# maxgillett/tinysplat

Measured on AMD Instinct MI355X. Metric: Gaussians*pixels/s fwd+bwd, higher is better.
Workload: dtype f32; 1 GPU; 1000000 random Gaussians, SH degree 3, 1920x1080, fwd+bwd (RGB), BASELINE configs[2]; max_per_tile=614, parallelism=single GPU, tile_lists=16x16 (gsplat's) (auto), gaussian_order=as generated (i.i.d.)

## Files before the change

include/tinysplat_hip.h:

```cpp
#ifndef TINYSPLAT_HIP_H
#define TINYSPLAT_HIP_H

#include <stdint.h>

#ifdef __cplusplus
extern "C" {
#endif

#define TS_ABI_VERSION 8

#define TS_E_BADARG (-1)
#define TS_E_DEGREE (-2)

#define TS_TILE 16
#define TS_SPLAT_RECORD_FLOATS 12
#define TS_PARTIAL_ROW_FLOATS 12

int ts_abi_version(void);

typedef struct ts_camera {
    float fx, fy, cx, cy;
    int32_t img_width, img_height;
    int32_t tile_bounds_x, tile_bounds_y;
    int32_t tile_row0, tile_rows;
    float glob_scale;
    float clip_thresh;
    int32_t wide_tiles;
    int32_t hints;
} ts_camera;
#define TS_HINT_BALANCED_WALK 1
#define TS_HINT_COOP_SPLIT (1 << 20)
#define TS_CAM_LIST_SEGMENTS(s) (((s) & 15) << 8)
#define TS_CAM_WHOLE_TILES(w16) (((w16) & 15) << 12)
#define TS_CAM_COOP_TILES(c16) (((c16) & 15) << 16)
int64_t ts_final_floats(const ts_camera* cam_host, int32_t channels);
int32_t ts_cut_tiles(const ts_camera* cam_host, int32_t* band, int32_t* whole);
int32_t ts_num_tiles(const ts_camera* cam_host);


#define TS_PROJECT_LOG_SCALES 1
#define TS_PROJECT_RAW_QUATS 2

int ts_project_fwd(int32_t n, const float* means3d, const float* scales, const float* quats,
                   const float* viewmat, const float* projmat, const ts_camera* cam_host,
                   int32_t flags, float* xys, float* depths, int32_t* radii, float* conics,
                   int32_t* num_tiles_hit, float* cov3d, void* stream);

int ts_project_bwd(int32_t n, const float* means3d, const float* scales, const float* quats,
                   const float* viewmat, const float* projmat, const ts_camera* cam_host,
                   int32_t flags, const int32_t* radii, const float* v_xy, const float* v_depth,
                   const float* v_conic, const float* v_cov3d,
                   float* v_means3d, float* v_scales, float* v_quats, void* stream);


int ts_sh_fwd(int32_t n, int32_t degrees_to_use, int32_t num_bases, const float* viewdirs,
              const float* coeffs, float* colors, void* stream);

int ts_sh_bwd(int32_t n, int32_t degrees_to_use, int32_t num_bases, const float* viewdirs,
              const float* v_colors, float* v_coeffs, void* stream);

int ts_sh_colors_fwd(int32_t n, int32_t degrees_to_use, int32_t num_bases, const float* means3d,
                     const float* origin, const float* colors_dc, const float* colors_rest,
                     float* colors, uint8_t* clamp_mask, const int32_t* live, void* stream);
int ts_sh_colors_bwd(int32_t n, int32_t degrees_to_use, int32_t num_bases, const float* means3d,
                     const float* origin, const uint8_t* clamp_mask, const float* v_colors,
                     float* v_colors_dc, float* v_colors_rest, void* stream);
int ts_colors_pack_fwd(int32_t n, int32_t degrees_to_use, int32_t num_bases, const float* means3d,
                       const float* origin, const float* colors_dc, const float* colors_rest,
                       uint8_t* clamp_mask, const int32_t* live, int32_t channels, int32_t flags,
                       const float* xys, const int32_t* radii, const float* conics, const float* opacity,
                       const int32_t* cum_tiles_hit, const ts_camera* cam_host, const float* depths,
                       float* splats, void* stream);


int64_t ts_scan_ws_ints(int32_t n);
int ts_scan_tiles(int32_t n, const int32_t* num_tiles_hit, int32_t* cum_tiles_hit,
                  int32_t* scan_ws, int32_t* total_out, void* stream);

int64_t ts_bin_ws_ints(int32_t n, int32_t num_tiles);

int ts_bin_count(int32_t n, const float* xys, const int32_t* radii, const float* splats,
                 const ts_camera* cam_host, int32_t* bin_ws, void* stream);

int ts_tile_offsets(int32_t n, int32_t num_tiles, int32_t* bin_ws, int32_t* tile_bins,
                    const int32_t* cum_tiles_hit, int64_t capacity, void* stream);
int ts_tile_offsets_stats(int32_t n, int32_t num_tiles, int32_t* bin_ws, int32_t* tile_bins,
                          const int32_t* cum_tiles_hit, int64_t capacity, int32_t* longest_list, void* stream);

int ts_bin_scatter(int32_t n, const float* xys, const int32_t* radii, const float* splats,
                   const ts_camera* cam_host, const int32_t* bin_ws, int32_t* bucket_ids, int32_t* scratch,
                   void* stream);

int ts_sort_tiles(int32_t num_tiles, const int32_t* tile_bins, const float* depths,
                  const int32_t* bucket_ids, int32_t* gaussian_ids_sorted, int32_t* sort_ws,
                  int32_t* zeroed_counter, void* stream);
int ts_sort_tiles_above(int32_t num_tiles, const int32_t* tile_bins, const float* depths,
                        const int32_t* bucket_ids, int32_t* gaussian_ids_sorted, int32_t* sort_ws,
                        int32_t* zeroed_counter, void* stream);

#define TS_RASTER_LOGIT_OPACITY 1

int ts_pack_splats(int32_t n, int32_t channels, int32_t flags, const float* xys, const int32_t* radii,
                   const float* conics, const float* colors, const float* opacity,
                   const int32_t* cum_tiles_hit, const ts_camera* cam_host, const float* depths,
                   float* splats, void* stream);

#define TS_RASTER_CLAMP_RGB 2
#define TS_RASTER_SPLIT_BLOCKS 4
#define TS_RASTER_NARROW_WAVES 8
#define TS_RASTER_FLAG_GEN(g) (((g) & 0xff) << 8)
int ts_raster_fwd(int32_t channels, int32_t flags, const ts_camera* cam_host, const int32_t* tile_bins,
                  const int32_t* gaussian_ids_sorted, const float* splats, const float* background,
                  float* out_img, float* final_Ts, int32_t* final_index, uint8_t* clamp_mask,
                  void* stream);
int ts_raster_fwd_planes(int32_t channels, int32_t flags, const ts_camera* cam_host, const int32_t* tile_bins,
                         const int32_t* gaussian_ids_sorted, const float* splats, const float* background,
                         float* out_img, float* out_depth, float* final_Ts, int32_t* final_index,
                         uint8_t* clamp_mask, void* stream);

int ts_raster_fwd_sort(int32_t channels, int32_t flags, const ts_camera* cam_host, const int32_t* tile_bins,
                       const int32_t* bucket_ids, const float* depths, int32_t* gaussian_ids_sorted,
                       const float* splats, const float* background, float* out_img, float* out_depth,
                       float* final_Ts, int32_t* final_index, uint8_t* clamp_mask, void* stream);

int ts_raster_bwd(int32_t channels, int32_t flags, int64_t num_intersects, const ts_camera* cam_host,
                  const int32_t* tile_bins, const int32_t* gaussian_ids_sorted, const float* splats,
                  const float* background, const float* final_Ts, const int32_t* final_index,
                  const float* v_out_img, const float* v_out_alpha, const uint8_t* clamp_mask,
                  float* partials, uint8_t* row_flags, void* stream);
int ts_raster_bwd_planes(int32_t channels, int32_t flags, int64_t num_intersects, const ts_camera* cam_host,
                         const int32_t* tile_bins, const int32_t* gaussian_ids_sorted, const float* splats,
                         const float* background, const float* final_Ts, const int32_t* final_index,
                         const float* v_out_img, const float* v_out_depth, int32_t planes,
                         const float* v_out_alpha, const uint8_t* clamp_mask,
                         float* partials, uint8_t* row_flags, void* stream);

int ts_reduce_partials(int32_t n, int32_t channels, int32_t flags, const int32_t* num_tiles_hit,
                       const int32_t* cum_tiles_hit, const float* partials,
                       const uint8_t* row_flags, const float* splats, float* v_xy, float* v_conic,
                       float* v_colors, float* v_opacity, float* v_depth, const uint8_t* color_mask,
                       void* stream);

#define TS_FRAME_TIGHT 1
#define TS_FRAME_SPLIT 2
#define TS_FRAME_NARROW_WAVES 8
#define TS_FRAME_DIRECT_SCATTER 32
#define TS_FRAME_PLANES 64
#define TS_FRAME_LIST_STATS 256
#define TS_FRAME_SEPARATE_SORT 128
#define TS_FRAME_STRIPE 16
#define TS_FRAME_SURVIVORS 512
typedef struct ts_frame {
    int32_t n, num_bases, sh_degree, channels, flags;
    int32_t flag_gen;
    ts_camera cam;
    const float *means, *scales, *quats, *opacities, *colors_dc, *colors_rest;
    const float *view34, *projview, *origin, *background;
    float *xys, *depths, *conics, *colors, *splats;
    int32_t *radii, *num_tiles_hit, *cum_tiles_hit;
    uint8_t* sh_mask;
    int32_t *scan_ws, *bin_ws, *tile_bins;
    int32_t* total_host;
    int64_t num_intersects;
    int64_t capacity;
    int32_t *bucket_ids, *gaussian_ids_sorted;
    float *out_img, *final_Ts;
    int32_t* final_index;
    uint8_t* clamp_mask;
    const float* v_out_img;
    float* partials;
    uint8_t* row_flags;
    float *v_xy, *v_conic, *v_colors, *v_depth, *v_opacity;
    float *v_means, *v_scales, *v_quats, *v_colors_dc, *v_colors_rest;
    float* out_depth;
    const float* v_out_depth;
    int32_t* survivors;
} ts_frame;
int32_t ts_frame_struct_bytes(void);
int ts_frame_fwd_project(const ts_frame* f, void* stream);
int ts_frame_fwd_prepare(const ts_frame* f, void* stream);
int ts_frame_fwd_composite(const ts_frame* f, void* stream);
int ts_frame_bwd_composite(const ts_frame* f, void* stream);
int ts_frame_bwd_params(const ts_frame* f, void* stream);

typedef void (*ts_entry_probe)(const char* entry, int32_t end, void* user);
int ts_set_entry_probe(ts_entry_probe fn, void* user);

#define TS_MAX_RANKS 16
#define TS_EXPORT_RECORD_FLOATS 16
typedef struct ts_stripes {
    int32_t num;
    int32_t row[TS_MAX_RANKS + 1];
} ts_stripes;
int64_t ts_route_ws_ints(int32_t n, int32_t num_ranks);
int ts_route_count(int32_t n, const float* xys, const int32_t* radii, const ts_camera* cam_host,
                   const ts_stripes* stripes_host, int32_t* route_ws, int32_t* counts, void* stream);
int ts_route_count_padded(int32_t n, const float* xys, const int32_t* radii, const ts_camera* cam_host,
                          const ts_stripes* stripes_host, const int32_t* group_base_host, int32_t* route_ws,
                          int32_t* counts, void* stream);
int ts_route_pack(int32_t n, int32_t gid_base, const float* xys, const int32_t* radii, const float* depths,
                  const float* splats, const ts_camera* cam_host, const ts_stripes* stripes_host,
                  const int32_t* route_ws, float* records, void* stream);
int ts_import_records(int32_t m, const float* records, const ts_camera* cam_host, float* xys, float* depths,
                      int32_t* radii, int32_t* num_tiles_hit, void* stream);
int ts_import_pack(int32_t m, const float* records, const int32_t* cum_tiles_hit, const ts_camera* cam_host,
                   float* splats, void* stream);
int ts_reduce_partials_rows(int32_t n, int32_t channels, int32_t flags, const int32_t* num_tiles_hit,
                            const int32_t* cum_tiles_hit, const float* partials, const uint8_t* row_flags,
                            const float* splats, float* grad_rows, void* stream);
int ts_route_accumulate(int32_t n, int32_t channels, const float* xys, const int32_t* radii, const float* splats,
                        const uint8_t* color_mask, const ts_camera* cam_host, const ts_stripes* stripes_host,
                        const int32_t* route_ws, const float* grad_rows, float* v_xy, float* v_conic,
                        float* v_colors, float* v_depth, float* v_opacity, void* stream);

int ts_shard_owner_fwd(const ts_frame* fo, const ts_stripes* stripes_host, int32_t* route_ws, int32_t* counts,
                       void* stream);
int ts_shard_owner_fwd_padded(const ts_frame* fo, const ts_stripes* stripes_host, const int32_t* group_base_host,
                              int32_t* route_ws, int32_t* counts, void* stream);
int ts_shard_owner_fwd_fused(int32_t n, int32_t degrees_to_use, int32_t num_bases, const float* means3d,
                             const float* scales, const float* quats, const float* view34, const float* projview,
                             const ts_camera* cam_host, int32_t project_flags, const float* origin,
                             const float* colors_dc, const float* colors_rest, const float* opacity, int32_t channels,
                             int32_t raster_flags, float* xys, float* depths, int32_t* radii, float* conics,
                             int32_t* num_tiles_hit, uint8_t* clamp_mask, float* splats, const ts_stripes* stripes_host,
                             const int32_t* group_base_host, int32_t* route_ws, int32_t* counts, void* stream);
int ts_shard_owner_bwd_fused(int32_t n, int32_t channels, int32_t degrees_to_use, int32_t num_bases, const float* means3d,
                             const float* scales, const float* quats, const float* view34, const float* projview,
                             const float* origin, const float* xys, const int32_t* radii, const float* splats,
                             const uint8_t* color_mask, const ts_camera* cam_host, const ts_stripes* stripes_host,
                             const int32_t* route_ws, const float* grad_rows, float* v_xy, float* v_conic,
                             float* v_colors, float* v_depth, float* v_opacity, float* v_colors_dc, float* v_colors_rest,
                             float* v_means3d, float* v_scales, float* v_quats, void* stream);
int ts_shard_stripe_fwd_import(const ts_frame* fs, const float* records, void* stream);
int ts_shard_stripe_bwd(const ts_frame* fs, float* grad_rows, void* stream);
int ts_shard_owner_bwd(const ts_frame* fo, const ts_stripes* stripes_host, const int32_t* route_ws,
                       const float* grad_rows, void* stream);

typedef struct ts_rank_step {
    ts_stripes stripes;
    int32_t group_base[TS_MAX_RANKS + 1];
    int32_t gid_base;
    int32_t send_rows, recv_rows;
    int32_t* route_ws;
    int32_t* counts;
    float *send, *recv;
    float *grad_rows, *back;
} ts_rank_step;
int32_t ts_rank_step_struct_bytes(void);
int ts_shard_rank_fwd_a(const ts_frame* fo, const ts_rank_step* r, void* stream);
int ts_shard_rank_fwd_b(const ts_frame* fs, const ts_rank_step* r, void* stream);
int ts_shard_rank_bwd_a(const ts_frame* fs, const ts_rank_step* r, void* stream);
int ts_shard_rank_bwd_b(const ts_frame* fo, const ts_rank_step* r, void* stream);


int64_t ts_photometric_ws_floats(int32_t height, int32_t width);
int ts_photometric_loss_rgbd(int32_t height, int32_t width, int32_t pixel_floats, const float* image,
                             const float* target, const float* depth_target, float w_l1,
                             float w_ssim, float w_depth, float* ws, float* v_image, void* stream);
int ts_photometric_loss(int32_t height, int32_t width, const float* image, const float* target,
                        float w_l1, float w_ssim, float* ws, float* v_image, void* stream);
int ts_photometric_loss_planes(int32_t height, int32_t width, const float* image, const float* depth,
                               const float* target, const float* depth_target, float w_l1, float w_ssim,
                               float w_depth, float* ws, float* v_image, float* v_depth, void* stream);
int ts_photometric_loss_reduce(int32_t height, int32_t width, float w_l1, float w_ssim, float w_depth,
                               const float* ws, float* out4, void* stream);

#define TS_ADAM_MAX_TENSORS 8
int ts_adam_step(int32_t num_tensors, float* const* params_host, const float* const* grads_host,
                 float* const* exp_avg_host, float* const* exp_avg_sq_host, const int64_t* numel_host,
                 const float* lr_host, const int32_t* steps_host, float beta1, float beta2, float eps,
                 void* stream);

#define TS_ADAM_MEANS 0
#define TS_ADAM_COLORS_DC 1
#define TS_ADAM_COLORS_REST 2
#define TS_ADAM_SCALES 3
#define TS_ADAM_QUATS 4
#define TS_ADAM_OPACITIES 5
typedef struct ts_adam {
    float* exp_avg[6];
    float* exp_avg_sq[6];
    float lr[6];
    int32_t step[6];
    float beta1, beta2, eps;
} ts_adam;
int ts_sh_colors_bwd_adam(int32_t n, int32_t degrees_to_use, int32_t num_bases, const float* means3d,
                          const float* origin, const uint8_t* clamp_mask, const float* v_colors,
                          float* colors_dc, float* colors_rest, const ts_adam* adam_host, void* stream);
int ts_project_bwd_adam(int32_t n, float* means3d, float* scales, float* quats, const float* viewmat,
                        const float* projmat, const ts_camera* cam_host, int32_t flags, const int32_t* radii,
                        const float* v_xy, const float* v_depth, const float* v_conic, float* opacities,
                        const float* v_opacity, const ts_adam* adam_host, void* stream);
int ts_frame_bwd_params_adam(const ts_frame* f, const ts_adam* adam_host, void* stream);

#define TS_DENSIFY_CLONE 1
#define TS_DENSIFY_SPLIT 2
#define TS_DENSIFY_PRUNE 4

typedef struct ts_densify_policy {
    float interval_densify;
    float max_dim;
    float tau_means;
    float scale_thresh;
} ts_densify_policy;

int ts_grad_accum(int32_t n, const float* v_xy, float* accum, void* stream);

int ts_densify_classify(int32_t n, const float* accum, const float* scales, const float* opacities,
                        const ts_densify_policy* policy, uint8_t* flags, void* stream);

int64_t ts_densify_ws_ints(int32_t n);
int ts_densify_plan(int32_t n, const uint8_t* flags, int32_t* ws, int32_t* counts, int32_t* src_of,
                    void* stream);

#define TS_GATHER_MAX_TENSORS 8
int ts_gather_rows(int32_t num_tensors, const float* const* src_host, float* const* dst_host,
                   const int32_t* row_floats_host, int32_t dst_rows, int32_t copy_rows,
                   const int32_t* src_of, void* stream);

int ts_split_fixup(int32_t rows, const int32_t* src_of_split, const float* means, const float* scales,
                   const float* quats, const float* z, float* means_out, float* scales_out,
                   void* stream);

int32_t ts_ply_row_floats(int32_t k_rest);
int ts_ply_pack_rows(int32_t n, int32_t k_rest, const float* means, const float* colors_dc,
                     const float* colors_rest, const float* opacities, const float* scales,
                     const float* quats, float* rows, void* stream);
int ts_ply_unpack_rows(int32_t n, int32_t k_rest, const float* rows, float* means, float* colors_dc,
                       float* colors_rest, float* opacities, float* scales, float* quats,
                       void* stream);

#define TS_KNN_MAX_K 16
int64_t ts_knn_ws_bytes(int32_t n, int32_t m, int32_t k);
int ts_knn(int32_t n, const float* points, int32_t m, const float* queries, int32_t k, float* dist,
           int32_t* idx, void* ws, int32_t* stats, void* stream);

// ... 76 lines not shown
```

tinysplat_amd/_lib.py:

```python
from __future__ import annotations

import ctypes
import os
from ctypes import POINTER, c_float, c_int32, c_int64, c_void_p
from pathlib import Path

LIB_PATH = Path(os.environ["TS_LIB_PATH"]) if os.environ.get("TS_LIB_PATH") else \
    Path(__file__).resolve().parent / "csrc" / "libtinysplat_hip.so"
ABI_VERSION = 8
HINT_BALANCED_WALK = 1
HINT_COOP_SPLIT = 1 << 20
PARTIAL_ROW_FLOATS = 12


class TsCamera(ctypes.Structure):
    _fields_ = [
        ("fx", c_float), ("fy", c_float), ("cx", c_float), ("cy", c_float),
        ("img_width", c_int32), ("img_height", c_int32),
        ("tile_bounds_x", c_int32), ("tile_bounds_y", c_int32),
        ("tile_row0", c_int32), ("tile_rows", c_int32),
        ("glob_scale", c_float), ("clip_thresh", c_float),
        ("wide_tiles", c_int32), ("hints", c_int32),
    ]


_P = c_void_p
_CAM = POINTER(TsCamera)


class TsDensifyPolicy(ctypes.Structure):
    _fields_ = [("interval_densify", c_float), ("max_dim", c_float), ("tau_means", c_float),
                ("scale_thresh", c_float)]


class TsFrame(ctypes.Structure):
    _fields_ = ([("n", c_int32), ("num_bases", c_int32), ("sh_degree", c_int32), ("channels", c_int32),
                 ("flags", c_int32), ("flag_gen", c_int32), ("cam", TsCamera)]
                + [(name, c_void_p) for name in (
                    "means", "scales", "quats", "opacities", "colors_dc", "colors_rest",
                    "view34", "projview", "origin", "background",
                    "xys", "depths", "conics", "colors", "splats",
                    "radii", "num_tiles_hit", "cum_tiles_hit", "sh_mask",
                    "scan_ws", "bin_ws", "tile_bins", "total_host")]
                + [("num_intersects", c_int64), ("capacity", c_int64)]
                + [(name, c_void_p) for name in (
                    "bucket_ids", "gaussian_ids_sorted", "out_img", "final_Ts", "final_index", "clamp_mask",
                    "v_out_img", "partials", "row_flags",
                    "v_xy", "v_conic", "v_colors", "v_depth", "v_opacity",
                    "v_means", "v_scales", "v_quats", "v_colors_dc", "v_colors_rest",
                    "out_depth", "v_out_depth", "survivors")])


_FRAME = POINTER(TsFrame)


class TsAdam(ctypes.Structure):
    _fields_ = [("exp_avg", c_void_p * 6), ("exp_avg_sq", c_void_p * 6), ("lr", c_float * 6), ("step", c_int32 * 6),
                ("beta1", c_float), ("beta2", c_float), ("eps", c_float)]


_ADAM = POINTER(TsAdam)

MAX_RANKS = 16


class TsStripes(ctypes.Structure):
    _fields_ = [("num", c_int32), ("row", c_int32 * (MAX_RANKS + 1))]


_STRIPES = POINTER(TsStripes)


class TsRankStep(ctypes.Structure):
    _fields_ = [("stripes", TsStripes), ("group_base", c_int32 * (MAX_RANKS + 1)), ("gid_base", c_int32),
                ("send_rows", c_int32), ("recv_rows", c_int32), ("route_ws", c_void_p), ("counts", c_void_p),
                ("send", c_void_p), ("recv", c_void_p), ("grad_rows", c_void_p), ("back", c_void_p)]


_RANK = POINTER(TsRankStep)

ENTRY_PROBE = ctypes.CFUNCTYPE(None, ctypes.c_char_p, c_int32, c_void_p)

SIGNATURES = {
    "ts_abi_version": (c_int32, []),
    "ts_project_fwd": (c_int32, [c_int32, _P, _P, _P, _P, _P, _CAM, c_int32, _P, _P, _P, _P, _P, _P, _P]),
    "ts_project_bwd": (c_int32, [c_int32, _P, _P, _P, _P, _P, _CAM, c_int32, _P, _P, _P, _P, _P, _P, _P, _P, _P]),
    "ts_sh_fwd": (c_int32, [c_int32, c_int32, c_int32, _P, _P, _P, _P]),
    "ts_sh_bwd": (c_int32, [c_int32, c_int32, c_int32, _P, _P, _P, _P]),
    "ts_sh_colors_fwd": (c_int32, [c_int32, c_int32, c_int32, _P, _P, _P, _P, _P, _P, _P, _P]),
    "ts_sh_colors_bwd": (c_int32, [c_int32, c_int32, c_int32, _P, _P, _P, _P, _P, _P, _P]),
    "ts_scan_ws_ints": (c_int64, [c_int32]),
    "ts_scan_tiles": (c_int32, [c_int32, _P, _P, _P, _P, _P]),
    "ts_bin_ws_ints": (c_int64, [c_int32, c_int32]),
    "ts_bin_count": (c_int32, [c_int32, _P, _P, _P, _CAM, _P, _P]),
    "ts_tile_offsets": (c_int32, [c_int32, c_int32, _P, _P, _P, c_int64, _P]),
    "ts_tile_offsets_stats": (c_int32, [c_int32, c_int32, _P, _P, _P, c_int64, _P, _P]),
    "ts_bin_scatter": (c_int32, [c_int32, _P, _P, _P, _CAM, _P, _P, _P, _P]),
    "ts_sort_tiles": (c_int32, [c_int32, _P, _P, _P, _P, _P, _P, _P]),
    "ts_sort_tiles_above": (c_int32, [c_int32, _P, _P, _P, _P, _P, _P, _P]),
    "ts_num_tiles": (c_int32, [_CAM]),
    "ts_final_floats": (c_int64, [_CAM, c_int32]),
    "ts_cut_tiles": (c_int32, [_CAM, _P, _P]),
    "ts_colors_pack_fwd": (c_int32, [c_int32, c_int32, c_int32, _P, _P, _P, _P, _P, _P, c_int32, c_int32,
                                     _P, _P, _P, _P, _P, _CAM, _P, _P, _P]),
    "ts_pack_splats": (c_int32, [c_int32, c_int32, c_int32, _P, _P, _P, _P, _P, _P, _CAM, _P, _P, _P]),
    "ts_raster_fwd": (c_int32, [c_int32, c_int32, _CAM, _P, _P, _P, _P, _P, _P, _P, _P, _P]),
    "ts_raster_bwd": (c_int32, [c_int32, c_int32, c_int64, _CAM, _P, _P, _P, _P, _P, _P, _P, _P, _P, _P, _P, _P]),
    "ts_raster_fwd_planes": (c_int32, [c_int32, c_int32, _CAM, _P, _P, _P, _P, _P, _P, _P, _P, _P, _P]),
    "ts_raster_fwd_sort": (c_int32, [c_int32, c_int32, _CAM, _P, _P, _P, _P, _P, _P, _P, _P, _P, _P, _P, _P]),
    "ts_raster_bwd_planes": (c_int32, [c_int32, c_int32, c_int64, _CAM, _P, _P, _P, _P, _P, _P, _P, _P, c_int32,
                                       _P, _P, _P, _P, _P]),
    "ts_bench_stream_read": (c_int32, [_P, c_int64, _P, _P]),
    "ts_bench_gather48": (c_int32, [_P, _P, c_int64, _P, _P]),
    "ts_photometric_ws_floats": (c_int64, [c_int32, c_int32]),
    "ts_photometric_loss": (c_int32, [c_int32, c_int32, _P, _P, c_float, c_float, _P, _P, _P]),
    "ts_photometric_loss_rgbd": (c_int32, [c_int32, c_int32, c_int32, _P, _P, _P, c_float, c_float, c_float, _P, _P, _P]),
    "ts_photometric_loss_planes": (c_int32, [c_int32, c_int32, _P, _P, _P, _P, c_float, c_float, c_float, _P, _P, _P,
                                             _P]),
    "ts_photometric_loss_reduce": (c_int32, [c_int32, c_int32, c_float, c_float, c_float, _P, _P, _P]),
    "ts_adam_step": (c_int32, [c_int32, _P, _P, _P, _P, _P, _P, _P, c_float, c_float, c_float, _P]),
    "ts_sh_colors_bwd_adam": (c_int32, [c_int32, c_int32, c_int32, _P, _P, _P, _P, _P, _P, _ADAM, _P]),
    "ts_project_bwd_adam": (c_int32, [c_int32, _P, _P, _P, _P, _P, _CAM, c_int32, _P, _P, _P, _P, _P, _P, _ADAM, _P]),
    "ts_frame_bwd_params_adam": (c_int32, [_FRAME, _ADAM, _P]),
    "ts_grad_accum": (c_int32, [c_int32, _P, _P, _P]),
    "ts_densify_classify": (c_int32, [c_int32, _P, _P, _P, POINTER(TsDensifyPolicy), _P, _P]),
    "ts_densify_ws_ints": (c_int64, [c_int32]),
    "ts_densify_plan": (c_int32, [c_int32, _P, _P, _P, _P, _P]),
    "ts_gather_rows": (c_int32, [c_int32, _P, _P, _P, c_int32, c_int32, _P, _P]),
    "ts_split_fixup": (c_int32, [c_int32, _P, _P, _P, _P, _P, _P, _P, _P]),
    "ts_ply_row_floats": (c_int32, [c_int32]),
    "ts_ply_pack_rows": (c_int32, [c_int32, c_int32, _P, _P, _P, _P, _P, _P, _P, _P]),
    "ts_ply_unpack_rows": (c_int32, [c_int32, c_int32, _P, _P, _P, _P, _P, _P, _P, _P]),
    "ts_reduce_partials": (c_int32, [c_int32, c_int32, c_int32, _P, _P, _P, _P, _P, _P, _P, _P, _P, _P, _P, _P]),
    "ts_route_ws_ints": (c_int64, [c_int32, c_int32]),
    "ts_route_count": (c_int32, [c_int32, _P, _P, _CAM, _STRIPES, _P, _P, _P]),
    "ts_route_count_padded": (c_int32, [c_int32, _P, _P, _CAM, _STRIPES, _P, _P, _P, _P]),
    "ts_route_pack": (c_int32, [c_int32, c_int32, _P, _P, _P, _P, _CAM, _STRIPES, _P, _P, _P]),
    "ts_import_records": (c_int32, [c_int32, _P, _CAM, _P, _P, _P, _P, _P]),
    "ts_import_pack": (c_int32, [c_int32, _P, _P, _CAM, _P, _P]),
    "ts_reduce_partials_rows": (c_int32, [c_int32, c_int32, c_int32, _P, _P, _P, _P, _P, _P, _P]),
    "ts_route_accumulate": (c_int32, [c_int32, c_int32, _P, _P, _P, _P, _CAM, _STRIPES, _P, _P, _P, _P, _P, _P, _P, _P]),
    "ts_shard_owner_fwd": (c_int32, [_FRAME, _STRIPES, _P, _P, _P]),
    "ts_shard_owner_fwd_padded": (c_int32, [_FRAME, _STRIPES, _P, _P, _P, _P]),
    "ts_shard_owner_fwd_fused": (c_int32, [c_int32, c_int32, c_int32, _P, _P, _P, _P, _P, _CAM, c_int32, _P, _P, _P, _P,
                                           c_int32, c_int32, _P, _P, _P, _P, _P, _P, _P, _STRIPES, _P, _P, _P, _P]),
    "ts_shard_owner_bwd_fused": (c_int32, [c_int32, c_int32, c_int32, c_int32, _P, _P, _P, _P, _P, _P, _P, _P, _P, _P,
                                           _CAM, _STRIPES, _P, _P, _P, _P, _P, _P, _P, _P, _P, _P, _P, _P, _P]),
    "ts_shard_stripe_fwd_import": (c_int32, [_FRAME, _P, _P]),
    "ts_shard_stripe_bwd": (c_int32, [_FRAME, _P, _P]),
    "ts_shard_owner_bwd": (c_int32, [_FRAME, _STRIPES, _P, _P, _P]),
    "ts_rank_step_struct_bytes": (c_int32, []),
    "ts_shard_rank_fwd_a": (c_int32, [_FRAME, _RANK, _P]),
    "ts_shard_rank_fwd_b": (c_int32, [_FRAME, _RANK, _P]),
    "ts_shard_rank_bwd_a": (c_int32, [_FRAME, _RANK, _P]),
    "ts_shard_rank_bwd_b": (c_int32, [_FRAME, _RANK, _P]),
    "ts_frame_struct_bytes": (c_int32, []),
    "ts_frame_fwd_project": (c_int32, [_FRAME, _P]),
    "ts_frame_fwd_prepare": (c_int32, [_FRAME, _P]),
    "ts_frame_fwd_composite": (c_int32, [_FRAME, _P]),
    "ts_frame_bwd_composite": (c_int32, [_FRAME, _P]),
    "ts_frame_bwd_params": (c_int32, [_FRAME, _P]),
    "ts_set_entry_probe": (c_int32, [_P, _P]),
    "ts_knn_ws_bytes": (c_int64, [c_int32, c_int32, c_int32]),
    "ts_knn": (c_int32, [c_int32, _P, c_int32, _P, c_int32, _P, _P, _P, _P, _P]),
    "ts_init_from_points": (c_int32, [c_int32, c_int32, _P, _P, _P, _P, _P, _P, _P, _P, _P, _P, _P, _P, _P, _P]),
    "ts_opacity_entropy_ws_bytes": (c_int64, [c_int32]),
    "ts_opacity_entropy": (c_int32, [c_int32, _P, _P, _P, _P, _P]),
    "ts_density_sample_ws_bytes": (c_int64, [c_int32]),
    "ts_density_sample": (c_int32, [c_int32, c_int32, c_int32, _P, _P, _P, _P, _P, _P, _P, _P, _P, _P, _P]),
    "ts_density_loss_ws_bytes": (c_int64, [c_int32]),
    "ts_density_loss": (c_int32, [c_int32, c_int32, _P, _P, _P, _P, _P, _P, _P, _P, c_int32, c_int32, _P, _P, c_int32,
                                  c_float, _P, _P, _P, _P, _P, _P, _P, _P, _P, _P]),
    "ts_segment_sum_ws_bytes": (c_int64, [c_int64, c_int32]),
    "ts_segment_sum": (c_int32, [c_int64, c_int32, c_int32, _P, _P, _P, _P, _P, _P, _P]),
    "ts_extract_pack": (c_int32, [c_int32, _P, _P, _P, _P, _P, _P, _P]),
    "ts_extract_rays": (c_int32, [c_int32, _P, c_int32, c_int32, _P, c_int32, _P, _P, _P, _P, _P, _P]),
    "ts_extract_samples": (c_int32, [c_int32, c_int32, c_int32, c_float, _P, _P, _P, _P, _P, _P, _P]),
    "ts_extract_march": (c_int32, [c_int32, c_int32, c_int32, c_float, c_float, _P, _P, _P, _P, _P, _P, _P, _P, _P, _P,
                                   _P, _P, _P]),
    "ts_extract_normals": (c_int32, [c_int32, c_int32, _P, _P, _P, _P, _P]),
    "ts_extract_chunk_bytes": (c_int64, [c_int32, c_int32, c_int32]),
    "ts_mesh_boxes": (c_int32, [c_int32, _P, _P, _P, c_float, _P, _P]),
    "ts_mesh_mark": (c_int32, [c_int32, _P, _P, _P, _P, _P]),
    "ts_mesh_chunk_bytes": (c_int64, [c_int32, c_int32]),
    "ts_mesh_corners": (c_int32, [c_int32, _P, _P, _P, _P, _P]),
    "ts_mesh_density": (c_int32, [c_int32, c_int32, _P, _P, _P, _P, _P, _P, _P, _P]),
    "ts_mesh_count": (c_int32, [c_int32, _P, _P, _P, c_float, _P, _P, _P]),
    "ts_mesh_emit": (c_int32, [c_int32, _P, _P, _P, c_float, _P, _P, _P, _P, _P, _P]),
}

_lib = None


class HipLibraryError(RuntimeError):
    pass


def load() -> ctypes.CDLL:
    global _lib
    if _lib is not None:
        return _lib
    if not LIB_PATH.exists():
        raise HipLibraryError(
            f"{LIB_PATH} is missing: tinysplat_amd has no CPU or PyTorch fallback. "
            "Build it with `python -m tinysplat_amd._build` (needs hipcc, targets gfx950).")
    stamp = LIB_PATH.with_suffix(LIB_PATH.suffix + ".flags")
    if stamp.exists() and "-DTS_" in stamp.read_text() and os.environ.get("TS_ALLOW_VARIANT_LIB") != "1":
        raise HipLibraryError(
            f"{LIB_PATH} was built with developer -DTS_* overrides (ablation variant; its results may be "
            "wrong). Rebuild with `python -m tinysplat_amd._build`, or set TS_ALLOW_VARIANT_LIB=1.")
    lib = ctypes.CDLL(str(LIB_PATH))
    for name, (res, args) in SIGNATURES.items():
        try:
            fn = getattr(lib, name)
        except AttributeError as e:
            raise HipLibraryError(f"{LIB_PATH} does not export {name}") from e
        fn.restype = res
        fn.argtypes = args
    v = lib.ts_abi_version()
    if v != ABI_VERSION:
        raise HipLibraryError(f"ABI version mismatch: library {v}, binding {ABI_VERSION}")
    if lib.ts_frame_struct_bytes() != ctypes.sizeof(TsFrame):
        raise HipLibraryError("struct ts_frame: the ctypes mirror does not match the library's layout")
    if lib.ts_rank_step_struct_bytes() != ctypes.sizeof(TsRankStep):
        raise HipLibraryError("struct ts_rank_step: the ctypes mirror does not match the library's layout")
    _lib = lib
    return lib


def check(code: int, what: str) -> None:
    if code == 0:
        return
    if code == -1:
        raise ValueError(f"{what}: bad argument (TS_E_BADARG)")
    if code == -2:
        raise ValueError(f"{what}: SH degree / number of bases not supported (TS_E_DEGREE)")
    raise RuntimeError(f"{what}: HIP error {code}")
```

tinysplat_amd/csrc/binning.hip:

```cpp
#include <hip/hip_runtime.h>

#include "../../include/tinysplat_hip.h"
#include "pack.h"
#include "splat_math.h"

namespace {

constexpr int kThreads = 256;
constexpr int kScanItems = 4;
constexpr int kScanBlock = kThreads * kScanItems;

__device__ __forceinline__ int wave_inclusive_scan(int v) {
    const int lane = threadIdx.x & 63;
#pragma unroll
    for (int d = 1; d < 64; d <<= 1) {
        const int u = __shfl_up(v, d, 64);
        if (lane >= d) v += u;
    }
    return v;
}

template <int WAVES = 4>
__device__ __forceinline__ int block_inclusive_scan(int v, int* total) {
    __shared__ int wave_sums[WAVES];
    const int lane = threadIdx.x & 63, wave = threadIdx.x >> 6;
    int inc = wave_inclusive_scan(v);
    if (lane == 63) wave_sums[wave] = inc;
    __syncthreads();
    int add = 0, tot = 0;
#pragma unroll
    for (int w = 0; w < WAVES; ++w) {
        const int s = wave_sums[w];
        if (w < wave) add += s;
        tot += s;
    }
    *total = tot;
    __syncthreads();
    return inc + add;
}

__global__ __launch_bounds__(kThreads) void scan_local_kernel(int n, const int* __restrict__ in,
                                                              int* __restrict__ out,
                                                              int* __restrict__ block_sums,
                                                              int* __restrict__ total_out) {
    const int base = blockIdx.x * kScanBlock + threadIdx.x * kScanItems;
    int v[kScanItems];
    int sum = 0;
#pragma unroll
    for (int k = 0; k < kScanItems; ++k) {
        v[k] = (base + k < n) ? in[base + k] : 0;
        sum += v[k];
        v[k] = sum;
    }
    int total;
    const int inc = block_inclusive_scan(sum, &total);
    const int excl = inc - sum;
#pragma unroll
    for (int k = 0; k < kScanItems; ++k)
        if (base + k < n) {
            out[base + k] = v[k] + excl;
            if (total_out && gridDim.x == 1 && base + k == n - 1)
                __hip_atomic_store(total_out, v[k] + excl, __ATOMIC_RELEASE, __HIP_MEMORY_SCOPE_SYSTEM);
        }
    if (threadIdx.x == 0) block_sums[blockIdx.x] = total;
}

__global__ __launch_bounds__(kThreads) void scan_add_kernel(int n, int* __restrict__ out,
                                                            const int* __restrict__ block_sums,
                                                            int* __restrict__ total_out) {
    __shared__ int red[kThreads / 64];
    int part = 0;
    for (int j = threadIdx.x; j < (int)blockIdx.x; j += kThreads) part += block_sums[j];
#pragma unroll
    for (int d = 32; d >= 1; d >>= 1) part += __shfl_xor(part, d, 64);
    if ((threadIdx.x & 63) == 0) red[threadIdx.x >> 6] = part;
    __syncthreads();
    int add = 0;
#pragma unroll
    for (int w = 0; w < kThreads / 64; ++w) add += red[w];
    const int base = blockIdx.x * kScanBlock + threadIdx.x * kScanItems;
#pragma unroll
    for (int k = 0; k < kScanItems; ++k)
        if (base + k < n) {
            const int v = out[base + k] + add;
            if (blockIdx.x != 0) out[base + k] = v;
            if (total_out && base + k == n - 1)
                __hip_atomic_store(total_out, v, __ATOMIC_RELEASE, __HIP_MEMORY_SCOPE_SYSTEM);
        }
}

#ifndef TS_BIN_THREADS
#define TS_BIN_THREADS 1024
#endif
constexpr int kBinThreads = TS_BIN_THREADS;
#ifndef TS_BIN_CHUNK
#define TS_BIN_CHUNK 4096
#endif
constexpr int kBinChunkMin = TS_BIN_CHUNK;
constexpr int kBinMaxChunks = 512;
constexpr int kBinWindowMax = 36864;
constexpr int kBinTargetBlocks = 1;

__host__ __device__ inline int bin_num_chunks(int n) {
    int per = n / 192;
    per = per < 1024 ? 1024 : (per > kBinChunkMin ? kBinChunkMin : per);
    int b = (n + per - 1) / per;
    if (b < 1) b = 1;
    if (b > kBinMaxChunks) b = kBinMaxChunks;
    return b;
}

inline int bin_window_tiles(int n, int num_tiles) {
    const int chunks = bin_num_chunks(n);
    int nwin = (kBinTargetBlocks + chunks - 1) / chunks;
    const int max_win = (num_tiles + 255) / 256;
    if (nwin > max_win) nwin = max_win;
    if (nwin < 1) nwin = 1;
    int window = (num_tiles + nwin - 1) / nwin;
    window = (window + 63) & ~63;
    if (window > kBinWindowMax) window = kBinWindowMax;
    return window;
}

using ts::TightTest;

#ifndef TS_BIN_PRE
#define TS_BIN_PRE 2
#endif
constexpr int kBinPre = TS_BIN_PRE;
template <typename Emit>
__device__ __forceinline__ void walk_chunk(int g0, int g1, const float* __restrict__ xys,
                                           const int* __restrict__ radii,
                                           const float4* __restrict__ splats, const ts_camera& cam,
                                           Emit emit) {
    const int ws = cam.wide_tiles ? 1 : 0;
    const int tbx = (cam.tile_bounds_x + ws) >> ws;
    const bool tight_lists = splats != nullptr;
    for (int base = g0 + threadIdx.x; base < g1; base += kBinPre * kBinThreads) {
        int r[kBinPre];
        float2 xy[kBinPre];
        float4 q0[kBinPre], q1[kBinPre];
#pragma unroll
        for (int u = 0; u < kBinPre; ++u) {
            const int i = base + u * kBinThreads;
            r[u] = i < g1 ? radii[i] : 0;
        }
#pragma unroll
        for (int u = 0; u < kBinPre; ++u) {
            const int i = base + u * kBinThreads;
            xy[u] = make_float2(0.f, 0.f);
            q0[u] = q1[u] = make_float4(0.f, 0.f, 0.f, 0.f);
            if (r[u] > 0) {
                xy[u] = reinterpret_cast<const float2*>(xys)[i];
                if (tight_lists) { q0[u] = splats[3 * (size_t)i]; q1[u] = splats[3 * (size_t)i + 1]; }
            }
        }
#pragma unroll
        for (int u = 0; u < kBinPre; ++u) {
            if (r[u] <= 0) continue;
            const ts::TileBox b = ts::tile_bbox(xy[u].x, xy[u].y, (float)r[u], cam.tile_bounds_x,
                                                cam.tile_bounds_y, cam.tile_row0, cam.tile_rows);
            if (b.maxy <= b.miny || b.maxx <= b.minx) continue;
            const TightTest tight(tight_lists, q0[u].x, q0[u].y, q0[u].z, q0[u].w, q1[u].x, q1[u].y, (float)r[u]);
            if (tight.cull_all) continue;
            const int i = base + u * kBinThreads;
            for (int ty = b.miny; ty < b.maxy; ++ty) {
                int lo, hi;
                tight.row_range(ty, b.minx, b.maxx, lo, hi);
                if (hi <= lo) continue;
                for (int tx = lo >> ws; tx <= (hi - 1) >> ws; ++tx) emit((ty - cam.tile_row0) * tbx + tx, i);
            }
        }
    }
}

constexpr int kItemCap = 4096;
constexpr int kStashWords = 11;
constexpr size_t kBalancedLds = (size_t)(kStashWords * kBinThreads + kItemCap + 32) * 4;
template <typename Emit>
__device__ __forceinline__ void walk_chunk_balanced(int g0, int g1, const float* __restrict__ xys,
                                                    const int* __restrict__ radii,
                                                    const float4* __restrict__ splats, const ts_camera& cam,
                                                    Emit emit) {
    static_assert(kBinThreads == 1024, "one Gaussian per thread and batch, items packed as lt | row << 10");
    __shared__ float stash[kStashWords][kBinThreads];
    __shared__ int items[kItemCap];
    __shared__ int wave_sum[kBinThreads / 64 + 1];
    const int ws = cam.wide_tiles ? 1 : 0;
    const int tbx = (cam.tile_bounds_x + ws) >> ws;
    const bool tight_lists = splats != nullptr;
    const int tid = threadIdx.x, lane = tid & 63, wave = tid >> 6;
    for (int base = g0; base < g1; base += kBinThreads) {
        const int i = base + tid;
        int rows = 0, miny = 0;
        if (i < g1) {
            const int r = radii[i];
            if (r > 0) {
                const float2 xy = reinterpret_cast<const float2*>(xys)[i];
                float4 q0 = make_float4(0.f, 0.f, 0.f, 0.f), q1 = q0;
                if (tight_lists) { q0 = splats[3 * (size_t)i]; q1 = splats[3 * (size_t)i + 1]; }
                const ts::TileBox b = ts::tile_bbox(xy.x, xy.y, (float)r, cam.tile_bounds_x, cam.tile_bounds_y,
                                                    cam.tile_row0, cam.tile_rows);
                if (b.maxy > b.miny && b.maxx > b.minx) {
                    const TightTest t(tight_lists, q0.x, q0.y, q0.z, q0.w, q1.x, q1.y, (float)r);
                    if (!t.cull_all) {
                        rows = b.maxy - b.miny;
                        miny = b.miny;
                        stash[0][tid] = t.geometric ? t.dymax : -1.0f;
                        stash[1][tid] = t.gx; stash[2][tid] = t.gy; stash[3][tid] = t.B; stash[4][tid] = t.D4;
                        stash[5][tid] = t.inv2A; stash[6][tid] = t.tau4A; stash[7][tid] = t.dxext;
                        stash[8][tid] = t.dy_left; stash[9][tid] = __int_as_float(b.miny);
                        stash[10][tid] = __int_as_float(b.minx | (b.maxx << 16));
                    }
                }
            }
        }
        int incl = rows;
#pragma unroll
        for (int d = 1; d < 64; d <<= 1) {
            const int v = __shfl_up(incl, d, 64);
            if (lane >= d) incl += v;
        }
        if (lane == 63) wave_sum[wave] = incl;
        __syncthreads();
        if (wave == 0) {
            int v = lane < kBinThreads / 64 ? wave_sum[lane] : 0;
#pragma unroll
            for (int d = 1; d < kBinThreads / 64; d <<= 1) {
                const int u = __shfl_up(v, d, 64);
                if (lane >= d) v += u;
            }
            if (lane < kBinThreads / 64) wave_sum[lane] = v;
        }
        __syncthreads();
        const int total = wave_sum[kBinThreads / 64 - 1];
        const int first = incl - rows + (wave > 0 ? wave_sum[wave - 1] : 0);
        for (int w0 = 0; w0 < total; w0 += kItemCap) {
            const int lo_k = max(0, w0 - first), hi_k = min(rows, w0 + kItemCap - first);
            for (int k = lo_k; k < hi_k; ++k) items[first + k - w0] = tid | (k << 10);
            __syncthreads();
            const int m = min(kItemCap, total - w0);
            for (int j = tid; j < m; j += kBinThreads) {
                const int it = items[j], lt = it & 1023, k = it >> 10;
                TightTest t(false, 0.0f, 0.0f, 0.0f, 0.0f, 0.0f, 0.0f, 0.0f);
                const float d0 = stash[0][lt];
                t.geometric = d0 >= 0.0f;
                t.dymax = d0;
                t.gx = stash[1][lt]; t.gy = stash[2][lt]; t.B = stash[3][lt]; t.D4 = stash[4][lt];
                t.inv2A = stash[5][lt]; t.tau4A = stash[6][lt]; t.dxext = stash[7][lt]; t.dy_left = stash[8][lt];
                const int ty = __float_as_int(stash[9][lt]) + k;
                const int xx = __float_as_int(stash[10][lt]);
                int lo, hi;
                t.row_range(ty, xx & 0xffff, xx >> 16, lo, hi);
                if (hi <= lo) continue;
                const int id = base + lt;
                for (int tx = lo >> ws; tx <= (hi - 1) >> ws; ++tx) emit((ty - cam.tile_row0) * tbx + tx, id);
            }
            __syncthreads();
        }
        __syncthreads();
    }
}

template <bool BAL>
__global__ __launch_bounds__(kBinThreads) void bin_count_kernel(
    int n, int chunk, const float* __restrict__ xys, const int* __restrict__ radii,
    const float4* __restrict__ splats, const ts_camera cam, int num_tiles, int window,
    int* __restrict__ counts) {
    extern __shared__ int hist[];
    const int t0 = blockIdx.y * window;
    const int tw = min(num_tiles - t0, window);
    for (int j = threadIdx.x; j < tw; j += kBinThreads) hist[j] = 0;
    __syncthreads();
    const int g0 = blockIdx.x * chunk, g1 = min(n, g0 + chunk);
    auto emit = [&](int t, int) {
        t -= t0;
        if ((unsigned)t < (unsigned)tw) atomicAdd(&hist[t], 1);
    };
    if (BAL) walk_chunk_balanced(g0, g1, xys, radii, splats, cam, emit);
    else walk_chunk(g0, g1, xys, radii, splats, cam, emit);
    __syncthreads();
    int* dst = counts + (size_t)blockIdx.x * num_tiles + t0;
    for (int j = threadIdx.x; j < tw; j += kBinThreads) dst[j] = hist[j];
}

constexpr int kScanGroups = 16;

constexpr int kColTiles = 64;
constexpr int kColPer = (kBinMaxChunks + kScanGroups - 1) / kScanGroups;
__global__ __launch_bounds__(kColTiles * kScanGroups) void column_scan_kernel(int num_tiles, int chunks,
                                                                              int per_group,
                                                                              int* __restrict__ counts,
                                                                              int* __restrict__ tile_total) {
    __shared__ int gsum[kScanGroups][kColTiles];
    const int tl = threadIdx.x & (kColTiles - 1), g = threadIdx.x / kColTiles;
    const int t = blockIdx.x * kColTiles + tl;
    const int b0 = g * per_group, b1 = min(chunks, b0 + per_group);
    int c[kColPer];
    int sum = 0;
    if (t < num_tiles) {
#pragma unroll
        for (int j = 0; j < kColPer; ++j) c[j] = (b0 + j < b1) ? counts[(size_t)(b0 + j) * num_tiles + t] : 0;
#pragma unroll
        for (int j = 0; j < kColPer; ++j) {
            const int v = c[j];
            c[j] = sum;
            sum += v;
        }
    }
    gsum[g][tl] = sum;
    __syncthreads();
    if (t >= num_tiles) return;
    int base = 0, tot = 0;
#pragma unroll
    for (int q = 0; q < kScanGroups; ++q) {
        const int v = gsum[q][tl];
        if (q < g) base += v;
        tot += v;
    }
#pragma unroll
    for (int j = 0; j < kColPer; ++j)
        if (b0 + j < b1) counts[(size_t)(b0 + j) * num_tiles + t] = base + c[j];
    if (g == 0) tile_total[t] = tot;
}

constexpr int kOffsetsThreads = 1024;
__global__ __launch_bounds__(kOffsetsThreads) void tile_offsets_kernel(int num_tiles,
                                                                       int* __restrict__ tile_total,
                                                                       int* __restrict__ tile_bins,
                                                                       int* __restrict__ spare,
                                                                       const int* __restrict__ total_ptr,
                                                                       long long capacity, int* __restrict__ longest_out) {
    constexpr int kPer = 8;
    __shared__ int carry, over, longest;
    int my_longest = 0;
    if (threadIdx.x == 0) {
        carry = 0;
        longest = 0;
        *spare = 0;
        over = (total_ptr && capacity >= 0 && ((long long)*total_ptr > capacity || *total_ptr < 0)) ? 1 : 0;
        spare[-1] = over;
    }
    __syncthreads();
    if (over) {
        for (int t = threadIdx.x; t <= num_tiles; t += kOffsetsThreads) {
            tile_total[t] = 0;
            if (t < num_tiles) reinterpret_cast<int2*>(tile_bins)[t] = make_int2(0, 0);
        }
        return;
    }
    for (int base = 0; base < num_tiles; base += kOffsetsThreads * kPer) {
        const int t0 = base + threadIdx.x * kPer;
        int v[kPer], sum = 0;
#pragma unroll
        for (int e = 0; e < kPer; ++e) {
            v[e] = (t0 + e < num_tiles) ? tile_total[t0 + e] : 0;
            sum += v[e];
            my_longest = max(my_longest, v[e]);
        }
        int total;
        const int inc = block_inclusive_scan<kOffsetsThreads / 64>(sum, &total);
        int start = carry + inc - sum;
#pragma unroll
        for (int e = 0; e < kPer; ++e) {
            if (t0 + e < num_tiles) {
                tile_total[t0 + e] = start;
                reinterpret_cast<int2*>(tile_bins)[t0 + e] =
                    v[e] > 0 ? make_int2(start, start + v[e]) : make_int2(0, 0);
            }
            start += v[e];
        }
        __syncthreads();
        if (threadIdx.x == 0) carry += total;
        __syncthreads();
    }
    if (threadIdx.x == 0) tile_total[num_tiles] = carry;
    if (longest_out) {
        atomicMax(&longest, my_longest);
        __syncthreads();
        if (threadIdx.x == 0) *longest_out = longest;
    }
}

__global__ __launch_bounds__(kBinThreads) void bin_scatter_kernel(
    int n, int chunk, const float* __restrict__ xys,
    const int* __restrict__ radii, const float4* __restrict__ splats, const ts_camera cam,
    int num_tiles, int window, const int* __restrict__ bases, const int* __restrict__ tile_start,
    int* __restrict__ bucket_ids) {
    extern __shared__ int cursor[];
    if (tile_start[num_tiles + 1] != 0) return;
    const int t0 = blockIdx.y * window;
    const int tw = min(num_tiles - t0, window);
    const int* src = bases + (size_t)blockIdx.x * num_tiles + t0;
    for (int j = threadIdx.x; j < tw; j += kBinThreads) cursor[j] = tile_start[t0 + j] + src[j];
    __syncthreads();
    const int g0 = blockIdx.x * chunk, g1 = min(n, g0 + chunk);
    walk_chunk(g0, g1, xys, radii, splats, cam, [&](int t, int i) {
        t -= t0;
        if ((unsigned)t < (unsigned)tw) bucket_ids[atomicAdd(&cursor[t], 1)] = i;
    });
}

#ifndef TS_COARSE_SHIFT
#define TS_COARSE_SHIFT 5
#endif
constexpr int kCoarseShift = TS_COARSE_SHIFT;
constexpr int kCoarseTiles = 1 << kCoarseShift;
constexpr int kCoarseIdBits = 32 - kCoarseShift;
#ifndef TS_TWO_HOP_FROM
#define TS_TWO_HOP_FROM (1 << 18)
#endif
constexpr int kTwoHopFrom = TS_TWO_HOP_FROM;

template <bool BAL>
__global__ __launch_bounds__(kBinThreads) void bin_scatter_coarse_kernel(
    int n, int chunk, const float* __restrict__ xys, const int* __restrict__ radii,
    const float4* __restrict__ splats, const ts_camera cam, int num_tiles, const int* __restrict__ bases,
    const int* __restrict__ tile_start, int* __restrict__ scratch) {
    extern __shared__ int cursor[];
    if (tile_start[num_tiles + 1] != 0) return;
    const int groups = (num_tiles + kCoarseTiles - 1) >> kCoarseShift;
    const int* src = bases + (size_t)blockIdx.x * num_tiles;
    for (int g = threadIdx.x; g < groups; g += kBinThreads) cursor[g] = tile_start[g << kCoarseShift];
    __syncthreads();
    for (int t = threadIdx.x; t < num_tiles; t += kBinThreads) {
        const int v = src[t];
        if (v) atomicAdd(&cursor[t >> kCoarseShift], v);
    }
    __syncthreads();
    const int g0 = blockIdx.x * chunk, g1 = min(n, g0 + chunk);
    auto emit = [&](int t, int i) {
        scratch[atomicAdd(&cursor[t >> kCoarseShift], 1)] = i | ((t & (kCoarseTiles - 1)) << kCoarseIdBits);
    };
    if (BAL) walk_chunk_balanced(g0, g1, xys, radii, splats, cam, emit);
    else walk_chunk(g0, g1, xys, radii, splats, cam, emit);
}

#ifndef TS_FINE_THREADS
#define TS_FINE_THREADS 1024
#endif
#ifndef TS_FINE_AHEAD
#define TS_FINE_AHEAD 8
#endif
constexpr int kFineThreads = TS_FINE_THREADS;
constexpr int kFineAhead = TS_FINE_AHEAD;
constexpr int kFinePass = kFineThreads * kFineAhead;
__global__ __launch_bounds__(kFineThreads) void bin_scatter_fine_kernel(int num_tiles,
                                                                        const int* __restrict__ tile_start,
                                                                        const int* __restrict__ scratch,
                                                                        int* __restrict__ bucket_ids) {
    __shared__ int cursor[kCoarseTiles];
    const int t0 = blockIdx.x << kCoarseShift, t1 = min(num_tiles, t0 + kCoarseTiles);
    if ((int)threadIdx.x < t1 - t0) cursor[threadIdx.x] = tile_start[t0 + threadIdx.x];
    const int begin = tile_start[t0], end = tile_start[t1];
    __shared__ int hist[kCoarseTiles], loff[kCoarseTiles + 1], gbase[kCoarseTiles];
    __shared__ int ids[kFinePass];
    __shared__ unsigned char tiles[kFinePass];
    if ((int)threadIdx.x < kCoarseTiles) hist[threadIdx.x] = 0;
    __syncthreads();
    for (int c0 = begin; c0 < end; c0 += kFinePass) {
        const int m = min(kFinePass, end - c0);
        unsigned int w[kFineAhead];
        int rank[kFineAhead];
#pragma unroll
        for (int u = 0; u < kFineAhead; ++u) {
            const int k = u * kFineThreads + (int)threadIdx.x;
            if (k < m) w[u] = (unsigned int)scratch[c0 + k];
        }
#pragma unroll
        for (int u = 0; u < kFineAhead; ++u) {
            const int k = u * kFineThreads + (int)threadIdx.x;
            if (k < m) rank[u] = atomicAdd(&hist[w[u] >> kCoarseIdBits], 1);
        }
        __syncthreads();
        if ((int)threadIdx.x < 64) {
            const int t = threadIdx.x;
            const int c = t < kCoarseTiles ? hist[t] : 0;
            int inc = c;
#pragma unroll
            for (int d = 1; d < kCoarseTiles; d <<= 1) {
                const int o = __shfl_up(inc, d, 64);
                if (t >= d) inc += o;
            }
            if (t < kCoarseTiles) {
                loff[t] = inc - c;
                gbase[t] = cursor[t];
                cursor[t] += c;
                hist[t] = 0;
            }
        }
        __syncthreads();
#pragma unroll
        for (int u = 0; u < kFineAhead; ++u) {
            const int k = u * kFineThreads + (int)threadIdx.x;
            if (k < m) {
                const int t = (int)(w[u] >> kCoarseIdBits);
                const int lp = loff[t] + rank[u];
                ids[lp] = (int)(w[u] & ((1u << kCoarseIdBits) - 1u));
                tiles[lp] = (unsigned char)t;
            }
        }
        __syncthreads();
#pragma unroll
        for (int u = 0; u < kFineAhead; ++u) {
            const int k = u * kFineThreads + (int)threadIdx.x;
            if (k < m) {
                const int t = tiles[k];
                bucket_ids[gbase[t] + (k - loff[t])] = ids[k];
            }
        }
        __syncthreads();
    }
}

constexpr int kSortCap = 4096;

#include "sort_network.h"

struct IdKeyArray {
    volatile int* ids;
    const float* depths;
};

__device__ __forceinline__ void cmpswap(IdKeyArray a, int i, int j) {
    const int x = a.ids[i], y = a.ids[j];
    if (make_key(a.depths, x) > make_key(a.depths, y)) { a.ids[i] = y; a.ids[j] = x; }
}

template <typename Ptr>
__device__ __forceinline__ void bitonic_network(Ptr a, int n) {
    int lg = 0;
    while ((1 << lg) < n) ++lg;
    const int half = (1 << lg) >> 1;
    for (int lk = 1; lk <= lg; ++lk) {
        const int k = 1 << lk, hk = k >> 1;
// ... 144 lines not shown
}

__global__ __launch_bounds__(kThreads) void sort_tiles_small_kernel(
    int num_tiles, const int* __restrict__ tile_bins, const float* __restrict__ depths,
    const int* __restrict__ bucket_ids, int* __restrict__ ids_sorted, int* __restrict__ large_count,
    int* __restrict__ large_list) {
    const int lane = threadIdx.x & 63;
    const int tile = blockIdx.x * (kThreads / 64) + (threadIdx.x >> 6);
    if (tile >= num_tiles) return;
    const int2 range = reinterpret_cast<const int2*>(tile_bins)[tile];
    const int n = range.y - range.x;
    if (n <= 0) return;
    if (n > kWaveSortMax) {
        if (n > kSortCap && lane == 0) large_list[atomicAdd(large_count, 1)] = tile;
        return;
    }
    const int* g = bucket_ids + range.x;
    int* out = ids_sorted + range.x;
    if (n <= 64) sort_tile_wave<1>(g, depths, out, n, lane);
    else if (n <= 128) sort_tile_wave<2>(g, depths, out, n, lane);
    else if (n <= 256) sort_tile_wave<4>(g, depths, out, n, lane);
    else if (n <= 512) sort_tile_wave<8>(g, depths, out, n, lane);
    else sort_tile_wave<16>(g, depths, out, n, lane);
}

__global__ __launch_bounds__(kThreads) void sort_tiles_mid_kernel(
    const int* __restrict__ tile_bins, const float* __restrict__ depths,
    const int* __restrict__ bucket_ids, int* __restrict__ ids_sorted, int* __restrict__ large_count,
    int* __restrict__ large_list) {
    __shared__ unsigned long long lk[kSortCap / 2];
    const int2 range = reinterpret_cast<const int2*>(tile_bins)[blockIdx.x];
    const int n = range.y - range.x;
    if (n > kSortCap && large_count && threadIdx.x == 0) large_list[atomicAdd(large_count, 1)] = blockIdx.x;
    if (n <= kWaveSortMax || n > kSortCap) return;
    sort_bucket_block(bucket_ids + range.x, depths, ids_sorted + range.x, n, lk);
}

__global__ __launch_bounds__(kThreads) void sort_tiles_large_kernel(
    const int* __restrict__ tile_bins, const float* __restrict__ depths,
    const int* __restrict__ bucket_ids, int* __restrict__ ids_sorted,
    const int* __restrict__ large_count, const int* __restrict__ large_list) {
    __shared__ unsigned long long lds_large[kLargeLdsU64];
    const int count = *large_count;
    for (int q = blockIdx.x; q < count; q += gridDim.x) {
        const int2 range = reinterpret_cast<const int2*>(tile_bins)[large_list[q]];
        const int n = range.y - range.x;
        if (n <= kSortCap) continue;
        __syncthreads();
        sort_tile_sample(bucket_ids + range.x, depths, ids_sorted + range.x, n, lds_large);
    }
}

__global__ __launch_bounds__(kThreads) void sort_tiles_above_kernel(
    const int* __restrict__ tile_bins, const float* __restrict__ depths,
    const int* __restrict__ bucket_ids, int* __restrict__ ids_sorted) {
    __shared__ unsigned long long lds_u64[kLargeLdsU64 > kSortCap / 2 ? kLargeLdsU64 : kSortCap / 2];
    const int2 range = reinterpret_cast<const int2*>(tile_bins)[blockIdx.x];
    const int n = range.y - range.x;
    if (n <= kWaveSortMax) return;
    if (n <= kSortCap) sort_bucket_block(bucket_ids + range.x, depths, ids_sorted + range.x, n, lds_u64);
    else sort_tile_sample(bucket_ids + range.x, depths, ids_sorted + range.x, n, lds_u64);
}

__global__ __launch_bounds__(kThreads) void pack_splats_kernel(int n, const ts::PackArgs a,
                                                              const float* __restrict__ colors) {
    const int i = blockIdx.x * kThreads + threadIdx.x;
    if (i >= n) return;
    if (a.radii[i] <= 0) return;
    float c0, c1, c2, c3 = 0.0f;
    if (a.channels == 4 && a.depths == nullptr) {
        const float4 c = reinterpret_cast<const float4*>(colors)[i];
        c0 = c.x; c1 = c.y; c2 = c.z; c3 = c.w;
    } else {
        c0 = colors[3 * i]; c1 = colors[3 * i + 1]; c2 = colors[3 * i + 2];
        if (a.channels == 4) c3 = a.depths[i];
    }
    ts::pack_one(a, i, c0, c1, c2, c3);
}

inline int launch_status() { return (int)hipGetLastError(); }

}

extern "C" {

int32_t ts_num_tiles(const ts_camera* cam) {
    if (!cam) return 0;
    const int tbx = cam->wide_tiles ? (cam->tile_bounds_x + 1) / 2 : cam->tile_bounds_x;
    return cam->tile_rows * tbx;
}

int64_t ts_scan_ws_ints(int32_t n) {
    return n <= 0 ? 1 : (int64_t)((n + kScanBlock - 1) / kScanBlock);
}

int ts_scan_tiles(int32_t n, const int32_t* num_tiles_hit, int32_t* cum_tiles_hit,
                  int32_t* scan_ws, int32_t* total_out, void* stream) {
    if (n < 0) return TS_E_BADARG;
    if (n == 0) return 0;
    if (!num_tiles_hit || !cum_tiles_hit || !scan_ws) return TS_E_BADARG;
    hipStream_t s = (hipStream_t)stream;
    const int nb = (n + kScanBlock - 1) / kScanBlock;
    hipLaunchKernelGGL(scan_local_kernel, dim3(nb), dim3(kThreads), 0, s, n, num_tiles_hit,
                       cum_tiles_hit, scan_ws, total_out);
    if (nb > 1)
        hipLaunchKernelGGL(scan_add_kernel, dim3(nb), dim3(kThreads), 0, s, n, cum_tiles_hit, scan_ws,
                           total_out);
    return launch_status();
}

int64_t ts_bin_ws_ints(int32_t n, int32_t num_tiles) {
    if (num_tiles < 0) num_tiles = 0;
    return (int64_t)(bin_num_chunks(n) + 1) * num_tiles + 3;
}



int ts_bin_count(int32_t n, const float* xys, const int32_t* radii, const float* splats,
                 const ts_camera* cam, int32_t* bin_ws, void* stream) {
    if (n < 0 || !cam || !bin_ws) return TS_E_BADARG;
    const int nt = ts_num_tiles(cam);
    if (nt <= 0) return 0;
    if (n > 0 && (!xys || !radii)) return TS_E_BADARG;
    const int chunks = bin_num_chunks(n);
    const int chunk = n > 0 ? (n + chunks - 1) / chunks : 1;
    const int window = bin_window_tiles(n, nt);
    const int windows = (nt + window - 1) / window;
    const size_t lds = (size_t)window * sizeof(int);
    if (lds > 64 * 1024)
        (void)hipFuncSetAttribute(reinterpret_cast<const void*>(&bin_count_kernel<false>),
                                  hipFuncAttributeMaxDynamicSharedMemorySize, (int)lds);
    hipLaunchKernelGGL(bin_count_kernel<false>, dim3(chunks, windows), dim3(kBinThreads), lds,
                       (hipStream_t)stream, n, chunk, xys, radii,
                       reinterpret_cast<const float4*>(splats), *cam, nt, window, bin_ws);
    return launch_status();
}

int ts_tile_offsets(int32_t n, int32_t num_tiles, int32_t* bin_ws, int32_t* tile_bins,
                    const int32_t* cum_tiles_hit, int64_t capacity, void* stream) {
    return ts_tile_offsets_stats(n, num_tiles, bin_ws, tile_bins, cum_tiles_hit, capacity, nullptr, stream);
}

int ts_tile_offsets_stats(int32_t n, int32_t num_tiles, int32_t* bin_ws, int32_t* tile_bins,
                          const int32_t* cum_tiles_hit, int64_t capacity, int32_t* longest_list, void* stream) {
    if (n < 0 || num_tiles < 0) return TS_E_BADARG;
    if (num_tiles == 0) return 0;
    if (!bin_ws || !tile_bins) return TS_E_BADARG;
    const int chunks = bin_num_chunks(n);
    int* tile_total = bin_ws + (size_t)chunks * num_tiles;
    const int per_group = (chunks + kScanGroups - 1) / kScanGroups;
    hipStream_t s = (hipStream_t)stream;
    hipLaunchKernelGGL(column_scan_kernel, dim3((num_tiles + kColTiles - 1) / kColTiles),
                       dim3(kColTiles * kScanGroups), 0, s, num_tiles, chunks, per_group, bin_ws, tile_total);
    hipLaunchKernelGGL(tile_offsets_kernel, dim3(1), dim3(kOffsetsThreads), 0, s, num_tiles, tile_total,
                       tile_bins, bin_ws + (ts_bin_ws_ints(n, num_tiles) - 1),
                       (cum_tiles_hit && n > 0) ? cum_tiles_hit + (n - 1) : nullptr, (long long)capacity, longest_list);
    return launch_status();
}

int ts_bin_scatter(int32_t n, const float* xys, const int32_t* radii, const float* splats,
                   const ts_camera* cam, const int32_t* bin_ws, int32_t* bucket_ids, int32_t* scratch,
                   void* stream) {
    if (n < 0 || !cam) return TS_E_BADARG;
    if (n == 0) return 0;
    if (!xys || !radii || !bin_ws || !bucket_ids) return TS_E_BADARG;
    const int nt = ts_num_tiles(cam);
    if (nt <= 0) return 0;
    const int chunks = bin_num_chunks(n);
    const int chunk = (n + chunks - 1) / chunks;
    const int* tile_start = bin_ws + (size_t)chunks * nt;
    if (scratch && n >= kTwoHopFrom && n < (1 << kCoarseIdBits)) {
        const int groups = (nt + kCoarseTiles - 1) >> kCoarseShift;
        if (cam->hints & TS_HINT_BALANCED_WALK)
            hipLaunchKernelGGL(bin_scatter_coarse_kernel<true>, dim3(chunks), dim3(kBinThreads),
                               (size_t)groups * sizeof(int), (hipStream_t)stream, n, chunk, xys, radii,
                               reinterpret_cast<const float4*>(splats), *cam, nt, bin_ws, tile_start, scratch);
        else
            hipLaunchKernelGGL(bin_scatter_coarse_kernel<false>, dim3(chunks), dim3(kBinThreads),
                               (size_t)groups * sizeof(int), (hipStream_t)stream, n, chunk, xys, radii,
                               reinterpret_cast<const float4*>(splats), *cam, nt, bin_ws, tile_start, scratch);
        hipLaunchKernelGGL(bin_scatter_fine_kernel, dim3(groups), dim3(kFineThreads), 0, (hipStream_t)stream, nt,
                           tile_start, scratch, bucket_ids);
        return launch_status();
    }
    const int window = bin_window_tiles(n, nt);
    const int windows = (nt + window - 1) / window;
    const size_t lds = (size_t)window * sizeof(int);
    if (lds > 64 * 1024)
        (void)hipFuncSetAttribute(reinterpret_cast<const void*>(&bin_scatter_kernel),
                                  hipFuncAttributeMaxDynamicSharedMemorySize, (int)lds);
    hipLaunchKernelGGL(bin_scatter_kernel, dim3(chunks, windows), dim3(kBinThreads), lds,
                       (hipStream_t)stream, n, chunk, xys, radii,
                       reinterpret_cast<const float4*>(splats), *cam, nt, window, bin_ws,
                       tile_start, bucket_ids);
    return launch_status();
}

int ts_sort_tiles(int32_t num_tiles, const int32_t* tile_bins, const float* depths,
                  const int32_t* bucket_ids, int32_t* gaussian_ids_sorted, int32_t* sort_ws,
                  int32_t* zeroed_counter, void* stream) {
    if (num_tiles < 0) return TS_E_BADARG;
    if (num_tiles == 0) return 0;
    if (!tile_bins || !depths || !bucket_ids || !gaussian_ids_sorted || !sort_ws) return TS_E_BADARG;
    hipStream_t s = (hipStream_t)stream;
    int32_t* counter = zeroed_counter ? zeroed_counter : sort_ws;
    int32_t* list = zeroed_counter ? sort_ws : sort_ws + 1;
    if (!zeroed_counter) {
        hipError_t e = hipMemsetAsync(sort_ws, 0, sizeof(int32_t), s);
        if (e != hipSuccess) return (int)e;
    }
    hipLaunchKernelGGL(sort_tiles_small_kernel, dim3((num_tiles + kThreads / 64 - 1) / (kThreads / 64)),
                       dim3(kThreads), 0, s, (int)num_tiles, tile_bins, depths, bucket_ids,
                       gaussian_ids_sorted, counter, list);
    hipLaunchKernelGGL(sort_tiles_mid_kernel, dim3(num_tiles), dim3(kThreads), 0, s, tile_bins, depths,
                       bucket_ids, gaussian_ids_sorted, (int*)nullptr, (int*)nullptr);
    const int grid = num_tiles < 768 ? num_tiles : 768;
    hipLaunchKernelGGL(sort_tiles_large_kernel, dim3(grid), dim3(kThreads), 0, s, tile_bins, depths,
                       bucket_ids, gaussian_ids_sorted, counter, list);
    return launch_status();
}

int ts_sort_tiles_above(int32_t num_tiles, const int32_t* tile_bins, const float* depths,
                        const int32_t* bucket_ids, int32_t* gaussian_ids_sorted, int32_t* sort_ws,
                        int32_t* zeroed_counter, void* stream) {
    if (num_tiles < 0) return TS_E_BADARG;
    if (num_tiles == 0) return 0;
    if (!tile_bins || !depths || !bucket_ids || !gaussian_ids_sorted) return TS_E_BADARG;
    (void)sort_ws; (void)zeroed_counter;
    hipLaunchKernelGGL(sort_tiles_above_kernel, dim3(num_tiles), dim3(kThreads), 0, (hipStream_t)stream, tile_bins,
                       depths, bucket_ids, gaussian_ids_sorted);
    return launch_status();
}

int ts_pack_splats(int32_t n, int32_t channels, int32_t flags, const float* xys, const int32_t* radii,
                   const float* conics, const float* colors, const float* opacity,
                   const int32_t* cum_tiles_hit, const ts_camera* cam, const float* depths, float* splats,
                   void* stream) {
    if (n < 0 || !cam || (channels != 3 && channels != 4)) return TS_E_BADARG;
    if (n == 0) return 0;
    if (!xys || !radii || !conics || !colors || !opacity || !cum_tiles_hit || !splats)
        return TS_E_BADARG;
    ts::PackArgs a;
    a.channels = channels; a.flags = (int)flags; a.xys = xys; a.radii = radii; a.conics = conics;
    a.opacity = opacity; a.cum_tiles_hit = cum_tiles_hit; a.depths = depths;
    a.splats = reinterpret_cast<float4*>(splats); a.cam = *cam;
    hipLaunchKernelGGL(pack_splats_kernel, dim3((n + kThreads - 1) / kThreads), dim3(kThreads), 0,
                       (hipStream_t)stream, n, a, colors);
    return launch_status();
}

}
```

tinysplat_amd/csrc/frame.hip:

```cpp
#include <hip/hip_runtime.h>

#include <atomic>
#include <cstdlib>
#if !defined(TS_NO_ROCTX) && __has_include(<rocprofiler-sdk-roctx/roctx.h>)
#include <rocprofiler-sdk-roctx/roctx.h>
#define TS_HAVE_ROCTX 1
#else
#define TS_HAVE_ROCTX 0
#endif

#include "../../include/tinysplat_hip.h"
#include "raster_survivors.h"

struct TsRange {
#if TS_HAVE_ROCTX
    explicit TsRange(const char* name) { roctxRangePush(name); }
    ~TsRange() { roctxRangePop(); }
#else
    explicit TsRange(const char*) {}
#endif
};

static std::atomic<ts_entry_probe> g_probe{nullptr};
static std::atomic<void*> g_probe_user{nullptr};

struct TsEntry {
    explicit TsEntry(const char* label) : fn_(g_probe.load(std::memory_order_relaxed)), label_(label) {
        if (fn_) {
            std::atomic_thread_fence(std::memory_order_acquire);
            user_ = g_probe_user.load(std::memory_order_relaxed);
            fn_(label_, 0, user_);
        }
    }
    ~TsEntry() {
        if (fn_) fn_(label_, 1, user_);
    }
    ts_entry_probe fn_;
    const char* label_;
    void* user_ = nullptr;
};
#define TS_ENTRY(label, call) ((void)TsEntry(label), (call))

#define TS_TRY(call)                 \
    do {                             \
        const int e_ = (call);       \
        if (e_ != 0) return e_;      \
    } while (0)

namespace {
inline bool bad(const ts_frame* f) {
    return !f || f->n < 0 || (f->channels != 3 && f->channels != 4) || f->num_bases < 1;
}
inline int num_tiles(const ts_frame* f) { return ts_num_tiles(&f->cam); }
inline int32_t* mapped_pointer(int32_t* host) {
    static thread_local int32_t* last_host = nullptr;
    static thread_local int32_t* last_dev = nullptr;
    static thread_local int last_device = -1;
    int device = -1;
    if (hipGetDevice(&device) != hipSuccess) return nullptr;
    if (host == last_host && device == last_device) return last_dev;
    void* dev = nullptr;
    if (hipHostGetDevicePointer(&dev, host, 0) != hipSuccess || !dev) {
        (void)hipGetLastError();
        return nullptr;
    }
    last_host = host;
    last_device = device;
    last_dev = static_cast<int32_t*>(dev);
    return last_dev;
}
inline bool segmented(const ts_frame* f) {
    return ((f->cam.hints >> 8) & 15) > 1 && !f->cam.wide_tiles && !(f->flags & TS_FRAME_NARROW_WAVES);
}
inline int bwd_split(const ts_frame* f) {
    return ((f->flags & TS_FRAME_SPLIT) && !segmented(f)) ? TS_RASTER_SPLIT_BLOCKS : 0;
}
inline int small_n_fused() {
    static const int v = [] {
        const char* e = getenv("TS_SMALL_N_FUSED");
        return e ? atoi(e) : 262144;
    }();
    return v;
}
inline bool survivors(const ts_frame* f) {
    return (f->flags & TS_FRAME_SURVIVORS) && f->survivors && f->final_Ts && f->num_intersects > 0 &&
           f->cam.wide_tiles == 0 &&
           !(f->flags & (TS_FRAME_SPLIT | TS_FRAME_NARROW_WAVES | TS_FRAME_SEPARATE_SORT));
}
inline int raster_flags(const ts_frame* f) {
    return TS_RASTER_CLAMP_RGB | ((f->flags & TS_FRAME_SPLIT) ? TS_RASTER_SPLIT_BLOCKS : 0) |
           ((f->flags & TS_FRAME_NARROW_WAVES) ? TS_RASTER_NARROW_WAVES : 0);
}
}

extern "C" {

int32_t ts_frame_struct_bytes(void) { return (int32_t)sizeof(ts_frame); }

int ts_set_entry_probe(ts_entry_probe fn, void* user) {
    g_probe_user.store(user, std::memory_order_relaxed);
    g_probe.store(fn, std::memory_order_release);
    return 0;
}

int ts_frame_fwd_project(const ts_frame* f, void* stream) {
    TsRange range_("ts_frame_fwd_project");
    if (bad(f)) return TS_E_BADARG;
    TS_TRY(TS_ENTRY("ts_project_fwd",
                    ts_project_fwd(f->n, f->means, f->scales, f->quats, f->view34, f->projview, &f->cam, 3, f->xys,
                                   f->depths, f->radii, f->conics, f->num_tiles_hit, nullptr, stream)));
    int32_t* total_dev = f->total_host ? mapped_pointer(f->total_host) : nullptr;
    TS_TRY(TS_ENTRY("ts_scan_tiles",
                    ts_scan_tiles(f->n, f->num_tiles_hit, f->cum_tiles_hit, f->scan_ws, total_dev, stream)));
    if (f->n > 0 && f->total_host && !total_dev) {
        const hipError_t e = hipMemcpyAsync(f->total_host, f->cum_tiles_hit + (f->n - 1), sizeof(int32_t),
                                            hipMemcpyDeviceToHost, (hipStream_t)stream);
        if (e != hipSuccess) return (int)e;
    }
    return 0;
}

int ts_frame_fwd_prepare(const ts_frame* f, void* stream) {
    TsRange range_("ts_frame_fwd_prepare");
    if (bad(f)) return TS_E_BADARG;
    TS_TRY(TS_ENTRY("ts_colors_pack_fwd",
                    ts_colors_pack_fwd(f->n, f->sh_degree, f->num_bases, f->means, f->origin, f->colors_dc,
                                       f->num_bases > 1 ? f->colors_rest : nullptr, f->sh_mask,
                                       (f->flags & TS_FRAME_STRIPE) ? f->num_tiles_hit : nullptr, f->channels,
                                       TS_RASTER_LOGIT_OPACITY, f->xys, f->radii, f->conics, f->opacities,
                                       f->cum_tiles_hit, &f->cam, f->channels == 4 ? f->depths : nullptr, f->splats,
                                       stream)));
    const float* tight = (f->flags & TS_FRAME_TIGHT) ? f->splats : nullptr;
    TS_TRY(TS_ENTRY("ts_bin_count", ts_bin_count(f->n, f->xys, f->radii, tight, &f->cam, f->bin_ws, stream)));
    int32_t* longest = nullptr;
    if ((f->flags & TS_FRAME_LIST_STATS) && f->total_host) {
        int32_t* dev = mapped_pointer(f->total_host);
        if (dev) longest = dev + 1;
    }
    TS_TRY(TS_ENTRY("ts_tile_offsets",
                    ts_tile_offsets_stats(f->n, num_tiles(f), f->bin_ws, f->tile_bins, f->cum_tiles_hit, f->capacity,
                                          longest, stream)));
    return 0;
}

int ts_frame_fwd_composite(const ts_frame* f, void* stream) {
    TsRange range_("ts_frame_fwd_composite");
    if (bad(f) || f->num_intersects < 0) return TS_E_BADARG;
    const bool planes = (f->flags & TS_FRAME_PLANES) != 0;
    if (planes && (f->channels != 4 || !f->out_depth)) return TS_E_BADARG;
    const bool fused_sort = f->num_intersects > 0 && f->cam.wide_tiles == 0 &&
                            !(f->flags & (TS_FRAME_NARROW_WAVES | TS_FRAME_SEPARATE_SORT));
    if (f->num_intersects > 0) {
        const float* tight = (f->flags & TS_FRAME_TIGHT) ? f->splats : nullptr;
        TS_TRY(TS_ENTRY("ts_bin_scatter",
                        ts_bin_scatter(f->n, f->xys, f->radii, tight, &f->cam, f->bin_ws, f->bucket_ids,
                                       (f->flags & TS_FRAME_DIRECT_SCATTER) ? nullptr : f->gaussian_ids_sorted,
                                       stream)));
        int32_t* counter = f->bin_ws + (ts_bin_ws_ints(f->n, num_tiles(f)) - 1);
        if (fused_sort)
            TS_TRY(TS_ENTRY("ts_sort_tiles",
                            ts_sort_tiles_above(num_tiles(f), f->tile_bins, f->depths, f->bucket_ids,
                                                f->gaussian_ids_sorted, f->bin_ws, counter, stream)));
        else
            TS_TRY(TS_ENTRY("ts_sort_tiles",
                            ts_sort_tiles(num_tiles(f), f->tile_bins, f->depths, f->bucket_ids, f->gaussian_ids_sorted,
                                          f->bin_ws, counter, stream)));
    }
    if (fused_sort)
        return TS_ENTRY("ts_raster_fwd",
                        ts_surv::raster_fwd_sort(f->channels, raster_flags(f), &f->cam, f->tile_bins, f->bucket_ids,
                                                 f->depths, f->gaussian_ids_sorted, f->splats, f->background,
                                                 f->out_img, planes ? f->out_depth : nullptr, f->final_Ts,
                                                 f->final_index, f->clamp_mask, survivors(f) ? f->survivors : nullptr,
                                                 stream));
    return TS_ENTRY("ts_raster_fwd",
                    ts_raster_fwd_planes(f->channels, raster_flags(f), &f->cam, f->tile_bins, f->gaussian_ids_sorted,
                                         f->splats, f->background, f->out_img, planes ? f->out_depth : nullptr,
                                         f->final_Ts, f->final_index, f->clamp_mask, stream));
}

int ts_frame_bwd_composite(const ts_frame* f, void* stream) {
    TsRange range_("ts_frame_bwd_composite");
    if (bad(f) || f->num_intersects < 0) return TS_E_BADARG;
    const bool planes = (f->flags & TS_FRAME_PLANES) != 0;
    const bool surv = survivors(f);
    TS_TRY(TS_ENTRY("ts_raster_bwd",
                    ts_surv::raster_bwd(f->channels,
                                        ((raster_flags(f) & ~(TS_RASTER_CLAMP_RGB | TS_RASTER_SPLIT_BLOCKS)) | bwd_split(f)) |
                                            TS_RASTER_FLAG_GEN(f->flag_gen),
                                        f->num_intersects, &f->cam, f->tile_bins, f->gaussian_ids_sorted, f->splats,
                                        f->background, f->final_Ts, f->final_index, f->v_out_img,
                                        planes ? f->v_out_depth : nullptr, planes ? 1 : 0, nullptr, f->clamp_mask,
                                        f->partials, f->row_flags, surv ? f->bucket_ids : nullptr,
                                        surv ? f->survivors : nullptr, stream)));
    const bool stripe = (f->flags & TS_FRAME_STRIPE) != 0;
    return TS_ENTRY("ts_reduce_partials",
                    ts_reduce_partials(f->n, f->channels,
                                       TS_RASTER_LOGIT_OPACITY | bwd_split(f) | TS_RASTER_FLAG_GEN(f->flag_gen),
                                       f->num_tiles_hit, f->cum_tiles_hit, f->partials, f->row_flags, f->splats,
                                       f->v_xy, f->v_conic, f->v_colors, f->v_opacity,
                                       f->channels == 4 ? f->v_depth : nullptr, stripe ? f->sh_mask : nullptr, stream));
}

int ts_frame_bwd_params(const ts_frame* f, void* stream) {
    TsRange range_("ts_frame_bwd_params");
    if (bad(f)) return TS_E_BADARG;
    TS_TRY(TS_ENTRY("ts_sh_colors_bwd",
                    ts_sh_colors_bwd(f->n, f->sh_degree, f->num_bases, f->means, f->origin,
                                     (f->flags & TS_FRAME_STRIPE) ? nullptr : f->sh_mask, f->v_colors, f->v_colors_dc,
                                     f->num_bases > 1 ? f->v_colors_rest : nullptr, stream)));
    return TS_ENTRY("ts_project_bwd",
                    ts_project_bwd(f->n, f->means, f->scales, f->quats, f->view34, f->projview, &f->cam, 3, f->radii,
                                   f->v_xy, f->v_depth, f->v_conic, nullptr, f->v_means, f->v_scales, f->v_quats,
                                   stream));
}

int ts_frame_bwd_params_adam(const ts_frame* f, const ts_adam* adam, void* stream) {
    TsRange range_("ts_frame_bwd_params_adam");
    if (bad(f) || !adam) return TS_E_BADARG;
    TS_TRY(TS_ENTRY("ts_sh_colors_bwd_adam",
                    ts_sh_colors_bwd_adam(f->n, f->sh_degree, f->num_bases, f->means, f->origin,
                                          (f->flags & TS_FRAME_STRIPE) ? nullptr : f->sh_mask, f->v_colors,
                                          const_cast<float*>(f->colors_dc),
                                          f->num_bases > 1 ? const_cast<float*>(f->colors_rest) : nullptr, adam,
                                          stream)));
    return TS_ENTRY("ts_project_bwd_adam",
                    ts_project_bwd_adam(f->n, const_cast<float*>(f->means), const_cast<float*>(f->scales),
                                        const_cast<float*>(f->quats), f->view34, f->projview, &f->cam, 3, f->radii,
                                        f->v_xy, f->v_depth, f->v_conic, const_cast<float*>(f->opacities), f->v_opacity,
                                        adam, stream));
}


int ts_shard_owner_fwd(const ts_frame* fo, const ts_stripes* stripes, int32_t* route_ws, int32_t* counts,
                       void* stream) {
    return ts_shard_owner_fwd_padded(fo, stripes, nullptr, route_ws, counts, stream);
}

int ts_shard_owner_fwd_padded(const ts_frame* fo, const ts_stripes* stripes, const int32_t* group_base,
                              int32_t* route_ws, int32_t* counts, void* stream) {
    TsRange range_("ts_shard_owner_fwd");
    if (bad(fo) || !stripes) return TS_E_BADARG;
    if (fo->n > 0 && fo->n <= small_n_fused())
        return TS_ENTRY("ts_owner_fwd_fused",
                        ts_shard_owner_fwd_fused(fo->n, fo->sh_degree, fo->num_bases, fo->means, fo->scales, fo->quats,
                                                 fo->view34, fo->projview, &fo->cam, 3, fo->origin, fo->colors_dc,
                                                 fo->num_bases > 1 ? fo->colors_rest : nullptr, fo->opacities,
                                                 fo->channels, TS_RASTER_LOGIT_OPACITY, fo->xys, fo->depths, fo->radii,
                                                 fo->conics, fo->num_tiles_hit, fo->sh_mask, fo->splats, stripes,
                                                 group_base, route_ws, counts, stream));
    TS_TRY(TS_ENTRY("ts_project_fwd",
                    ts_project_fwd(fo->n, fo->means, fo->scales, fo->quats, fo->view34, fo->projview, &fo->cam, 3,
                                   fo->xys, fo->depths, fo->radii, fo->conics, fo->num_tiles_hit, nullptr, stream)));
    TS_TRY(TS_ENTRY("ts_colors_pack_fwd",
                    ts_colors_pack_fwd(fo->n, fo->sh_degree, fo->num_bases, fo->means, fo->origin, fo->colors_dc,
                                       fo->num_bases > 1 ? fo->colors_rest : nullptr, fo->sh_mask, nullptr,
                                       fo->channels, TS_RASTER_LOGIT_OPACITY, fo->xys, fo->radii, fo->conics,
                                       fo->opacities, fo->num_tiles_hit, &fo->cam,
                                       fo->channels == 4 ? fo->depths : nullptr, fo->splats, stream)));
    return TS_ENTRY("ts_route_count",
                    ts_route_count_padded(fo->n, fo->xys, fo->radii, &fo->cam, stripes, group_base, route_ws, counts,
                                          stream));
}

int ts_shard_stripe_fwd_import(const ts_frame* fs, const float* records, void* stream) {
    TsRange range_("ts_shard_stripe_fwd_import");
    if (bad(fs)) return TS_E_BADARG;
    if (fs->n > 0) {
        TS_TRY(TS_ENTRY("ts_import_records",
                        ts_import_records(fs->n, records, &fs->cam, fs->xys, fs->depths, fs->radii, fs->num_tiles_hit,
                                          stream)));
        int32_t* total_dev = fs->total_host ? mapped_pointer(fs->total_host) : nullptr;
        TS_TRY(TS_ENTRY("ts_scan_tiles",
                        ts_scan_tiles(fs->n, fs->num_tiles_hit, fs->cum_tiles_hit, fs->scan_ws, total_dev, stream)));
        if (fs->total_host && !total_dev) {
            const hipError_t e = hipMemcpyAsync(fs->total_host, fs->cum_tiles_hit + (fs->n - 1), sizeof(int32_t),
                                                hipMemcpyDeviceToHost, (hipStream_t)stream);
// ... 89 lines not shown
```

tinysplat_amd/csrc/pack.h:

```cpp
#pragma once

#include <hip/hip_runtime.h>

#include "../../include/tinysplat_hip.h"
#include "splat_math.h"

namespace ts {

struct PackArgs {
    int channels, flags;
    const float* xys;
    const int* radii;
    const float* conics;
    const float* opacity;
    const int* cum_tiles_hit;
    const float* depths;
    float4* splats;
    ts_camera cam;
};

__device__ __forceinline__ void pack_one(const PackArgs& a, int i, float c0, float c1, float c2, float c3) {
    const int r = a.radii[i];
    if (r <= 0) return;
    const float2 xy = reinterpret_cast<const float2*>(a.xys)[i];
    const TileBox b = tile_bbox(xy.x, xy.y, (float)r, a.cam.tile_bounds_x, a.cam.tile_bounds_y,
                                a.cam.tile_row0, a.cam.tile_rows);
    const int w = b.maxx - b.minx, h = b.maxy - b.miny;
    const int cnt = h > 0 ? w * h : 0;
    if (cnt <= 0) return;
    const int excl = a.cum_tiles_hit[i] - cnt;
    const int slot_base = excl - b.miny * w - b.minx;
    float op = a.opacity[i];
    if (a.flags & TS_RASTER_LOGIT_OPACITY) op = 1.0f / (1.0f + expf(-op));
    a.splats[3 * (size_t)i] = make_float4(xy.x, xy.y, op, a.conics[3 * i]);
    a.splats[3 * (size_t)i + 1] = make_float4(a.conics[3 * i + 1], a.conics[3 * i + 2], c0, c1);
    a.splats[3 * (size_t)i + 2] =
        make_float4(c2, c3, __int_as_float(slot_base), __int_as_float(w | (b.minx << 16)));
}

}
```

tinysplat_amd/csrc/project.hip:

```cpp
#include <hip/hip_runtime.h>

#include "../../include/tinysplat_hip.h"
#include "pack.h"
#include "splat_math.h"
#include "adam_math.h"

namespace {

constexpr int kThreads = 256;
#ifndef TS_SH_THREADS_FWD
#define TS_SH_THREADS_FWD 128
#endif
#ifndef TS_SH_THREADS_BWD
#define TS_SH_THREADS_BWD 256
#endif
typedef float f4v __attribute__((ext_vector_type(4)));
__device__ __forceinline__ void store4(float4* p, float a, float b, float c, float d) {
    f4v v = {a, b, c, d};
    __builtin_nontemporal_store(v, reinterpret_cast<f4v*>(p));
}
constexpr int kShThreadsFwd = TS_SH_THREADS_FWD, kShThreadsBwd = TS_SH_THREADS_BWD;
__device__ __forceinline__ float4 load4_stream(const float4* p) {
    const f4v v = __builtin_nontemporal_load(reinterpret_cast<const f4v*>(p));
    return make_float4(v.x, v.y, v.z, v.w);
}

#include "project_inputs.h"

__global__ __launch_bounds__(kThreads) void project_fwd_kernel(
    int n, const float* __restrict__ means3d, const float* __restrict__ scales,
    const float* __restrict__ quats, const float* __restrict__ viewmat,
    const float* __restrict__ projmat, const ts_camera cam, const int flags,
    float* __restrict__ xys, float* __restrict__ depths, int* __restrict__ radii,
    float* __restrict__ conics, int* __restrict__ num_tiles_hit, float* __restrict__ cov3d) {
    const int i = blockIdx.x * kThreads + threadIdx.x;
    if (i >= n) return;
    const ts::Cam C = load_cam(viewmat, projmat, cam);
    const float m[3] = {means3d[3 * i], means3d[3 * i + 1], means3d[3 * i + 2]};
    float s[3] = {scales[3 * i], scales[3 * i + 1], scales[3 * i + 2]};
    const float4 qv = reinterpret_cast<const float4*>(quats)[i];
    float q[4] = {qv.x, qv.y, qv.z, qv.w};
    prep_inputs(flags, s, q, nullptr);
    ts::ProjOut o;
    ts::project_one(C, m, s, q, o);
    reinterpret_cast<float2*>(xys)[i] = make_float2(o.x, o.y);
    depths[i] = o.depth;
    radii[i] = o.radius;
    conics[3 * i] = o.conic[0]; conics[3 * i + 1] = o.conic[1]; conics[3 * i + 2] = o.conic[2];
    num_tiles_hit[i] = o.tiles;
    if (cov3d) {
        float2* c3 = reinterpret_cast<float2*>(cov3d) + 3 * (size_t)i;
        c3[0] = make_float2(o.cov3d[0], o.cov3d[1]);
        c3[1] = make_float2(o.cov3d[2], o.cov3d[3]);
        c3[2] = make_float2(o.cov3d[4], o.cov3d[5]);
    }
}

struct ProjAdam {
    float *means, *scales, *quats, *opacities;
    const float* v_opacity;
    float *m_means, *v_means, *m_scales, *v_scales, *m_quats, *v_quats, *m_opac, *v_opac;
    ts::AdamCoef c_means, c_scales, c_quats, c_opac;
};
template <bool ADAM>
__global__ __launch_bounds__(kThreads) void project_bwd_kernel(
    int n, const float* __restrict__ means3d, const float* __restrict__ scales,
    const float* __restrict__ quats, const float* __restrict__ viewmat,
    const float* __restrict__ projmat, const ts_camera cam, const int flags,
    const int* __restrict__ radii, const float* __restrict__ v_xy, const float* __restrict__ v_depth,
    const float* __restrict__ v_conic, const float* __restrict__ v_cov3d,
    float* __restrict__ v_means3d, float* __restrict__ v_scales, float* __restrict__ v_quats, const ProjAdam ad) {
    const int i = blockIdx.x * kThreads + threadIdx.x;
    if (i >= n) return;
    ts::ProjGrad g;
    for (int k = 0; k < 3; ++k) { g.v_mean[k] = 0.0f; g.v_scale[k] = 0.0f; }
    for (int k = 0; k < 4; ++k) g.v_quat[k] = 0.0f;
    float pm[3] = {0.f, 0.f, 0.f}, ps[3] = {0.f, 0.f, 0.f}, pq[4] = {0.f, 0.f, 0.f, 0.f};
    if (ADAM) {
        pm[0] = means3d[3 * i]; pm[1] = means3d[3 * i + 1]; pm[2] = means3d[3 * i + 2];
        ps[0] = scales[3 * i]; ps[1] = scales[3 * i + 1]; ps[2] = scales[3 * i + 2];
        const float4 qv = reinterpret_cast<const float4*>(quats)[i];
        pq[0] = qv.x; pq[1] = qv.y; pq[2] = qv.z; pq[3] = qv.w;
    }
    if (radii[i] > 0) {
        const ts::Cam C = load_cam(viewmat, projmat, cam);
        const float m[3] = {ADAM ? pm[0] : means3d[3 * i], ADAM ? pm[1] : means3d[3 * i + 1], ADAM ? pm[2] : means3d[3 * i + 2]};
        float s[3] = {ADAM ? ps[0] : scales[3 * i], ADAM ? ps[1] : scales[3 * i + 1], ADAM ? ps[2] : scales[3 * i + 2]};
        float4 qv;
        if (ADAM) qv = make_float4(pq[0], pq[1], pq[2], pq[3]);
        else qv = reinterpret_cast<const float4*>(quats)[i];
        float q[4] = {qv.x, qv.y, qv.z, qv.w};
        float inv_n = 1.0f;
        prep_inputs(flags, s, q, &inv_n);
        const float2 vxy = reinterpret_cast<const float2*>(v_xy)[i];
        const float vx[2] = {vxy.x, vxy.y};
        const float vc[3] = {v_conic[3 * i], v_conic[3 * i + 1], v_conic[3 * i + 2]};
        float vcov[6];
        if (v_cov3d) {
            for (int k = 0; k < 6; ++k) vcov[k] = v_cov3d[6 * (size_t)i + k];
        }
        ts::project_one_vjp(C, m, s, q, vx, v_depth ? v_depth[i] : 0.0f, vc, v_cov3d ? vcov : nullptr, g);
        if (flags & TS_PROJECT_LOG_SCALES) {
            g.v_scale[0] *= s[0]; g.v_scale[1] *= s[1]; g.v_scale[2] *= s[2];
        }
        if (flags & TS_PROJECT_RAW_QUATS) {
            const float dotp = q[0] * g.v_quat[0] + q[1] * g.v_quat[1] + q[2] * g.v_quat[2] +
                               q[3] * g.v_quat[3];
            for (int k = 0; k < 4; ++k) g.v_quat[k] = (g.v_quat[k] - q[k] * dotp) * inv_n;
        }
    }
    if (ADAM) {
        float mo[3], vo[3];
#pragma unroll
        for (int k = 0; k < 3; ++k) { mo[k] = ad.m_means[3 * i + k]; vo[k] = ad.v_means[3 * i + k]; }
#pragma unroll
        for (int k = 0; k < 3; ++k) {
            ts::adam_update(pm[k], g.v_mean[k], mo[k], vo[k], ad.c_means);
            ad.means[3 * i + k] = pm[k]; ad.m_means[3 * i + k] = mo[k]; ad.v_means[3 * i + k] = vo[k];
        }
#pragma unroll
        for (int k = 0; k < 3; ++k) { mo[k] = ad.m_scales[3 * i + k]; vo[k] = ad.v_scales[3 * i + k]; }
#pragma unroll
        for (int k = 0; k < 3; ++k) {
            ts::adam_update(ps[k], g.v_scale[k], mo[k], vo[k], ad.c_scales);
            ad.scales[3 * i + k] = ps[k]; ad.m_scales[3 * i + k] = mo[k]; ad.v_scales[3 * i + k] = vo[k];
        }
        float4 mq = reinterpret_cast<float4*>(ad.m_quats)[i], vq = reinterpret_cast<float4*>(ad.v_quats)[i];
        ts::adam_update(pq[0], g.v_quat[0], mq.x, vq.x, ad.c_quats); ts::adam_update(pq[1], g.v_quat[1], mq.y, vq.y, ad.c_quats);
        ts::adam_update(pq[2], g.v_quat[2], mq.z, vq.z, ad.c_quats); ts::adam_update(pq[3], g.v_quat[3], mq.w, vq.w, ad.c_quats);
        reinterpret_cast<float4*>(ad.quats)[i] = make_float4(pq[0], pq[1], pq[2], pq[3]);
        reinterpret_cast<float4*>(ad.m_quats)[i] = mq;
        reinterpret_cast<float4*>(ad.v_quats)[i] = vq;
        if (ad.opacities) {
            float po = ad.opacities[i], mo1 = ad.m_opac[i], vo1 = ad.v_opac[i];
            ts::adam_update(po, ad.v_opacity[i], mo1, vo1, ad.c_opac);
            ad.opacities[i] = po; ad.m_opac[i] = mo1; ad.v_opac[i] = vo1;
        }
        return;
    }
    v_means3d[3 * i] = g.v_mean[0]; v_means3d[3 * i + 1] = g.v_mean[1];
    v_means3d[3 * i + 2] = g.v_mean[2];
    v_scales[3 * i] = g.v_scale[0]; v_scales[3 * i + 1] = g.v_scale[1];
    v_scales[3 * i + 2] = g.v_scale[2];
    reinterpret_cast<float4*>(v_quats)[i] =
        make_float4(g.v_quat[0], g.v_quat[1], g.v_quat[2], g.v_quat[3]);
}

template <int DEG>
__global__ __launch_bounds__(kThreads) void sh_fwd_kernel(
    int n, int num_bases, const float* __restrict__ viewdirs, const float* __restrict__ coeffs,
    float* __restrict__ colors) {
    constexpr int KA = (DEG + 1) * (DEG + 1);
    constexpr int RS = 3 * KA;
    constexpr int RSP = RS | 1;
    extern __shared__ __align__(16) float lds[];
    const int g0 = blockIdx.x * kThreads;
    const int cnt = min(kThreads, n - g0);
    const int tid = threadIdx.x;
    const size_t row = 3 * (size_t)num_bases;
    const float* src = coeffs + (size_t)g0 * row;
    if (num_bases == KA && cnt == kThreads) {
        const float4* src4 = reinterpret_cast<const float4*>(src);
        constexpr int total4 = kThreads * RS / 4;
        for (int f4 = tid; f4 < total4; f4 += kThreads) {
            const float4 v = src4[f4];
            const int f = 4 * f4;
            const float e[4] = {v.x, v.y, v.z, v.w};
#pragma unroll
            for (int u = 0; u < 4; ++u) {
                const int ff = f + u;
                lds[(ff / RS) * RSP + (ff % RS)] = e[u];
            }
        }
    } else {
        const int total = cnt * RS;
        for (int f = tid; f < total; f += kThreads) {
            const int g = f / RS, j = f % RS;
            lds[g * RSP + j] = src[(size_t)g * row + j];
        }
    }
    __syncthreads();
    if (tid >= cnt) return;
    const int i = g0 + tid;
    float Y[KA];
    ts::sh_basis(DEG, viewdirs[3 * i], viewdirs[3 * i + 1], viewdirs[3 * i + 2], Y);
    const float* r = lds + tid * RSP;
    float c0 = Y[0] * r[0], c1 = Y[0] * r[1], c2 = Y[0] * r[2];
#pragma unroll
    for (int k = 1; k < KA; ++k) {
        c0 = c0 + Y[k] * r[3 * k];
        c1 = c1 + Y[k] * r[3 * k + 1];
        c2 = c2 + Y[k] * r[3 * k + 2];
    }
    colors[3 * i] = c0; colors[3 * i + 1] = c1; colors[3 * i + 2] = c2;
}

template <int DEG>
__global__ __launch_bounds__(kThreads) void sh_bwd_kernel(
    int n, int num_bases, const float* __restrict__ viewdirs, const float* __restrict__ v_colors,
    float* __restrict__ v_coeffs) {
    constexpr int KA = (DEG + 1) * (DEG + 1);
    extern __shared__ __align__(16) float lds[];
    const int RS = 3 * num_bases;
    const int RSP = RS | 1;
    const int g0 = blockIdx.x * kThreads;
    const int cnt = min(kThreads, n - g0);
    const int tid = threadIdx.x;
    if (tid < cnt) {
        const int i = g0 + tid;
        float Y[KA];
        ts::sh_basis(DEG, viewdirs[3 * i], viewdirs[3 * i + 1], viewdirs[3 * i + 2], Y);
        const float v0 = v_colors[3 * i], v1 = v_colors[3 * i + 1], v2 = v_colors[3 * i + 2];
        float* r = lds + tid * RSP;
#pragma unroll
        for (int k = 0; k < KA; ++k) {
            r[3 * k] = Y[k] * v0; r[3 * k + 1] = Y[k] * v1; r[3 * k + 2] = Y[k] * v2;
        }
        for (int j = 3 * KA; j < RS; ++j) r[j] = 0.0f;
    }
    __syncthreads();
    float* dst = v_coeffs + (size_t)g0 * RS;
    const int total = cnt * RS;
    if ((total & 3) == 0) {
        float4* dst4 = reinterpret_cast<float4*>(dst);
        for (int f4 = tid; f4 < total / 4; f4 += kThreads) {
            float e[4];
#pragma unroll
            for (int u = 0; u < 4; ++u) {
                const int ff = 4 * f4 + u;
                e[u] = lds[(ff / RS) * RSP + (ff % RS)];
            }
            dst4[f4] = make_float4(e[0], e[1], e[2], e[3]);
        }
    } else {
        for (int f = tid; f < total; f += kThreads) dst[f] = lds[(f / RS) * RSP + (f % RS)];
    }
}

template <int DEG>
__global__ __launch_bounds__(kShThreadsFwd) void sh_colors_fwd_kernel(
    int n, int num_bases, const float* __restrict__ means, const float* __restrict__ origin,
    const float* __restrict__ dc, const float* __restrict__ rest, float* __restrict__ colors,
    unsigned char* __restrict__ mask, const ts::PackArgs pk) {
    constexpr int KA = (DEG + 1) * (DEG + 1);
    constexpr int RS = 3 * (KA - 1);
    constexpr int RSP = RS | 1;
    extern __shared__ __align__(16) float lds[];
    const int g0 = blockIdx.x * kShThreadsFwd;
    const int cnt = min(kShThreadsFwd, n - g0);
    const int tid = threadIdx.x;
    if (RS > 0) {
        const size_t row = 3 * (size_t)(num_bases - 1);
        const float* src = rest + (size_t)g0 * row;
        if (num_bases == KA && cnt == kShThreadsFwd && ((kShThreadsFwd * RS) & 3) == 0) {
            const float4* src4 = reinterpret_cast<const float4*>(src);
            constexpr int total4 = kShThreadsFwd * RS / 4;
            constexpr int per = (total4 + kShThreadsFwd - 1) / kShThreadsFwd;
            float4 v[per > 0 ? per : 1];
#pragma unroll
            for (int u = 0; u < per; ++u) {
                const int f4 = tid + u * kShThreadsFwd;
                v[u] = f4 < total4 ? load4_stream(src4 + f4) : make_float4(0.f, 0.f, 0.f, 0.f);
            }
#pragma unroll
            for (int u = 0; u < per; ++u) {
                const int f4 = tid + u * kShThreadsFwd;
                if (f4 < total4) {
                    const float e[4] = {v[u].x, v[u].y, v[u].z, v[u].w};
#pragma unroll
                    for (int c = 0; c < 4; ++c) {
                        const int ff = 4 * f4 + c;
                        lds[(ff / RS) * RSP + (ff % RS)] = e[c];
                    }
                }
            }
        } else {
            const int total = cnt * RS;
            for (int f = tid; f < total; f += kShThreadsFwd) {
                const int g = f / RS, j = f % RS;
                lds[g * RSP + j] = src[(size_t)g * row + j];
            }
        }
        __syncthreads();
    }
    if (tid >= cnt) return;
    const int i = g0 + tid;
    float Y[KA];
    ts::sh_basis(DEG, means[3 * i] - origin[0], means[3 * i + 1] - origin[1],
                 means[3 * i + 2] - origin[2], Y);
    float c0 = Y[0] * dc[3 * i], c1 = Y[0] * dc[3 * i + 1], c2 = Y[0] * dc[3 * i + 2];
    const float* r = lds + tid * RSP;
#pragma unroll
    for (int k = 1; k < KA; ++k) {
        c0 = c0 + Y[k] * r[3 * (k - 1)];
        c1 = c1 + Y[k] * r[3 * (k - 1) + 1];
        c2 = c2 + Y[k] * r[3 * (k - 1) + 2];
    }
    c0 = c0 + 0.5f; c1 = c1 + 0.5f; c2 = c2 + 0.5f;
    if (mask) mask[i] = (unsigned char)((c0 >= 0.0f ? 1 : 0) | (c1 >= 0.0f ? 2 : 0) | (c2 >= 0.0f ? 4 : 0));
    c0 = fmaxf(c0, 0.0f); c1 = fmaxf(c1, 0.0f); c2 = fmaxf(c2, 0.0f);
    if (colors) { colors[3 * i] = c0; colors[3 * i + 1] = c1; colors[3 * i + 2] = c2; }
    if (pk.splats) ts::pack_one(pk, i, c0, c1, c2, pk.channels == 4 ? pk.depths[i] : 0.0f);
}

template <int DEG>
__global__ __launch_bounds__(kThreads) void sh_colors_fwd_sparse_kernel(
    int n, int num_bases, const int* __restrict__ live, const float* __restrict__ means,
    const float* __restrict__ origin, const float* __restrict__ dc, const float* __restrict__ rest,
    float* __restrict__ colors, unsigned char* __restrict__ mask, const ts::PackArgs pk) {
    constexpr int KA = (DEG + 1) * (DEG + 1);
    const int i = blockIdx.x * kThreads + threadIdx.x;
    if (i >= n || live[i] == 0) return;
    float Y[KA];
    ts::sh_basis(DEG, means[3 * i] - origin[0], means[3 * i + 1] - origin[1],
                 means[3 * i + 2] - origin[2], Y);
    float c0 = Y[0] * dc[3 * i], c1 = Y[0] * dc[3 * i + 1], c2 = Y[0] * dc[3 * i + 2];
    const float* r = rest + (size_t)i * 3 * (num_bases - 1);
#pragma unroll
    for (int k = 1; k < KA; ++k) {
        c0 = c0 + Y[k] * r[3 * (k - 1)];
        c1 = c1 + Y[k] * r[3 * (k - 1) + 1];
        c2 = c2 + Y[k] * r[3 * (k - 1) + 2];
    }
    c0 = c0 + 0.5f; c1 = c1 + 0.5f; c2 = c2 + 0.5f;
    if (mask) mask[i] = (unsigned char)((c0 >= 0.0f ? 1 : 0) | (c1 >= 0.0f ? 2 : 0) | (c2 >= 0.0f ? 4 : 0));
    c0 = fmaxf(c0, 0.0f); c1 = fmaxf(c1, 0.0f); c2 = fmaxf(c2, 0.0f);
    if (colors) { colors[3 * i] = c0; colors[3 * i + 1] = c1; colors[3 * i + 2] = c2; }
    if (pk.splats) ts::pack_one(pk, i, c0, c1, c2, pk.channels == 4 ? pk.depths[i] : 0.0f);
}

struct ShAdam {
    float *dc, *rest, *m_dc, *v_dc, *m_rest, *v_rest;
    ts::AdamCoef c_dc, c_rest;
};
template <int DEG, bool ADAM>
__global__ __launch_bounds__(kShThreadsBwd) void sh_colors_bwd_kernel(
    int n, int num_bases, const float* __restrict__ means, const float* __restrict__ origin,
    const unsigned char* __restrict__ mask, const float* __restrict__ v_colors,
    float* __restrict__ v_dc, float* __restrict__ v_rest, const ShAdam ad) {
    constexpr int KA = (DEG + 1) * (DEG + 1);
    extern __shared__ __align__(16) float lds[];
    const int RS = 3 * (num_bases - 1);
    const int RSP = RS | 1;
    const int g0 = blockIdx.x * kShThreadsBwd;
    const int cnt = min(kShThreadsBwd, n - g0);
    const int tid = threadIdx.x;
    if (tid < cnt) {
        const int i = g0 + tid;
        float Y[KA];
        ts::sh_basis(DEG, means[3 * i] - origin[0], means[3 * i + 1] - origin[1],
                     means[3 * i + 2] - origin[2], Y);
        const int m = mask ? mask[i] : 7;
        const float v0 = (m & 1) ? v_colors[3 * i] : 0.0f, v1 = (m & 2) ? v_colors[3 * i + 1] : 0.0f,
                    v2 = (m & 4) ? v_colors[3 * i + 2] : 0.0f;
        if (ADAM) {
            const float gd[3] = {Y[0] * v0, Y[0] * v1, Y[0] * v2};
#pragma unroll
            for (int c = 0; c < 3; ++c) {
                float p_ = ad.dc[3 * i + c], m_ = ad.m_dc[3 * i + c], s_ = ad.v_dc[3 * i + c];
                ts::adam_update(p_, gd[c], m_, s_, ad.c_dc);
                ad.dc[3 * i + c] = p_; ad.m_dc[3 * i + c] = m_; ad.v_dc[3 * i + c] = s_;
            }
        } else {
            v_dc[3 * i] = Y[0] * v0; v_dc[3 * i + 1] = Y[0] * v1; v_dc[3 * i + 2] = Y[0] * v2;
        }
        float* r = lds + tid * RSP;
#pragma unroll
        for (int k = 1; k < KA; ++k) {
            r[3 * (k - 1)] = Y[k] * v0; r[3 * (k - 1) + 1] = Y[k] * v1; r[3 * (k - 1) + 2] = Y[k] * v2;
        }
        for (int j = 3 * (KA - 1); j < RS; ++j) r[j] = 0.0f;
    }
    if (RS == 0) return;
    __syncthreads();
    const size_t off = (size_t)g0 * RS;
    float* dst = ADAM ? nullptr : v_rest + off;
    const int total = cnt * RS;
    if ((total & 3) == 0 && ((off) & 3) == 0) {
        float4* dst4 = reinterpret_cast<float4*>(dst);
        for (int f4 = tid; f4 < total / 4; f4 += kShThreadsBwd) {
            float e[4];
#pragma unroll
            for (int u = 0; u < 4; ++u) {
                const int ff = 4 * f4 + u;
                e[u] = lds[(ff / RS) * RSP + (ff % RS)];
            }
            if (ADAM) {
                float4* p4 = reinterpret_cast<float4*>(ad.rest + off) + f4;
                float4* m4 = reinterpret_cast<float4*>(ad.m_rest + off) + f4;
                float4* s4 = reinterpret_cast<float4*>(ad.v_rest + off) + f4;
                float4 pp = *p4, mm = *m4, ss = *s4;
                ts::adam_update(pp.x, e[0], mm.x, ss.x, ad.c_rest); ts::adam_update(pp.y, e[1], mm.y, ss.y, ad.c_rest);
                ts::adam_update(pp.z, e[2], mm.z, ss.z, ad.c_rest); ts::adam_update(pp.w, e[3], mm.w, ss.w, ad.c_rest);
                *p4 = pp; *m4 = mm; *s4 = ss;
            } else {
                store4(dst4 + f4, e[0], e[1], e[2], e[3]);
            }
        }
    } else {
        for (int f = tid; f < total; f += kShThreadsBwd) {
            const float e = lds[(f / RS) * RSP + (f % RS)];
            if (ADAM) {
                float p_ = ad.rest[off + f], m_ = ad.m_rest[off + f], s_ = ad.v_rest[off + f];
                ts::adam_update(p_, e, m_, s_, ad.c_rest);
                ad.rest[off + f] = p_; ad.m_rest[off + f] = m_; ad.v_rest[off + f] = s_;
            } else {
                dst[f] = e;
            }
        }
    }
}

__global__ __launch_bounds__(kThreads) void stream_read_kernel(const float4* __restrict__ src,
                                                               size_t n16, float* __restrict__ sink) {
    constexpr int U = 8;
    const size_t stride = (size_t)gridDim.x * kThreads;
    size_t i = (size_t)blockIdx.x * kThreads + threadIdx.x;
    float4 acc[U];
#pragma unroll
    for (int u = 0; u < U; ++u) acc[u] = make_float4(0.f, 0.f, 0.f, 0.f);
    for (; i + (U - 1) * stride < n16; i += U * stride) {
        float4 v[U];
#pragma unroll
        for (int u = 0; u < U; ++u) {
            const f4v t = __builtin_nontemporal_load(reinterpret_cast<const f4v*>(src + i + u * stride));
            v[u] = make_float4(t.x, t.y, t.z, t.w);
        }
#pragma unroll
        for (int u = 0; u < U; ++u) {
            acc[u].x += v[u].x; acc[u].y += v[u].y; acc[u].z += v[u].z; acc[u].w += v[u].w;
        }
    }
    for (; i < n16; i += stride) {
        const float4 v0 = src[i];
        acc[0].x += v0.x; acc[0].y += v0.y; acc[0].z += v0.z; acc[0].w += v0.w;
    }
    float t = 0.f;
#pragma unroll
    for (int u = 0; u < U; ++u) t += (acc[u].x + acc[u].y) + (acc[u].z + acc[u].w);
    if (t == 123456.789f) sink[0] = t;
}

__global__ __launch_bounds__(kThreads) void gather48_kernel(const float4* __restrict__ records,
                                                            const int* __restrict__ ids, size_t m,
                                                            float* __restrict__ sink) {
    const size_t stride = (size_t)gridDim.x * kThreads;
    float4 a = make_float4(0.f, 0.f, 0.f, 0.f);
    for (size_t j = (size_t)blockIdx.x * kThreads + threadIdx.x; j < m; j += stride) {
        const size_t g = (size_t)ids[j];
        const float4 q0 = records[3 * g], q1 = records[3 * g + 1], q2 = records[3 * g + 2];
        a.x += q0.x + q1.x + q2.x; a.y += q0.y + q1.y + q2.y; a.z += q0.z + q1.z + q2.z; a.w += q0.w + q1.w + q2.w;
    }
    if ((a.x + a.y) + (a.z + a.w) == 123456.789f) sink[0] = a.x;
}

// ... 7 lines not shown

int ts_project_fwd(int32_t n, const float* means3d, const float* scales, const float* quats,
                   const float* viewmat, const float* projmat, const ts_camera* cam,
                   int32_t flags, float* xys, float* depths, int32_t* radii, float* conics,
                   int32_t* num_tiles_hit, float* cov3d, void* stream) {
    if (n < 0 || !cam) return TS_E_BADARG;
    if (n == 0) return 0;
    if (!means3d || !scales || !quats || !viewmat || !projmat || !xys || !depths || !radii ||
        !conics || !num_tiles_hit)
        return TS_E_BADARG;
    const int grid = (n + kThreads - 1) / kThreads;
    hipLaunchKernelGGL(project_fwd_kernel, dim3(grid), dim3(kThreads), 0, (hipStream_t)stream, n,
                       means3d, scales, quats, viewmat, projmat, *cam, (int)flags, xys, depths, radii,
                       conics, num_tiles_hit, cov3d);
    return launch_status();
}

int ts_project_bwd(int32_t n, const float* means3d, const float* scales, const float* quats,
                   const float* viewmat, const float* projmat, const ts_camera* cam,
                   int32_t flags, const int32_t* radii, const float* v_xy, const float* v_depth,
                   const float* v_conic, const float* v_cov3d, float* v_means3d, float* v_scales,
                   float* v_quats, void* stream) {
    if (n < 0 || !cam) return TS_E_BADARG;
    if (n == 0) return 0;
    if (!means3d || !scales || !quats || !viewmat || !projmat || !radii || !v_xy ||
        !v_conic || !v_means3d || !v_scales || !v_quats)
        return TS_E_BADARG;
    const int grid = (n + kThreads - 1) / kThreads;
    hipLaunchKernelGGL(project_bwd_kernel<false>, dim3(grid), dim3(kThreads), 0, (hipStream_t)stream, n,
                       means3d, scales, quats, viewmat, projmat, *cam, (int)flags, radii, v_xy, v_depth,
                       v_conic, v_cov3d, v_means3d, v_scales, v_quats, ProjAdam{});
    return launch_status();
}

static bool adam_group_ok(const ts_adam* a, int k) {
    return a->exp_avg[k] && a->exp_avg_sq[k] && a->step[k] >= 1;
}

int ts_project_bwd_adam(int32_t n, float* means3d, float* scales, float* quats, const float* viewmat,
                        const float* projmat, const ts_camera* cam, int32_t flags, const int32_t* radii,
                        const float* v_xy, const float* v_depth, const float* v_conic, float* opacities,
                        const float* v_opacity, const ts_adam* adam, void* stream) {
    if (n < 0 || !cam || !adam) return TS_E_BADARG;
    if (n == 0) return 0;
    if (!means3d || !scales || !quats || !viewmat || !projmat || !radii || !v_xy || !v_conic) return TS_E_BADARG;
    if (!adam_group_ok(adam, TS_ADAM_MEANS) || !adam_group_ok(adam, TS_ADAM_SCALES) || !adam_group_ok(adam, TS_ADAM_QUATS))
        return TS_E_BADARG;
    if (opacities && (!v_opacity || !adam_group_ok(adam, TS_ADAM_OPACITIES))) return TS_E_BADARG;
    ProjAdam ad{};
    ad.means = means3d; ad.scales = scales; ad.quats = quats; ad.opacities = opacities; ad.v_opacity = v_opacity;
    ad.m_means = adam->exp_avg[TS_ADAM_MEANS]; ad.v_means = adam->exp_avg_sq[TS_ADAM_MEANS];
    ad.m_scales = adam->exp_avg[TS_ADAM_SCALES]; ad.v_scales = adam->exp_avg_sq[TS_ADAM_SCALES];
    ad.m_quats = adam->exp_avg[TS_ADAM_QUATS]; ad.v_quats = adam->exp_avg_sq[TS_ADAM_QUATS];
    ad.m_opac = adam->exp_avg[TS_ADAM_OPACITIES]; ad.v_opac = adam->exp_avg_sq[TS_ADAM_OPACITIES];
    auto coef = [&](int k) { return ts::adam_coef(adam->lr[k], adam->step[k], adam->beta1, adam->beta2, adam->eps); };
    ad.c_means = coef(TS_ADAM_MEANS); ad.c_scales = coef(TS_ADAM_SCALES); ad.c_quats = coef(TS_ADAM_QUATS);
    if (opacities) ad.c_opac = coef(TS_ADAM_OPACITIES);
    const int grid = (n + kThreads - 1) / kThreads;
    hipLaunchKernelGGL(project_bwd_kernel<true>, dim3(grid), dim3(kThreads), 0, (hipStream_t)stream, n,
                       means3d, scales, quats, viewmat, projmat, *cam, (int)flags, radii, v_xy, v_depth,
                       v_conic, (const float*)nullptr, (float*)nullptr, (float*)nullptr, (float*)nullptr, ad);
    return launch_status();
}

static int sh_check(int32_t n, int32_t degree, int32_t num_bases) {
    if (n < 0) return TS_E_BADARG;
    if (num_bases != 1 && num_bases != 4 && num_bases != 9 && num_bases != 16 && num_bases != 25)
        return TS_E_DEGREE;
    if (degree < 0 || degree > 4 || (degree + 1) * (degree + 1) > num_bases) return TS_E_DEGREE;
    return 0;
}

int ts_sh_fwd(int32_t n, int32_t degrees_to_use, int32_t num_bases, const float* viewdirs,
              const float* coeffs, float* colors, void* stream) {
    const int chk = sh_check(n, degrees_to_use, num_bases);
    if (chk) return chk;
    if (n == 0) return 0;
    if (!viewdirs || !coeffs || !colors) return TS_E_BADARG;
    const int grid = (n + kThreads - 1) / kThreads;
    const int ka = (degrees_to_use + 1) * (degrees_to_use + 1);
    const size_t lds = (size_t)kThreads * ((3 * ka) | 1) * sizeof(float);
    hipStream_t s = (hipStream_t)stream;
#define TS_SH_FWD(D)                                                                          \
    hipLaunchKernelGGL(sh_fwd_kernel<D>, dim3(grid), dim3(kThreads), lds, s, n, num_bases,     \
                       viewdirs, coeffs, colors)
    switch (degrees_to_use) {
        case 0: TS_SH_FWD(0); break;
        case 1: TS_SH_FWD(1); break;
        case 2: TS_SH_FWD(2); break;
        case 3: TS_SH_FWD(3); break;
        default: {
            (void)hipFuncSetAttribute(reinterpret_cast<const void*>(&sh_fwd_kernel<4>),
                                hipFuncAttributeMaxDynamicSharedMemorySize, (int)lds);
            TS_SH_FWD(4);
        } break;
    }
#undef TS_SH_FWD
    return launch_status();
}

int ts_sh_bwd(int32_t n, int32_t degrees_to_use, int32_t num_bases, const float* viewdirs,
              const float* v_colors, float* v_coeffs, void* stream) {
    const int chk = sh_check(n, degrees_to_use, num_bases);
    if (chk) return chk;
    if (n == 0) return 0;
    if (!viewdirs || !v_colors || !v_coeffs) return TS_E_BADARG;
    const int grid = (n + kThreads - 1) / kThreads;
    const size_t lds = (size_t)kThreads * ((3 * num_bases) | 1) * sizeof(float);
    hipStream_t s = (hipStream_t)stream;
#define TS_SH_BWD(D)                                                                          \
    do {                                                                                      \
        if (lds > 48 * 1024)                                                                  \
            (void)hipFuncSetAttribute(reinterpret_cast<const void*>(&sh_bwd_kernel<D>),           \
                                hipFuncAttributeMaxDynamicSharedMemorySize, (int)lds);        \
        hipLaunchKernelGGL(sh_bwd_kernel<D>, dim3(grid), dim3(kThreads), lds, s, n, num_bases, \
                           viewdirs, v_colors, v_coeffs);                                     \
    } while (0)
    switch (degrees_to_use) {
        case 0: TS_SH_BWD(0); break;
        case 1: TS_SH_BWD(1); break;
        case 2: TS_SH_BWD(2); break;
        case 3: TS_SH_BWD(3); break;
        default: TS_SH_BWD(4); break;
    }
#undef TS_SH_BWD
    return launch_status();
}

static int launch_colors_fwd(int32_t n, int32_t degrees_to_use, int32_t num_bases, const float* means3d,
                             const float* origin, const float* colors_dc, const float* colors_rest,
                             float* colors, uint8_t* clamp_mask, const int32_t* live, const ts::PackArgs& pk,
                             void* stream) {
    const int chk = sh_check(n, degrees_to_use, num_bases);
    if (chk) return chk;
    if (n == 0) return 0;
    if (!means3d || !origin || !colors_dc || (!colors && !pk.splats) || (num_bases > 1 && !colors_rest))
        return TS_E_BADARG;
    const int grid = (n + kThreads - 1) / kThreads;
    hipStream_t s = (hipStream_t)stream;
    if (live) {
#define TS_SHC_SPARSE(D)                                                                           \
        hipLaunchKernelGGL(sh_colors_fwd_sparse_kernel<D>, dim3(grid), dim3(kThreads), 0, s, n,    \
                           num_bases, live, means3d, origin, colors_dc, colors_rest, colors, clamp_mask, pk)
        switch (degrees_to_use) {
            case 0: TS_SHC_SPARSE(0); break;
            case 1: TS_SHC_SPARSE(1); break;
            case 2: TS_SHC_SPARSE(2); break;
            case 3: TS_SHC_SPARSE(3); break;
            default: TS_SHC_SPARSE(4); break;
        }
#undef TS_SHC_SPARSE
        return launch_status();
    }
    const int ka = (degrees_to_use + 1) * (degrees_to_use + 1);
    const size_t lds = (size_t)kShThreadsFwd * ((3 * (ka - 1)) | 1) * sizeof(float);
    const int grid_d = (n + kShThreadsFwd - 1) / kShThreadsFwd;
#define TS_SHC_FWD(D)                                                                             \
    do {                                                                                          \
        if (lds > 48 * 1024)                                                                      \
            (void)hipFuncSetAttribute(reinterpret_cast<const void*>(&sh_colors_fwd_kernel<D>),    \
                                      hipFuncAttributeMaxDynamicSharedMemorySize, (int)lds);      \
        hipLaunchKernelGGL(sh_colors_fwd_kernel<D>, dim3(grid_d), dim3(kShThreadsFwd), lds, s, n,  \
                           num_bases, means3d, origin, colors_dc, colors_rest, colors, clamp_mask, pk); \
    } while (0)
    switch (degrees_to_use) {
        case 0: TS_SHC_FWD(0); break;
        case 1: TS_SHC_FWD(1); break;
        case 2: TS_SHC_FWD(2); break;
        case 3: TS_SHC_FWD(3); break;
        default: TS_SHC_FWD(4); break;
    }
#undef TS_SHC_FWD
    return launch_status();
}

int ts_sh_colors_fwd(int32_t n, int32_t degrees_to_use, int32_t num_bases, const float* means3d,
                     const float* origin, const float* colors_dc, const float* colors_rest,
                     float* colors, uint8_t* clamp_mask, const int32_t* live, void* stream) {
    ts::PackArgs none;
    none.splats = nullptr;
    if (!colors) return TS_E_BADARG;
    return launch_colors_fwd(n, degrees_to_use, num_bases, means3d, origin, colors_dc, colors_rest, colors,
                             clamp_mask, live, none, stream);
}

int ts_colors_pack_fwd(int32_t n, int32_t degrees_to_use, int32_t num_bases, const float* means3d,
                       const float* origin, const float* colors_dc, const float* colors_rest,
                       uint8_t* clamp_mask, const int32_t* live, int32_t channels, int32_t flags,
                       const float* xys, const int32_t* radii, const float* conics, const float* opacity,
                       const int32_t* cum_tiles_hit, const ts_camera* cam, const float* depths,
                       float* splats, void* stream) {
    if (n < 0 || !cam || (channels != 3 && channels != 4)) return TS_E_BADARG;
    if (n > 0 && (!xys || !radii || !conics || !opacity || !cum_tiles_hit || !splats ||
                  (channels == 4 && !depths)))
        return TS_E_BADARG;
    ts::PackArgs pk;
    pk.channels = channels; pk.flags = (int)flags; pk.xys = xys; pk.radii = radii; pk.conics = conics;
    pk.opacity = opacity; pk.cum_tiles_hit = cum_tiles_hit; pk.depths = depths;
    pk.splats = reinterpret_cast<float4*>(splats); pk.cam = *cam;
    return launch_colors_fwd(n, degrees_to_use, num_bases, means3d, origin, colors_dc, colors_rest, nullptr,
                             clamp_mask, live, pk, stream);
}

static int sh_colors_bwd_launch(int32_t n, int32_t degrees_to_use, int32_t num_bases, const float* means3d,
                                const float* origin, const uint8_t* clamp_mask, const float* v_colors,
                                float* v_colors_dc, float* v_colors_rest, const ShAdam* ad, void* stream) {
    const int grid = (n + kShThreadsBwd - 1) / kShThreadsBwd;
    const size_t lds = (size_t)kShThreadsBwd * ((3 * (num_bases - 1)) | 1) * sizeof(float);
    hipStream_t s = (hipStream_t)stream;
#define TS_SHC_BWD2(D, A)                                                                            \
    do {                                                                                             \
        if (lds > 48 * 1024)                                                                         \
            (void)hipFuncSetAttribute(reinterpret_cast<const void*>(&sh_colors_bwd_kernel<D, A>),    \
                                      hipFuncAttributeMaxDynamicSharedMemorySize, (int)lds);         \
        hipLaunchKernelGGL((sh_colors_bwd_kernel<D, A>), dim3(grid), dim3(kShThreadsBwd), lds, s, n, \
                           num_bases, means3d, origin, clamp_mask, v_colors, v_colors_dc,            \
                           v_colors_rest, ad ? *ad : ShAdam{});                                      \
    } while (0)
#define TS_SHC_BWD(D)                                       \
    do {                                                    \
        if (ad) TS_SHC_BWD2(D, true);                       \
        else TS_SHC_BWD2(D, false);                         \
    } while (0)
    switch (degrees_to_use) {
        case 0: TS_SHC_BWD(0); break;
        case 1: TS_SHC_BWD(1); break;
        case 2: TS_SHC_BWD(2); break;
        case 3: TS_SHC_BWD(3); break;
        default: TS_SHC_BWD(4); break;
    }
#undef TS_SHC_BWD
#undef TS_SHC_BWD2
    return launch_status();
}

int ts_sh_colors_bwd(int32_t n, int32_t degrees_to_use, int32_t num_bases, const float* means3d,
                     const float* origin, const uint8_t* clamp_mask, const float* v_colors,
                     float* v_colors_dc, float* v_colors_rest, void* stream) {
    const int chk = sh_check(n, degrees_to_use, num_bases);
    if (chk) return chk;
    if (n == 0) return 0;
    if (!means3d || !origin || !v_colors || !v_colors_dc || (num_bases > 1 && !v_colors_rest))
        return TS_E_BADARG;
    return sh_colors_bwd_launch(n, degrees_to_use, num_bases, means3d, origin, clamp_mask, v_colors, v_colors_dc,
                                v_colors_rest, nullptr, stream);
}

int ts_sh_colors_bwd_adam(int32_t n, int32_t degrees_to_use, int32_t num_bases, const float* means3d,
                          const float* origin, const uint8_t* clamp_mask, const float* v_colors,
                          float* colors_dc, float* colors_rest, const ts_adam* adam, void* stream) {
    const int chk = sh_check(n, degrees_to_use, num_bases);
    if (chk) return chk;
    if (n == 0) return 0;
    if (!adam || !means3d || !origin || !v_colors || !colors_dc || (num_bases > 1 && !colors_rest)) return TS_E_BADARG;
    if (!adam_group_ok(adam, TS_ADAM_COLORS_DC) || (num_bases > 1 && !adam_group_ok(adam, TS_ADAM_COLORS_REST)))
        return TS_E_BADARG;
    ShAdam ad{};
    ad.dc = colors_dc; ad.rest = colors_rest;
    ad.m_dc = adam->exp_avg[TS_ADAM_COLORS_DC]; ad.v_dc = adam->exp_avg_sq[TS_ADAM_COLORS_DC];
    ad.m_rest = adam->exp_avg[TS_ADAM_COLORS_REST]; ad.v_rest = adam->exp_avg_sq[TS_ADAM_COLORS_REST];
    ad.c_dc = ts::adam_coef(adam->lr[TS_ADAM_COLORS_DC], adam->step[TS_ADAM_COLORS_DC], adam->beta1, adam->beta2, adam->eps);
    if (num_bases > 1)
        ad.c_rest = ts::adam_coef(adam->lr[TS_ADAM_COLORS_REST], adam->step[TS_ADAM_COLORS_REST], adam->beta1, adam->beta2,
                                  adam->eps);
    return sh_colors_bwd_launch(n, degrees_to_use, num_bases, means3d, origin, clamp_mask, v_colors, nullptr, nullptr, &ad,
                                stream);
}

int ts_bench_gather48(const float* records, const int32_t* ids, int64_t m, float* sink, void* stream) {
    if (!records || !ids || !sink || m < 1) return TS_E_BADARG;
    hipLaunchKernelGGL(gather48_kernel, dim3(256 * 8), dim3(kThreads), 0, (hipStream_t)stream,
                       reinterpret_cast<const float4*>(records), ids, (size_t)m, sink);
    return launch_status();
}

int ts_bench_stream_read(const float* src, int64_t n_floats, float* sink, void* stream) {
    if (!src || !sink || n_floats < 4) return TS_E_BADARG;
    const size_t n16 = (size_t)n_floats / 4;
    hipLaunchKernelGGL(stream_read_kernel, dim3(256 * 8), dim3(kThreads), 0, (hipStream_t)stream,
                       reinterpret_cast<const float4*>(src), n16, sink);
    return launch_status();
}

}
```

tinysplat_amd/csrc/splat_math.h:

```cpp
#pragma once

#include <math.h>
#include <stdint.h>

#if defined(__HIPCC__)
#define TS_HD __host__ __device__ __forceinline__
#else
#define TS_HD inline
#endif

namespace ts {

constexpr float kBlur = 0.3f;
#ifndef TS_PIX_OFF
#define TS_PIX_OFF 0.0f
#endif
#ifndef TS_BWD_CLAMP_UPSTREAM
#define TS_BWD_CLAMP_UPSTREAM 0
#endif
#ifndef TS_FOV_CLAMP_BWD_UNGATED
#define TS_FOV_CLAMP_BWD_UNGATED 0
#endif
constexpr float kAlphaMax = 0.999f;
constexpr float kAlphaMaxBwd = TS_BWD_CLAMP_UPSTREAM ? 0.99f : kAlphaMax;
// ... 187 lines not shown
    const float Y00 = X00 * G00 + X01 * G01, Y01 = X00 * G01 + X01 * G11;
    const float Y10 = X01 * G00 + X11 * G01, Y11 = X01 * G01 + X11 * G11;
    const float S00 = -(Y00 * X00 + Y01 * X01);
    const float S01 = -(Y00 * X01 + Y01 * X11);
    const float S11 = -(Y10 * X01 + Y11 * X11);

    const float a0 = S00 * o.t00 + S01 * o.t10, a1 = S00 * o.t01 + S01 * o.t11,
                a2 = S00 * o.t02 + S01 * o.t12;
    const float b0 = S01 * o.t00 + S11 * o.t10, b1 = S01 * o.t01 + S11 * o.t11,
                b2 = S01 * o.t02 + S11 * o.t12;
    float vc00 = o.t00 * a0 + o.t10 * b0, vc01 = o.t00 * a1 + o.t10 * b1,
          vc02 = o.t00 * a2 + o.t10 * b2, vc11 = o.t01 * a1 + o.t11 * b1,
          vc12 = o.t01 * a2 + o.t11 * b2, vc22 = o.t02 * a2 + o.t12 * b2;
    if (v_cov3d) {
        vc00 += v_cov3d[0]; vc01 += 0.5f * v_cov3d[1]; vc02 += 0.5f * v_cov3d[2];
        vc11 += v_cov3d[3]; vc12 += 0.5f * v_cov3d[4]; vc22 += v_cov3d[5];
    }
    const float vt00 = 2.0f * (a0 * o.c00 + a1 * o.c01 + a2 * o.c02);
    const float vt01 = 2.0f * (a0 * o.c01 + a1 * o.c11 + a2 * o.c12);
    const float vt02 = 2.0f * (a0 * o.c02 + a1 * o.c12 + a2 * o.c22);
    const float vt10 = 2.0f * (b0 * o.c00 + b1 * o.c01 + b2 * o.c02);
    const float vt11 = 2.0f * (b0 * o.c01 + b1 * o.c11 + b2 * o.c12);
    const float vt12 = 2.0f * (b0 * o.c02 + b1 * o.c12 + b2 * o.c22);
    const float vj00 = vt00 * V[0] + vt01 * V[1] + vt02 * V[2];
    const float vj02 = vt00 * V[8] + vt01 * V[9] + vt02 * V[10];
    const float vj11 = vt10 * V[4] + vt11 * V[5] + vt12 * V[6];
    const float vj12 = vt10 * V[8] + vt11 * V[9] + vt12 * V[10];
    const float rz3 = o.rz2 * o.rz;
    const float v_tx = -C.fx * o.rz2 * vj02;
    const float v_ty = -C.fy * o.rz2 * vj12;
    float v_pz = -C.fx * o.rz2 * vj00 - C.fy * o.rz2 * vj11
                 + 2.0f * C.fx * o.tx * rz3 * vj02 + 2.0f * C.fy * o.ty * rz3 * vj12;
    float v_px = 0.0f, v_py = 0.0f;
    if (TS_FOV_CLAMP_BWD_UNGATED) {
        v_px = v_tx; v_py = v_ty;
    } else {
        if (o.clamp_x) v_pz += o.sgn_x * v_tx; else v_px = v_tx;
        if (o.clamp_y) v_pz += o.sgn_y * v_ty; else v_py = v_ty;
    }
    v_pz += v_depth;
    vm0 += V[0] * v_px + V[4] * v_py + V[8] * v_pz;
    vm1 += V[1] * v_px + V[5] * v_py + V[9] * v_pz;
    vm2 += V[2] * v_px + V[6] * v_py + V[10] * v_pz;
    g.v_mean[0] = vm0; g.v_mean[1] = vm1; g.v_mean[2] = vm2;

    const float vM00 = 2.0f * (vc00 * o.m00 + vc01 * o.m10 + vc02 * o.m20);
    const float vM01 = 2.0f * (vc00 * o.m01 + vc01 * o.m11 + vc02 * o.m21);
    const float vM02 = 2.0f * (vc00 * o.m02 + vc01 * o.m12 + vc02 * o.m22);
    const float vM10 = 2.0f * (vc01 * o.m00 + vc11 * o.m10 + vc12 * o.m20);
    const float vM11 = 2.0f * (vc01 * o.m01 + vc11 * o.m11 + vc12 * o.m21);
    const float vM12 = 2.0f * (vc01 * o.m02 + vc11 * o.m12 + vc12 * o.m22);
    const float vM20 = 2.0f * (vc02 * o.m00 + vc12 * o.m10 + vc22 * o.m20);
    const float vM21 = 2.0f * (vc02 * o.m01 + vc12 * o.m11 + vc22 * o.m21);
    const float vM22 = 2.0f * (vc02 * o.m02 + vc12 * o.m12 + vc22 * o.m22);
    g.v_scale[0] = C.gs * (o.R.r00 * vM00 + o.R.r10 * vM10 + o.R.r20 * vM20);
    g.v_scale[1] = C.gs * (o.R.r01 * vM01 + o.R.r11 * vM11 + o.R.r21 * vM21);
    g.v_scale[2] = C.gs * (o.R.r02 * vM02 + o.R.r12 * vM12 + o.R.r22 * vM22);
    const float vR00 = vM00 * o.s0, vR01 = vM01 * o.s1, vR02 = vM02 * o.s2;
    const float vR10 = vM10 * o.s0, vR11 = vM11 * o.s1, vR12 = vM12 * o.s2;
    const float vR20 = vM20 * o.s0, vR21 = vM21 * o.s1, vR22 = vM22 * o.s2;
    float inv_n, nq[4];
    quat_to_rot(q[0], q[1], q[2], q[3], &inv_n, nq);
    const float w = nq[0], x = nq[1], y = nq[2], z = nq[3];
    const float gw = 2.0f * (-z * vR01 + y * vR02 + z * vR10 - x * vR12 - y * vR20 + x * vR21);
    const float gx = 2.0f * (y * vR01 + z * vR02 + y * vR10 - 2.0f * x * vR11 - w * vR12
                             + z * vR20 + w * vR21 - 2.0f * x * vR22);
    const float gy = 2.0f * (-2.0f * y * vR00 + x * vR01 + w * vR02 + x * vR10 + z * vR12
                             - w * vR20 + z * vR21 - 2.0f * y * vR22);
    const float gz = 2.0f * (-2.0f * z * vR00 - w * vR01 + x * vR02 + w * vR10 - 2.0f * z * vR11
                             + y * vR12 + x * vR20 + y * vR21);
    const float dotp = w * gw + x * gx + y * gy + z * gz;
    g.v_quat[0] = (gw - w * dotp) * inv_n;
    g.v_quat[1] = (gx - x * dotp) * inv_n;
    g.v_quat[2] = (gy - y * dotp) * inv_n;
    g.v_quat[3] = (gz - z * dotp) * inv_n;
}

TS_HD int sh_num_bases(int degree) {
    return degree == 0 ? 1 : degree == 1 ? 4 : degree == 2 ? 9 : degree == 3 ? 16 : 25;
}

TS_HD void sh_basis(int degree, float dx, float dy, float dz, float* Y) {
    const float n = sqrtf(dx * dx + dy * dy + dz * dz);
    const float x = dx / n, y = dy / n, z = dz / n;
    Y[0] = 0.28209479177387814f;
    if (degree < 1) return;
    Y[1] = -0.4886025119029199f * y;
    Y[2] = 0.4886025119029199f * z;
    Y[3] = -0.4886025119029199f * x;
    if (degree < 2) return;
    const float xx = x * x, yy = y * y, zz = z * z, xy = x * y, yz = y * z, xz = x * z;
    Y[4] = 1.0925484305920792f * xy;
    Y[5] = -1.0925484305920792f * yz;
    Y[6] = 0.31539156525252005f * (2.0f * zz - xx - yy);
    Y[7] = -1.0925484305920792f * xz;
    Y[8] = 0.5462742152960396f * (xx - yy);
    if (degree < 3) return;
    Y[9] = -0.5900435899266435f * y * (3.0f * xx - yy);
    Y[10] = 2.890611442640554f * xy * z;
    Y[11] = -0.4570457994644658f * y * (4.0f * zz - xx - yy);
    Y[12] = 0.3731763325901154f * z * (2.0f * zz - 3.0f * xx - 3.0f * yy);
    Y[13] = -0.4570457994644658f * x * (4.0f * zz - xx - yy);
    Y[14] = 1.445305721320277f * z * (xx - yy);
    Y[15] = -0.5900435899266435f * x * (xx - 3.0f * yy);
    if (degree < 4) return;
    Y[16] = 2.5033429417967046f * xy * (xx - yy);
    Y[17] = -1.7701307697799304f * yz * (3.0f * xx - yy);
    Y[18] = 0.9461746957575601f * xy * (7.0f * zz - 1.0f);
    Y[19] = -0.6690465435572892f * yz * (7.0f * zz - 3.0f);
    Y[20] = 0.10578554691520431f * (zz * (35.0f * zz - 30.0f) + 3.0f);
    Y[21] = -0.6690465435572892f * xz * (7.0f * zz - 3.0f);
    Y[22] = 0.47308734787878004f * (xx - yy) * (7.0f * zz - 1.0f);
    Y[23] = -1.7701307697799304f * xz * (xx - 3.0f * yy);
    Y[24] = 0.6258357354491761f * (xx * (xx - 3.0f * yy) - yy * (3.0f * xx - yy));
}

constexpr float kLog2e = 1.4426950408889634f;
constexpr float kLog2_255 = 7.994353436858858f;

TS_HD float min_form_on_rect(float hA, float B, float hC, float inv2A, float inv2C, float xlo,
                             float xhi, float ylo, float yhi) {
    if (xlo <= 0.0f && xhi >= 0.0f && ylo <= 0.0f && yhi >= 0.0f) return 0.0f;
    float best = 3.0e38f;
#pragma unroll
    for (int e = 0; e < 2; ++e) {
        const float dx = e ? xhi : xlo;
        const float dy = fminf(fmaxf(-B * dx * inv2C, ylo), yhi);
        best = fminf(best, hA * dx * dx + dy * (B * dx + hC * dy));
        const float ey = e ? yhi : ylo;
        const float ex = fminf(fmaxf(-B * ey * inv2A, xlo), xhi);
        best = fminf(best, hC * ey * ey + ex * (B * ey + hA * ex));
    }
    return best;
}

TS_HD bool rect_may_contribute(float hA, float B, float hC, float inv2A, float inv2C, float tau,
                               float gx, float gy, float x0, float x1, float y0, float y1) {
    const float xlo = gx - x1, xhi = gx - x0;
    const float ylo = gy - y1, yhi = gy - y0;
    const float m = min_form_on_rect(hA, B, hC, inv2A, inv2C, xlo, xhi, ylo, yhi);
    const float dxm = fmaxf(fabsf(xlo), fabsf(xhi));
    const float dym = fmaxf(fabsf(ylo), fabsf(yhi));
    const float mag = hA * dxm * dxm + hC * dym * dym + fabsf(B) * dxm * dym;
    return m <= tau + 0.02f + 4.0e-6f * mag;
}

TS_HD float fast_log2(float x) {
#if defined(__HIP_DEVICE_COMPILE__)
    return __log2f(x);
#else
    return log2f(x);
#endif
}

constexpr int kTilePix = 16;
constexpr float kTightEps = 0.02f;
struct TightTest {
    bool cull_all, geometric;
    float gx, gy, hA, B, tau4A, D4, inv2A, dymax, dxext, dy_left;
    TS_HD TightTest(bool tight, float x, float y, float op, float cxx, float cxy, float cyy, float radius) {
        cull_all = false; geometric = false;
        gx = gy = hA = B = tau4A = D4 = inv2A = dymax = dxext = dy_left = 0.0f;
        if (!tight) return;
        gx = x - kPixOff; gy = y - kPixOff;
        hA = 0.5f * kLog2e * cxx; B = kLog2e * cxy;
        const float hC = 0.5f * kLog2e * cyy;
        float tau = fast_log2(op) + kLog2_255;
        if (!(op > 0.0f) || !(tau >= -0.02f)) { cull_all = true; return; }
        D4 = 4.0f * hA * hC - B * B;
        if (!(hA > 0.0f && hC > 0.0f && D4 > 1e-2f * (4.0f * hA * hC))) return;
        const float far = radius + (float)kTilePix;
        tau += 0.02f + 4.0e-6f * (hA + hC + fabsf(B)) * far * far;
        geometric = true;
        inv2A = 0.5f / hA;
        tau4A = 4.0f * hA * tau;
        dymax = sqrtf(tau4A / D4) + kTightEps;
        dxext = sqrtf(4.0f * hC * tau / D4);
        dy_left = B * dxext / (2.0f * hC);
    }
    TS_HD void row_range(int ty, int minx, int maxx, int& lo, int& hi) const {
        lo = minx; hi = maxx;
        if (!geometric) return;
        const float a = fmaxf((float)(ty * kTilePix) - gy - kTightEps, -dymax);
        const float b = fminf((float)(ty * kTilePix + kTilePix - 1) - gy + kTightEps, dymax);
        if (a > b) { hi = lo; return; }
        const float sa = sqrtf(fmaxf(tau4A - D4 * a * a, 0.0f)), sb = sqrtf(fmaxf(tau4A - D4 * b * b, 0.0f));
        float left = fminf((-B * a - sa) * inv2A, (-B * b - sb) * inv2A);
        float right = fmaxf((-B * a + sa) * inv2A, (-B * b + sb) * inv2A);
        if (dy_left >= a && dy_left <= b) left = -dxext;
        if (-dy_left >= a && -dy_left <= b) right = dxext;
        left = fminf(left, right);
        const float xl = gx + left - kTightEps, xr = gx + right + kTightEps;
        const int tlo = (int)ceilf((xl - (float)(kTilePix - 1)) * (1.0f / kTilePix));
        const int thi = (int)floorf(xr * (1.0f / kTilePix)) + 1;
        lo = lo < tlo ? tlo : lo; hi = hi > thi ? thi : hi;
        if (hi < lo) hi = lo;
    }
};

}
```

tinysplat_amd/frame.py:

```python
from __future__ import annotations

import ctypes
import os
import threading
from typing import Optional, Tuple

import torch
import torch.distributed as dist
from torch import Tensor

from ._comm import collective_timer
from . import _lib
from ._lib import TsFrame
from .ops import TileBinning, _camera, _f32c, _need_hip, _stream, _stripe_rows, _tile_bounds, deg_from_sh

TIGHT_BINNING = os.environ.get("TS_TIGHT_BINNING", "1") != "0"

SPLIT_BLOCKS_BELOW = int(os.environ.get("TS_SPLIT_BLOCKS_BELOW", "2400"))

_ls = os.environ.get("TS_LIST_SEGMENTS", "auto")
LIST_SEGMENTS = _ls if _ls == "auto" else max(1, min(8, int(_ls)))
LIST_SEGMENTS_FROM = int(os.environ.get("TS_LIST_SEGMENTS_FROM", "192"))
SEGMENT_ITEMS = int(os.environ.get("TS_SEGMENT_ITEMS", "16384"))


HYBRID_FROM = int(os.environ.get("TS_HYBRID_FROM", "4096"))
HYBRID_SEGS = max(1, min(8, int(os.environ.get("TS_HYBRID_SEGS", "8"))))
HYBRID_WHOLE16 = max(1, min(15, int(os.environ.get("TS_HYBRID_WHOLE16", "13"))))
HYBRID_MID_FROM = int(os.environ.get("TS_HYBRID_MID_FROM", "1537"))
HYBRID_MID_WHOLE16 = max(1, min(15, int(os.environ.get("TS_HYBRID_MID_WHOLE16", "6"))))
HYBRID_MID_COOP16 = max(0, min(15, int(os.environ.get("TS_HYBRID_MID_COOP16", "6"))))
HYBRID_COOP16 = max(0, min(15, int(os.environ.get("TS_HYBRID_COOP16", "3"))))
COOP_SPLIT = os.environ.get("TS_COOP_SPLIT", "1") != "0"


def set_launch_hints(cam, segs: int, w16: int, mode: int, split: bool, skewed: bool = False) -> None:
    cam.hints = (cam.hints & ~0x1FFF00) | (((segs << 8) | (w16 << 12)) if segs > 1 else 0)
    tiles16 = cam.tile_rows * cam.tile_bounds_x
    if mode == 0 and not split and tiles16 >= HYBRID_FROM:
        cam.hints |= (HYBRID_MID_COOP16 if skewed else HYBRID_COOP16) << 16
    elif mode == 0 and not split and tiles16 >= HYBRID_MID_FROM:
        cam.hints |= HYBRID_MID_COOP16 << 16
    if mode == 0 and split and COOP_SPLIT:
        cam.hints |= _lib.HINT_COOP_SPLIT


def _list_segments(tiles16: int, mode: int, split: bool, skewed: bool = False):
    if mode != 0 or tiles16 <= 0:
        return 1, 0
    if not split:
        if HYBRID_SEGS > 1 and tiles16 >= HYBRID_FROM:
            return HYBRID_SEGS, (HYBRID_MID_WHOLE16 if skewed else HYBRID_WHOLE16)
        if HYBRID_SEGS > 1 and tiles16 >= HYBRID_MID_FROM:
            return HYBRID_SEGS, HYBRID_MID_WHOLE16
        return 1, 0
    if LIST_SEGMENTS != "auto":
        return int(LIST_SEGMENTS), 0
    return max(2, min(8, SEGMENT_ITEMS // tiles16)), 0


last_segments = {}


def segments_for_count(cam, segs: int, total: int) -> int:
    if segs > 1 and total >= LIST_SEGMENTS_FROM * cam.tile_rows * cam.tile_bounds_x:
        return segs
    cam.hints &= ~0xFF00
    return 1


def backward_segments(cam, segs: int, total: int, dev_index: int = 0) -> int:
    segs = segments_for_count(cam, segs, total)
    last_segments[dev_index] = segs
    return segs

_wt = os.environ.get("TS_WIDE_TILES", "auto")
WIDE_TILES = _wt if _wt == "auto" else int(_wt)
WIDE_LISTS_FROM = int(os.environ.get("TS_WIDE_LISTS_FROM", "2300"))
BALANCED_WALK_FROM = float(os.environ.get("TS_BALANCED_WALK_FROM", "10"))
_pairs_per_tile = {}


MANY_TILES_FROM = int(os.environ.get("TS_MANY_TILES_FROM", "20000"))
LONG_LIST = int(os.environ.get("TS_LONG_LIST", "2048"))
SKEW_FROM = float(os.environ.get("TS_SKEW_FROM", "4"))
_stats_mode = {}
_longest_list = {}


def _list_mode(dev_index: int, tiles16: int) -> int:
    if WIDE_TILES != "auto":
        return int(WIDE_TILES)
    prev = _pairs_per_tile.get(dev_index)
    if prev is None:
        return 2 if tiles16 >= MANY_TILES_FROM else 0
    if prev >= WIDE_LISTS_FROM:
        return 2
    st = _longest_list.get(dev_index)
    if tiles16 >= MANY_TILES_FROM and st is not None:
        longest, mode = st
        return 2 if longest < (2 * LONG_LIST if mode == 2 else LONG_LIST) else 0
    return 0


def _skewed(dev_index: int, mode: int) -> bool:
    st, prev = _longest_list.get(dev_index), _pairs_per_tile.get(dev_index)
    if WIDE_TILES != "auto" or mode != 0 or st is None or prev is None or st[1] != 0:
        return False
    return st[0] >= SKEW_FROM * max(prev, 1.0)

last_binning = {}

TRACE = None


def _mark(label):
    if TRACE is not None:
        import time
        TRACE.append((label, time.perf_counter()))


_layouts = {}
_pinned_total = {}
_row_flags = {}
_row_flags_lock = threading.Lock()
_row_flags_tick = [0]

FLAG_GENERATIONS = os.environ.get("TS_FLAG_GENERATIONS", "1") != "0"


FLAGS_SHRINK_AFTER = 256


def row_flags_for(dev: torch.device, rows: int):
    if not FLAG_GENERATIONS:
        return torch.empty((rows,), dtype=torch.uint8, device=dev), 0
    key = (dev.index, _stream(dev))
    with _row_flags_lock:
        slot = _row_flags.get(key)
        if slot is not None and slot[0].numel() > 8 * max(rows, 1 << 20):
            slot[2] += 1
            if slot[2] >= FLAGS_SHRINK_AFTER:
                slot = None
        elif slot is not None:
            slot[2] = 0
        if slot is None or slot[0].numel() < rows:
            if key not in _row_flags and len(_row_flags) >= 32:
                _row_flags.pop(min(_row_flags, key=lambda k_: _row_flags[k_][3]))
            slot = _row_flags[key] = [torch.zeros((int(rows * 1.25) + 4096,), dtype=torch.uint8, device=dev), 0, 0, 0]
        _row_flags_tick[0] += 1
        slot[3] = _row_flags_tick[0]
        slot[1] += 1
        if slot[1] > 255:
            slot[0].zero_()
            slot[1] = 1
        return slot[0], slot[1]

_bg_cache = {}

STRIPE_SPARSE = os.environ.get("TS_STRIPE_SPARSE", "1") != "0"

TWO_HOP_SCATTER = os.environ.get("TS_TWO_HOP_SCATTER", "1") != "0"
INLINE_SORT = os.environ.get("TS_INLINE_SORT", "1") != "0"

DIRECT_GRADS = os.environ.get("TS_DIRECT_GRADS", "1") != "0"

SURVIVORS = os.environ.get("TS_SURVIVORS", "1") != "0"

CAPACITY_ALLOC = os.environ.get("TS_CAPACITY_ALLOC", "0") != "0"
CAPACITY_GROWTH = 1.25
_capacity = {}

COUNT_WAIT = os.environ.get("TS_COUNT_WAIT", "spin")
_SPIN_LIMIT = 50_000_000


def alloc_quantum(count: int) -> int:
    count = max(int(count), 1)
    if count <= 65536:
        return 65536
    g = 1 << (count.bit_length() - 4)
    return (count + g - 1) // g * g


def _total_slot(dev: torch.device):
    slot = _pinned_total.get(dev.index)
    if slot is None:
        slot = (torch.zeros((4,), dtype=torch.int32, pin_memory=True), torch.cuda.Event(), threading.Lock())
        _pinned_total[dev.index] = slot
    return slot


class _Frame:
    __slots__ = ("fr", "cam", "n", "nb", "ch", "w", "h", "num_tiles", "total", "split", "segs", "keep",
                 "wf", "tile_bins", "ids", "bucket_ids", "out_img", "out_depth", "planes", "xys", "radii", "nth", "cum",
                 "inputs", "bg")


def _forward(means, scales, quats, opacities, colors_dc, colors_rest, view34, projview, origin, background,
             fx, fy, width, height, sh_degree, with_depth, tile_rows, keep: bool, planes: bool = False) -> _Frame:
    _mark("fwd:enter")
    dev = _need_hip(means, scales, quats, opacities, colors_dc, colors_rest, view34, projview, origin, background)
    n = means.shape[0]
    nb = colors_rest.shape[1] + 1
    if sh_degree < 0 or sh_degree > deg_from_sh(nb):
        raise ValueError("sh_degree exceeds the stored coefficients")
    means, scales, quats = _f32c(means), _f32c(scales), _f32c(quats)
    opacities, colors_dc, colors_rest = _f32c(opacities), _f32c(colors_dc), _f32c(colors_rest)
    view34, projview, origin = _f32c(view34), _f32c(projview), _f32c(origin)
    w, h = int(width), int(height)
    cam = _camera(fx, fy, w / 2, h / 2, h, w, _tile_bounds(h, w), 1.0, tile_rows=tile_rows)
    slot_ = _pinned_total.get(dev.index)
    if slot_ is not None and dev.index in _stats_mode:
        _longest_list[dev.index] = (int(ctypes.c_int32.from_address(slot_[0].data_ptr() + 4).value), _stats_mode[dev.index])
    mode = _list_mode(dev.index, cam.tile_rows * cam.tile_bounds_x)
    cam.wide_tiles = 1 if mode else 0
    prev_i = _pairs_per_tile.get(dev.index)
    if prev_i is not None and n > 0 and prev_i * cam.tile_rows * cam.tile_bounds_x >= BALANCED_WALK_FROM * n:
        cam.hints = _lib.HINT_BALANCED_WALK
    ch = 4 if with_depth else 3
    if with_depth:
        key = (background.data_ptr(), background._version, dev.index)
        hit = _bg_cache.get(key)
        if hit is None:
            if len(_bg_cache) > 16:
                _bg_cache.clear()
            hit = _bg_cache[key] = (_f32c(torch.cat([background, background[:1]])), background)
        bg = hit[0]
    else:
        bg = _f32c(background)
    lib = _lib.load()
    s = _stream(dev)
    F = _Frame()
    F.cam, F.n, F.nb, F.ch, F.w, F.h, F.keep = cam, n, nb, ch, w, h, keep
    F.inputs = (means, scales, quats, opacities, colors_dc, colors_rest, view34, projview, origin)
    F.bg = bg
    num_tiles = int(lib.ts_num_tiles(ctypes.byref(cam)))
    F.num_tiles = num_tiles
    F.split = 0 < cam.tile_rows * cam.tile_bounds_x <= SPLIT_BLOCKS_BELOW
    rows = _stripe_rows(cam)
    m = max(n, 1)
    skewed = _skewed(dev.index, mode)
    segs, w16 = _list_segments(cam.tile_rows * cam.tile_bounds_x, mode, F.split, skewed) if keep else (1, 0)
    set_launch_hints(cam, segs, w16, mode, F.split, skewed)
    F.segs = segs
    _mark("fwd:inputs checked")
    cur = torch.cuda.current_device()
    if cur != dev.index:
        torch.cuda.set_device(dev)
    try:
        f32 = dict(dtype=torch.float32, device=dev)
        i32 = dict(dtype=torch.int32, device=dev)
        px = rows * w
        lkey = (n, num_tiles, w, rows, ch, keep, cam.hints & 0xFFFF00, cam.wide_tiles, cam.tile_rows, cam.tile_row0, cam.tile_bounds_x, cam.img_height)
        lay = _layouts.get(lkey)
        if lay is None:
            nscan = int(lib.ts_scan_ws_ints(n))
            nbin = int(lib.ts_bin_ws_ints(n, num_tiles))
            fin_floats = int(lib.ts_final_floats(ctypes.byref(cam), ch)) if keep else px
            sizes = [48 * m, 8 * m, 12 * m, 0, 4 * m, 4 * m, 4 * m, 4 * m, 4 * nscan, 4 * nbin,
                     8 * max(num_tiles, 1)] + ([m, 4 * fin_floats, 4 * px, px] if keep else [])
            offs, off = [], 0
            for sz in sizes:
                offs.append(off)
                off += (sz + 255) & ~255
            if len(_layouts) > 64:
                _layouts.clear()
            lay = _layouts[lkey] = (offs, off)
        offs, off = lay
        _mark("fwd:sizes")
        F.wf = torch.empty((off,), dtype=torch.uint8, device=dev)
        _mark("fwd:workspace allocated")
        base = F.wf.data_ptr()
        ptr = [base + o for o in offs]
        F.planes = bool(planes and with_depth)
        F.out_img = torch.empty((rows, w, 3 if F.planes else ch), **f32)
        F.out_depth = torch.empty((rows, w), **f32) if F.planes else None
        _mark("fwd:image allocated")

        def view(k, dtype, count, shape):
            return F.wf[offs[k]:offs[k] + count * dtype.itemsize].view(dtype).view(shape)
        F.xys = view(1, torch.float32, 2 * n, (n, 2))
        F.radii = view(5, torch.int32, n, (n,))
        F.nth = view(6, torch.int32, n, (n,))
        F.cum = view(7, torch.int32, n, (n,))
        F.tile_bins = view(10, torch.int32, 2 * max(num_tiles, 1), (max(num_tiles, 1), 2))
        host, event, count_lock = _total_slot(dev)
        fr = TsFrame()
        fr.n, fr.num_bases, fr.sh_degree, fr.channels = n, nb, int(sh_degree), ch
        stripe = STRIPE_SPARSE and cam.tile_rows < cam.tile_bounds_y
        full = cam.tile_rows == cam.tile_bounds_y
        fr.flags = ((1 if TIGHT_BINNING else 0) | (2 if F.split else 0) | (8 if mode == 2 else 0) | (16 if stripe else 0)
                    | (0 if TWO_HOP_SCATTER else 32) | (64 if F.planes else 0) | (0 if INLINE_SORT else 128)
                    | (256 if full else 0))
        surv = SURVIVORS and keep and full and mode == 0 and not F.split and INLINE_SORT
        if surv:
            fr.flags |= 512
        if full:
            _stats_mode[dev.index] = mode
        fr.cam = cam
        fr.means, fr.scales, fr.quats, fr.opacities = means.data_ptr(), scales.data_ptr(), quats.data_ptr(), opacities.data_ptr()
        fr.colors_dc, fr.colors_rest = colors_dc.data_ptr(), colors_rest.data_ptr()
        fr.view34, fr.projview, fr.origin, fr.background = view34.data_ptr(), projview.data_ptr(), origin.data_ptr(), bg.data_ptr()
        fr.splats, fr.xys, fr.conics, fr.depths = ptr[0], ptr[1], ptr[2], ptr[4]
        fr.radii, fr.num_tiles_hit, fr.cum_tiles_hit, fr.scan_ws = ptr[5], ptr[6], ptr[7], ptr[8]
        fr.bin_ws, fr.tile_bins = ptr[9], ptr[10]
        fr.total_host = host.data_ptr()
        fr.out_img = F.out_img.data_ptr()
        if F.planes:
            fr.out_depth = F.out_depth.data_ptr()
        if keep:
            fr.sh_mask, fr.final_Ts, fr.final_index, fr.clamp_mask = ptr[11], ptr[12], ptr[13], ptr[14]
        F.fr = fr
        _mark("fwd:allocated + struct")
        spin = COUNT_WAIT == "spin" and n > 0
        cap_key = (dev.index, n, w, h, cam.tile_row0, cam.tile_rows)
        est = _capacity.get(cap_key) if (CAPACITY_ALLOC and n > 0) else None

        def lists(size):
            cap = alloc_quantum(size)
            counts = (8 * num_tiles + 63) // 64 * 64 if surv else 0
            F.bucket_ids = torch.empty(((3 * cap + counts) if surv else 2 * cap,), **i32)
            fr.bucket_ids, fr.gaussian_ids_sorted = F.bucket_ids.data_ptr(), F.bucket_ids.data_ptr() + 4 * cap
            if surv:
                fr.survivors = F.bucket_ids.data_ptr() + 8 * cap
            return cap

        def prepare():
            _lib.check(lib.ts_frame_fwd_prepare(ctypes.byref(fr), s), "ts_frame_fwd_prepare")

        def composite():
            _lib.check(lib.ts_frame_fwd_composite(ctypes.byref(fr), s), "ts_frame_fwd_composite")

        count_lock.acquire()
        issued = consumed = False
        try:
            if spin:
                word = ctypes.c_int32.from_address(host.data_ptr())
                word.value = -(1 << 31)
            _lib.check(lib.ts_frame_fwd_project(ctypes.byref(fr), s), "ts_frame_fwd_project")
            issued = n > 0
            _mark("fwd:call project")
            event.record()
            cap = None
            if est is not None:
                cap = lists(est)
                fr.capacity, fr.num_intersects = cap, cap
                prepare()
                composite()
            else:
                fr.capacity = -1
                prepare()
            _mark("fwd:call prepare")
            total = 0
            if n > 0:
                if spin:
                    k = 0
                    while word.value == -(1 << 31):
                        k += 1
                        if k > _SPIN_LIMIT:
                            event.synchronize()
                            break
                    total = int(word.value)
                else:
                    event.synchronize()
                    total = int(host[0])
            consumed = True
        finally:
            if issued and not consumed:
                try:
                    event.synchronize()
                except Exception:
                    pass
            count_lock.release()
        if total < 0:
            raise OverflowError("more than 2^31-1 tile intersections: num_tiles_hit overflows its "
                                "int32 prefix sum (gsplat's cum_tiles_hit is int32 as well)")
        _mark("fwd:waited for count")
        F.total = total
        _pairs_per_tile[dev.index] = total / max(1, cam.tile_rows * cam.tile_bounds_x)
        if n > 0 and CAPACITY_ALLOC:
            if len(_capacity) > 64:
                _capacity.clear()
            _capacity[cap_key] = int(total * CAPACITY_GROWTH) + 4096
        if cap is None or total > cap:
            redo = cap is not None
            cap = lists(total)
            _mark("fwd:lists allocated")
            fr.capacity, fr.num_intersects = -1, total
            F.segs = segments_for_count(fr.cam, F.segs, total)
            if redo:
                prepare()
            composite()
            _mark("fwd:composite enqueued")
        else:
            fr.num_intersects = total
        F.ids = F.bucket_ids[cap:cap + total]
        _mark("fwd:call composite")
    finally:
        if cur != dev.index:
            torch.cuda.set_device(cur)
    b = TileBinning()
    b.cam, b.n, b.num_tiles, b.num_intersects = cam, n, num_tiles, total
    b.tile_bins, b.gaussian_ids_sorted, b.cum_tiles_hit, b.num_tiles_hit = F.tile_bins[:num_tiles], F.ids, F.cum, F.nth
    last_binning[dev.index] = b
    _mark("fwd:exit")
    return F


class _AdamHook:
    opt = None


_adam_hook = _AdamHook()


class fused_adam:
    def __init__(self, optimizer):
        self.optimizer = optimizer

    def __enter__(self):
        self.prev = getattr(_adam_hook, "opt", None)
        _adam_hook.opt = self.optimizer
        return self

    def __exit__(self, *exc):
        _adam_hook.opt = self.prev
        return False


class _RenderFrame(torch.autograd.Function):
    @staticmethod
    def forward(ctx, means, scales, quats, opacities, colors_dc, colors_rest, view34, projview,
                origin, background, fx, fy, width, height, sh_degree, with_depth, tile_rows, group, planes=False):
        F = _forward(means, scales, quats, opacities, colors_dc, colors_rest, view34, projview, origin,
                     background, fx, fy, width, height, sh_degree, with_depth, tile_rows, keep=True, planes=planes)
        ctx.frame, ctx.group = F, group
        ctx.opacity_shape = opacities.shape
        ctx.rest_shape = colors_rest.shape
        xys, radii = F.xys, F.radii
        ctx.xys_out = xys
        ctx.mark_non_differentiable(xys, radii)
        ctx.set_materialize_grads(False)
        out, F.out_img = F.out_img, None
        depth, F.out_depth = F.out_depth, None
        return out, depth, xys, radii

    @staticmethod
    def backward(ctx, v_img, v_depth_img, _v_xys, _v_radii):
        _mark("bwd:enter")
        F = ctx.frame
        if F is None:
# ... 102 lines not shown
```

Before: 2019000 billion Gaussians*pixels/s.

## Fuse SH color evaluation into binning count, scan and offset launches

Adds fused kernels in which some workgroups run the bin-count, column-scan or tile-offsets role and the rest evaluate SH colors and pack splat records, so the separate color pass overlaps the small, under-occupied binning launches. The count role reads conics and opacities directly instead of packed splat records, because the records are written concurrently. The color work is divided among the three launches by an env-configurable split; with the default split every color block lands in the tile-offsets launch. This risks occupancy changes from the shared launch bounds and LDS sizing, and adds complexity in keeping the roles ordered.

Result: no change. 2032000 billion Gaussians*pixels/s, median of 5 (+0.7%).

```diff
diff --git a/include/tinysplat_hip.h b/include/tinysplat_hip.h
--- a/include/tinysplat_hip.h
+++ b/include/tinysplat_hip.h
@@ -150,6 +150,7 @@
 #define TS_FRAME_SEPARATE_SORT 128
 #define TS_FRAME_STRIPE 16
 #define TS_FRAME_SURVIVORS 512
+#define TS_FRAME_FUSED_COLORS 1024
 typedef struct ts_frame {
     int32_t n, num_bases, sh_degree, channels, flags;
     int32_t flag_gen;
@@ -175,6 +176,7 @@
     float* out_depth;
     const float* v_out_depth;
     int32_t* survivors;
+    int32_t fused_a, fused_c;
 } ts_frame;
 int32_t ts_frame_struct_bytes(void);
 int ts_frame_fwd_project(const ts_frame* f, void* stream);
@@ -182,6 +184,12 @@
 int ts_frame_fwd_composite(const ts_frame* f, void* stream);
 int ts_frame_bwd_composite(const ts_frame* f, void* stream);
 int ts_frame_bwd_params(const ts_frame* f, void* stream);
+#define TS_FUSED_COUNT 0
+#define TS_FUSED_COLUMN_SCAN 1
+#define TS_FUSED_TILE_OFFSETS 2
+int32_t ts_frame_fused_colors_ok(const ts_frame* f);
+int ts_frame_fused_colors(const ts_frame* f, int32_t role, int32_t first, int32_t end, int32_t* longest_list,
+                          void* stream);
 
 typedef void (*ts_entry_probe)(const char* entry, int32_t end, void* user);
 int ts_set_entry_probe(ts_entry_probe fn, void* user);
diff --git a/tinysplat_amd/_lib.py b/tinysplat_amd/_lib.py
--- a/tinysplat_amd/_lib.py
+++ b/tinysplat_amd/_lib.py
@@ -48,7 +48,8 @@
                     "v_out_img", "partials", "row_flags",
                     "v_xy", "v_conic", "v_colors", "v_depth", "v_opacity",
                     "v_means", "v_scales", "v_quats", "v_colors_dc", "v_colors_rest",
-                    "out_depth", "v_out_depth", "survivors")])
+                    "out_depth", "v_out_depth", "survivors")]
+                + [("fused_a", c_int32), ("fused_c", c_int32)])
 
 
 _FRAME = POINTER(TsFrame)
@@ -157,6 +158,8 @@
     "ts_frame_struct_bytes": (c_int32, []),
     "ts_frame_fwd_project": (c_int32, [_FRAME, _P]),
     "ts_frame_fwd_prepare": (c_int32, [_FRAME, _P]),
+    "ts_frame_fused_colors_ok": (c_int32, [_FRAME]),
+    "ts_frame_fused_colors": (c_int32, [_FRAME, c_int32, c_int32, c_int32, _P, _P]),
     "ts_frame_fwd_composite": (c_int32, [_FRAME, _P]),
     "ts_frame_bwd_composite": (c_int32, [_FRAME, _P]),
     "ts_frame_bwd_params": (c_int32, [_FRAME, _P]),
diff --git a/tinysplat_amd/csrc/binning.hip b/tinysplat_amd/csrc/binning.hip
--- a/tinysplat_amd/csrc/binning.hip
+++ b/tinysplat_amd/csrc/binning.hip
@@ -1,6 +1,7 @@
 #include <hip/hip_runtime.h>
 
 #include "../../include/tinysplat_hip.h"
+#include "colors_stage.h"
 #include "pack.h"
 #include "splat_math.h"
 
@@ -128,14 +129,19 @@
 #define TS_BIN_PRE 2
 #endif
 constexpr int kBinPre = TS_BIN_PRE;
-template <typename Emit>
+struct TightArrays {
+    const float* conics;
+    const float* opacity;
+    int logit;
+};
+template <bool ARRAYS = false, typename Emit>
 __device__ __forceinline__ void walk_chunk(int g0, int g1, const float* __restrict__ xys,
                                            const int* __restrict__ radii,
                                            const float4* __restrict__ splats, const ts_camera& cam,
-                                           Emit emit) {
+                                           Emit emit, const TightArrays src = TightArrays{nullptr, nullptr, 0}) {
     const int ws = cam.wide_tiles ? 1 : 0;
     const int tbx = (cam.tile_bounds_x + ws) >> ws;
-    const bool tight_lists = splats != nullptr;
+    const bool tight_lists = ARRAYS ? src.conics != nullptr : splats != nullptr;
     for (int base = g0 + threadIdx.x; base < g1; base += kBinPre * kBinThreads) {
         int r[kBinPre];
         float2 xy[kBinPre];
@@ -152,12 +158,18 @@
             q0[u] = q1[u] = make_float4(0.f, 0.f, 0.f, 0.f);
             if (r[u] > 0) {
                 xy[u] = reinterpret_cast<const float2*>(xys)[i];
-                if (tight_lists) { q0[u] = splats[3 * (size_t)i]; q1[u] = splats[3 * (size_t)i + 1]; }
+                if (ARRAYS) {
+                    if (tight_lists) {
+                        q0[u] = make_float4(xy[u].x, xy[u].y, src.opacity[i], src.conics[3 * i]);
+                        q1[u].x = src.conics[3 * i + 1]; q1[u].y = src.conics[3 * i + 2];
+                    }
+                } else if (tight_lists) { q0[u] = splats[3 * (size_t)i]; q1[u] = splats[3 * (size_t)i + 1]; }
             }
         }
 #pragma unroll
         for (int u = 0; u < kBinPre; ++u) {
             if (r[u] <= 0) continue;
+            if (ARRAYS && tight_lists) q0[u].z = ts::record_opacity(q0[u].z, src.logit != 0);
             const ts::TileBox b = ts::tile_bbox(xy[u].x, xy[u].y, (float)r[u], cam.tile_bounds_x,
                                                 cam.tile_bounds_y, cam.tile_row0, cam.tile_rows);
             if (b.maxy <= b.miny || b.maxx <= b.minx) continue;
@@ -262,75 +274,92 @@
     }
 }
 
+template <bool BAL, bool ARRAYS = false>
+__device__ __forceinline__ void bin_count_block(
+    int bx, int by, int* __restrict__ hist, int n, int chunk, const float* __restrict__ xys,
+    const int* __restrict__ radii, const float4* __restrict__ splats, const ts_camera& cam, int num_tiles,
+    int window, int* __restrict__ counts, const TightArrays src = TightArrays{nullptr, nullptr, 0}) {
+    const int t0 = by * window;
+    const int tw = min(num_tiles - t0, window);
+    for (int j = threadIdx.x; j < tw; j += kBinThreads) hist[j] = 0;
+    __syncthreads();
+    const int g0 = bx * chunk, g1 = min(n, g0 + chunk);
+    auto emit = [&](int t, int) {
+        t -= t0;
+        if ((unsigned)t < (unsigned)tw) atomicAdd(&hist[t], 1);
+    };
+    if (BAL) walk_chunk_balanced(g0, g1, xys, radii, splats, cam, emit);
+    else walk_chunk<ARRAYS>(g0, g1, xys, radii, splats, cam, emit, src);
+    __syncthreads();
+    int* dst = counts + (size_t)bx * num_tiles + t0;
+    for (int j = threadIdx.x; j < tw; j += kBinThreads) dst[j] = hist[j];
+}
+
 template <bool BAL>
 __global__ __launch_bounds__(kBinThreads) void bin_count_kernel(
     int n, int chunk, const float* __restrict__ xys, const int* __restrict__ radii,
     const float4* __restrict__ splats, const ts_camera cam, int num_tiles, int window,
     int* __restrict__ counts) {
     extern __shared__ int hist[];
-    const int t0 = blockIdx.y * window;
-    const int tw = min(num_tiles - t0, window);
-    for (int j = threadIdx.x; j < tw; j += kBinThreads) hist[j] = 0;
-    __syncthreads();
-    const int g0 = blockIdx.x * chunk, g1 = min(n, g0 + chunk);
-    auto emit = [&](int t, int) {
-        t -= t0;
-        if ((unsigned)t < (unsigned)tw) atomicAdd(&hist[t], 1);
-    };
-    if (BAL) walk_chunk_balanced(g0, g1, xys, radii, splats, cam, emit);
-    else walk_chunk(g0, g1, xys, radii, splats, cam, emit);
-    __syncthreads();
-    int* dst = counts + (size_t)blockIdx.x * num_tiles + t0;
-    for (int j = threadIdx.x; j < tw; j += kBinThreads) dst[j] = hist[j];
+    bin_count_block<BAL>(blockIdx.x, blockIdx.y, hist, n, chunk, xys, radii, splats, cam, num_tiles, window, counts);
 }
 
 constexpr int kScanGroups = 16;
 
 constexpr int kColTiles = 64;
 constexpr int kColPer = (kBinMaxChunks + kScanGroups - 1) / kScanGroups;
+__device__ __forceinline__ void column_scan_block(int bx, int num_tiles, int chunks, int per_group,
+                                                  int* __restrict__ counts, int* __restrict__ tile_total) {
+    __shared__ int gsum[kScanGroups][kColTiles];
+    const int tl = threadIdx.x & (kColTiles - 1), g = threadIdx.x / kColTiles;
+    const int t = bx * kColTiles + tl;
+    const int b0 = g * per_group, b1 = min(chunks, b0 + per_group);
+    int c[kColPer];
+    int sum = 0;
+    if (t < num_tiles) {
+#pragma unroll
+        for (int j = 0; j < kColPer; ++j) c[j] = (b0 + j < b1) ? counts[(size_t)(b0 + j) * num_tiles + t] : 0;
+#pragma unroll
+        for (int j = 0; j < kColPer; ++j) {
+            const int v = c[j];
+            c[j] = sum;
+            sum += v;
+        }
+    }
+    gsum[g][tl] = sum;
+    __syncthreads();
+    if (t >= num_tiles) return;
+    int base = 0, tot = 0;
+#pragma unroll
+    for (int q = 0; q < kScanGroups; ++q) {
+        const int v = gsum[q][tl];
+        if (q < g) base += v;
+        tot += v;
+    }
+#pragma unroll
+    for (int j = 0; j < kColPer; ++j)
+        if (b0 + j < b1) counts[(size_t)(b0 + j) * num_tiles + t] = base + c[j];
+    if (g == 0) tile_total[t] = tot;
+}
 __global__ __launch_bounds__(kColTiles * kScanGroups) void column_scan_kernel(int num_tiles, int chunks,
                                                                               int per_group,
                                                                               int* __restrict__ counts,
                                                                               int* __restrict__ tile_total) {
-    __shared__ int gsum[kScanGroups][kColTiles];
-    const int tl = threadIdx.x & (kColTiles - 1), g = threadIdx.x / kColTiles;
-    const int t = blockIdx.x * kColTiles + tl;
-    const int b0 = g * per_group, b1 = min(chunks, b0 + per_group);
-    int c[kColPer];
-    int sum = 0;
-    if (t < num_tiles) {
-#pragma unroll
-        for (int j = 0; j < kColPer; ++j) c[j] = (b0 + j < b1) ? counts[(size_t)(b0 + j) * num_tiles + t] : 0;
-#pragma unroll
-        for (int j = 0; j < kColPer; ++j) {
-            const int v = c[j];
-            c[j] = sum;
-            sum += v;
-        }
-    }
-    gsum[g][tl] = sum;
-    __syncthreads();
-    if (t >= num_tiles) return;
-    int base = 0, tot = 0;
-#pragma unroll
-    for (int q = 0; q < kScanGroups; ++q) {
-        const int v = gsum[q][tl];
-        if (q < g) base += v;
-        tot += v;
-    }
-#pragma unroll
-    for (int j = 0; j < kColPer; ++j)
-        if (b0 + j < b1) counts[(size_t)(b0 + j) * num_tiles + t] = base + c[j];
-    if (g == 0) tile_total[t] = tot;
+    column_scan_block(blockIdx.x, num_tiles, chunks, per_group, counts, tile_total);
 }
 
 constexpr int kOffsetsThreads = 1024;
-__global__ __launch_bounds__(kOffsetsThreads) void tile_offsets_kernel(int num_tiles,
-                                                                       int* __restrict__ tile_total,
-                                                                       int* __restrict__ tile_bins,
-                                                                       int* __restrict__ spare,
-                                                                       const int* __restrict__ total_ptr,
-                                                                       long long capacity, int* __restrict__ longest_out) {
+struct OffsetsArgs {
+    int num_tiles;
+    int *tile_total, *tile_bins, *spare;
+    const int* total_ptr;
+    long long capacity;
+    int* longest_out;
+};
+__device__ __forceinline__ void tile_offsets_block(int num_tiles, int* __restrict__ tile_total,
+                                                   int* __restrict__ tile_bins, int* __restrict__ spare,
+                                                   const int* __restrict__ total_ptr, long long capacity,
+                                                   int* __restrict__ longest_out) {
     constexpr int kPer = 8;
     __shared__ int carry, over, longest;
     int my_longest = 0;
@@ -381,6 +410,50 @@
         if (threadIdx.x == 0) *longest_out = longest;
     }
 }
+__global__ __launch_bounds__(kOffsetsThreads) void tile_offsets_kernel(const OffsetsArgs o) {
+    tile_offsets_block(o.num_tiles, o.tile_total, o.tile_bins, o.spare, o.total_ptr, o.capacity, o.longest_out);
+}
+
+constexpr int kFusedWavesPerSimd = 8;
+struct CountArgs {
+    int n, chunk, num_tiles, window;
+    const float* xys;
+    const int* radii;
+    int* counts;
+    TightArrays src;
+    ts_camera cam;
+};
+template <int DEG>
+__global__ __launch_bounds__(kBinThreads, kFusedWavesPerSimd) void bin_count_kernel_colors(const CountArgs c, int role_blocks, int first,
+                                                                      int end, const ts::ColorsArgs a) {
+    extern __shared__ __align__(16) int smem[];
+    if ((int)blockIdx.x < role_blocks)
+        bin_count_block<false, true>(blockIdx.x, 0, smem, c.n, c.chunk, c.xys, c.radii, nullptr, c.cam, c.num_tiles,
+                                     c.window, c.counts, c.src);
+    else
+        ts::colors_role<DEG>(a, first, end, blockIdx.x - role_blocks, reinterpret_cast<float*>(smem));
+}
+template <int DEG>
+__global__ __launch_bounds__(kBinThreads, kFusedWavesPerSimd) void column_scan_kernel_colors(int num_tiles, int chunks, int per_group,
+                                                                         int* __restrict__ counts,
+                                                                         int* __restrict__ tile_total, int role_blocks,
+                                                                         int first, int end, const ts::ColorsArgs a) {
+    extern __shared__ __align__(16) int smem[];
+    if ((int)blockIdx.x < role_blocks) column_scan_block(blockIdx.x, num_tiles, chunks, per_group, counts, tile_total);
+    else ts::colors_role<DEG>(a, first, end, blockIdx.x - role_blocks, reinterpret_cast<float*>(smem));
+}
+template <int DEG>
+__global__ __launch_bounds__(kBinThreads, kFusedWavesPerSimd) void tile_offsets_kernel_colors(const OffsetsArgs o, int first, int end,
+                                                                          const ts::ColorsArgs a) {
+    extern __shared__ __align__(16) int smem[];
+    if (blockIdx.x == 0)
+        tile_offsets_block(o.num_tiles, o.tile_total, o.tile_bins, o.spare, o.total_ptr, o.capacity, o.longest_out);
+    else
+        ts::colors_role<DEG>(a, first, end, blockIdx.x - 1, reinterpret_cast<float*>(smem));
+}
+static_assert(kBinThreads == ts::kColorsRoleThreads && kColTiles * kScanGroups == kBinThreads &&
+                  kOffsetsThreads == kBinThreads,
+              "a launch has one block size: every role of the fused launches is a 1024-thread workgroup");
 
 __global__ __launch_bounds__(kBinThreads) void bin_scatter_kernel(
     int n, int chunk, const float* __restrict__ xys,
@@ -831,9 +904,95 @@
     hipStream_t s = (hipStream_t)stream;
     hipLaunchKernelGGL(column_scan_kernel, dim3((num_tiles + kColTiles - 1) / kColTiles),
                        dim3(kColTiles * kScanGroups), 0, s, num_tiles, chunks, per_group, bin_ws, tile_total);
-    hipLaunchKernelGGL(tile_offsets_kernel, dim3(1), dim3(kOffsetsThreads), 0, s, num_tiles, tile_total,
-                       tile_bins, bin_ws + (ts_bin_ws_ints(n, num_tiles) - 1),
-                       (cum_tiles_hit && n > 0) ? cum_tiles_hit + (n - 1) : nullptr, (long long)capacity, longest_list);
+    const OffsetsArgs o{num_tiles, tile_total, tile_bins, bin_ws + (ts_bin_ws_ints(n, num_tiles) - 1),
+                        (cum_tiles_hit && n > 0) ? cum_tiles_hit + (n - 1) : nullptr, (long long)capacity, longest_list};
+    hipLaunchKernelGGL(tile_offsets_kernel, dim3(1), dim3(kOffsetsThreads), 0, s, o);
+    return launch_status();
+}
+
+constexpr size_t kFusedLdsMax = 80 * 1024;
+
+int32_t ts_frame_fused_colors_ok(const ts_frame* f) {
+    if (!f || f->n <= 0 || f->n >= (1 << 30) || f->num_bases < 1 || f->sh_degree < 0) return 0;
+    if (f->sh_degree > 3) return 0;
+    if ((f->flags & TS_FRAME_STRIPE) || f->cam.wide_tiles) return 0;
+    if ((f->sh_degree + 1) * (f->sh_degree + 1) > f->num_bases) return 0;
+    const int nt = ts_num_tiles(&f->cam);
+    if (nt <= 0) return 0;
+    const int window = bin_window_tiles(f->n, nt);
+    return window >= nt && (size_t)window * sizeof(int) <= kFusedLdsMax;
+}
+
+int ts_frame_fused_colors(const ts_frame* f, int32_t role, int32_t first, int32_t end, int32_t* longest_list,
+                          void* stream) {
+    if (!ts_frame_fused_colors_ok(f) || role < TS_FUSED_COUNT || role > TS_FUSED_TILE_OFFSETS || first < 0 ||
+        end < first || end > f->n)
+        return TS_E_BADARG;
+    if (!f->xys || !f->radii || !f->conics || !f->opacities || !f->cum_tiles_hit || !f->splats || !f->bin_ws ||
+        !f->tile_bins || !f->means || !f->origin || !f->colors_dc || (f->num_bases > 1 && !f->colors_rest) ||
+        (f->channels != 3 && f->channels != 4) || (f->channels == 4 && !f->depths))
+        return TS_E_BADARG;
+    const int n = f->n, nt = ts_num_tiles(&f->cam);
+    const int chunks = bin_num_chunks(n);
+    hipStream_t s = (hipStream_t)stream;
+    ts::ColorsArgs a;
+    a.num_bases = f->num_bases; a.means = f->means; a.origin = f->origin; a.dc = f->colors_dc;
+    a.rest = f->num_bases > 1 ? f->colors_rest : nullptr; a.colors = nullptr; a.mask = f->sh_mask;
+    a.pk.channels = f->channels; a.pk.flags = TS_RASTER_LOGIT_OPACITY; a.pk.xys = f->xys; a.pk.radii = f->radii;
+    a.pk.conics = f->conics; a.pk.opacity = f->opacities; a.pk.cum_tiles_hit = f->cum_tiles_hit;
+    a.pk.depths = f->channels == 4 ? f->depths : nullptr; a.pk.splats = reinterpret_cast<float4*>(f->splats);
+    a.pk.cam = f->cam;
+    const int cblocks = ts::colors_role_blocks(first, end);
+    size_t clds = 0;
+    if (cblocks > 0) switch (f->sh_degree) {
+        case 0: clds = ts::colors_role_lds<0>(); break;
+        case 1: clds = ts::colors_role_lds<1>(); break;
+        case 2: clds = ts::colors_role_lds<2>(); break;
+        default: clds = ts::colors_role_lds<3>(); break;
+    }
+#define TS_FUSED_LAUNCH(KERNEL, GRID, LDS, ...)                                                                  \
+    do {                                                                                                         \
+        const size_t lds_ = (LDS);                                                                               \
+        if (lds_ > 48 * 1024)                                                                                    \
+            (void)hipFuncSetAttribute(reinterpret_cast<const void*>(&KERNEL),                                    \
+                                      hipFuncAttributeMaxDynamicSharedMemorySize, (int)lds_);                    \
+        hipLaunchKernelGGL(KERNEL, dim3(GRID), dim3(kBinThreads), lds_, s, __VA_ARGS__);                         \
+    } while (0)
+#define TS_FUSED_BY_DEGREE(KERNEL, GRID, LDS, ...)                                       \
+    do {                                                                                 \
+        switch (f->sh_degree) {                                                          \
+            case 0: TS_FUSED_LAUNCH(KERNEL<0>, GRID, LDS, __VA_ARGS__); break;           \
+            case 1: TS_FUSED_LAUNCH(KERNEL<1>, GRID, LDS, __VA_ARGS__); break;           \
+            case 2: TS_FUSED_LAUNCH(KERNEL<2>, GRID, LDS, __VA_ARGS__); break;           \
+            default: TS_FUSED_LAUNCH(KERNEL<3>, GRID, LDS, __VA_ARGS__); break;          \
+        }                                                                                \
+    } while (0)
+    if (role == TS_FUSED_COUNT) {
+        CountArgs c;
+        c.n = n; c.chunk = (n + chunks - 1) / chunks; c.num_tiles = nt; c.window = bin_window_tiles(n, nt);
+        c.xys = f->xys; c.radii = f->radii; c.counts = f->bin_ws; c.cam = f->cam;
+        c.src = (f->flags & TS_FRAME_TIGHT) ? TightArrays{f->conics, f->opacities, 1} : TightArrays{nullptr, nullptr, 0};
+        const size_t hist = (size_t)c.window * sizeof(int);
+        TS_FUSED_BY_DEGREE(bin_count_kernel_colors, chunks + cblocks, hist > clds ? hist : clds, c, chunks, first, end,
+                           a);
+    } else if (role == TS_FUSED_COLUMN_SCAN) {
+        int* tile_total = f->bin_ws + (size_t)chunks * nt;
+        const int per_group = (chunks + kScanGroups - 1) / kScanGroups;
+        const int sblocks = (nt + kColTiles - 1) / kColTiles;
+        if (cblocks == 0)
+            hipLaunchKernelGGL(column_scan_kernel, dim3(sblocks), dim3(kBinThreads), 0, s, nt, chunks, per_group,
+                               f->bin_ws, tile_total);
+        else
+            TS_FUSED_BY_DEGREE(column_scan_kernel_colors, sblocks + cblocks, clds, nt, chunks, per_group, f->bin_ws,
+                           tile_total, sblocks, first, end, a);
+    } else {
+        const OffsetsArgs o{nt, f->bin_ws + (size_t)chunks * nt, f->tile_bins, f->bin_ws + (ts_bin_ws_ints(n, nt) - 1),
+                            f->cum_tiles_hit + (n - 1), (long long)f->capacity, longest_list};
+        if (cblocks == 0) hipLaunchKernelGGL(tile_offsets_kernel, dim3(1), dim3(kBinThreads), 0, s, o);
+        else TS_FUSED_BY_DEGREE(tile_offsets_kernel_colors, 1 + cblocks, clds, o, first, end, a);
+    }
+#undef TS_FUSED_BY_DEGREE
+#undef TS_FUSED_LAUNCH
     return launch_status();
 }
 
diff --git a/tinysplat_amd/csrc/colors_stage.h b/tinysplat_amd/csrc/colors_stage.h
--- /dev/null
+++ b/tinysplat_amd/csrc/colors_stage.h
@@ -0,0 +1,121 @@
+#pragma once
+
+#include <hip/hip_runtime.h>
+
+#include "pack.h"
+#include "splat_math.h"
+
+namespace ts {
+
+typedef float stream_f4 __attribute__((ext_vector_type(4)));
+__device__ __forceinline__ float4 load4_stream(const float4* p) {
+    const stream_f4 v = __builtin_nontemporal_load(reinterpret_cast<const stream_f4*>(p));
+    return make_float4(v.x, v.y, v.z, v.w);
+}
+
+struct ColorsArgs {
+    int num_bases;
+    const float *means, *origin, *dc, *rest;
+    float* colors;
+    unsigned char* mask;
+    PackArgs pk;
+};
+
+template <int DEG, int THREADS, int ROWS>
+struct ColorsBatch {
+    static constexpr int KA = (DEG + 1) * (DEG + 1);
+    static constexpr int RS = 3 * (KA - 1);
+    static constexpr int RSP = RS | 1;
+    static constexpr int kTotal4 = ROWS * RS / 4;
+    static constexpr int kPer = (kTotal4 + THREADS - 1) / THREADS;
+    static constexpr size_t kLdsBytes = RS > 0 ? (size_t)ROWS * RSP * sizeof(float) : 0;
+    float4 v[kPer > 0 ? kPer : 1];
+
+    static __device__ __forceinline__ bool whole(const ColorsArgs& a, int g0, int cnt) {
+        return RS > 0 && a.num_bases == KA && cnt == ROWS && ((ROWS * RS) & 3) == 0 && (((size_t)g0 * RS) & 3) == 0;
+    }
+    __device__ __forceinline__ void fetch(const ColorsArgs& a, int g0, int cnt) {
+        if (!whole(a, g0, cnt)) return;
+        const float4* src4 = reinterpret_cast<const float4*>(a.rest + (size_t)g0 * RS);
+#pragma unroll
+        for (int u = 0; u < kPer; ++u) {
+            const int f4 = threadIdx.x + u * THREADS;
+            v[u] = f4 < kTotal4 ? load4_stream(src4 + f4) : make_float4(0.f, 0.f, 0.f, 0.f);
+        }
+    }
+    __device__ __forceinline__ void stage(const ColorsArgs& a, int g0, int cnt, float* __restrict__ lds) const {
+        if (RS == 0) return;
+        if (whole(a, g0, cnt)) {
+#pragma unroll
+            for (int u = 0; u < kPer; ++u) {
+                const int f4 = threadIdx.x + u * THREADS;
+                if (f4 < kTotal4) {
+                    const float e[4] = {v[u].x, v[u].y, v[u].z, v[u].w};
+#pragma unroll
+                    for (int c = 0; c < 4; ++c) {
+                        const int ff = 4 * f4 + c;
+                        lds[(ff / RS) * RSP + (ff % RS)] = e[c];
+                    }
+                }
+            }
+        } else {
+            const size_t row = 3 * (size_t)(a.num_bases - 1);
+            const float* src = a.rest + (size_t)g0 * row;
+            const int total = cnt * RS;
+            for (int f = threadIdx.x; f < total; f += THREADS) {
+                const int g = f / RS, j = f % RS;
+                lds[g * RSP + j] = src[(size_t)g * row + j];
+            }
+        }
+    }
+    static __device__ __forceinline__ void evaluate(const ColorsArgs& a, int g0, int cnt, const float* __restrict__ lds) {
+        const int tid = threadIdx.x;
+        if (tid >= cnt) return;
+        const int i = g0 + tid;
+        float Y[KA];
+        sh_basis(DEG, a.means[3 * i] - a.origin[0], a.means[3 * i + 1] - a.origin[1],
+                 a.means[3 * i + 2] - a.origin[2], Y);
+        float c0 = Y[0] * a.dc[3 * i], c1 = Y[0] * a.dc[3 * i + 1], c2 = Y[0] * a.dc[3 * i + 2];
+        const float* r = lds + tid * RSP;
+#pragma unroll
+        for (int k = 1; k < KA; ++k) {
+            c0 = c0 + Y[k] * r[3 * (k - 1)];
+            c1 = c1 + Y[k] * r[3 * (k - 1) + 1];
+            c2 = c2 + Y[k] * r[3 * (k - 1) + 2];
+        }
+        c0 = c0 + 0.5f; c1 = c1 + 0.5f; c2 = c2 + 0.5f;
+        if (a.mask) a.mask[i] = (unsigned char)((c0 >= 0.0f ? 1 : 0) | (c1 >= 0.0f ? 2 : 0) | (c2 >= 0.0f ? 4 : 0));
+        c0 = fmaxf(c0, 0.0f); c1 = fmaxf(c1, 0.0f); c2 = fmaxf(c2, 0.0f);
+        if (a.colors) { a.colors[3 * i] = c0; a.colors[3 * i + 1] = c1; a.colors[3 * i + 2] = c2; }
+        if (a.pk.splats) pack_one(a.pk, i, c0, c1, c2, a.pk.channels == 4 ? a.pk.depths[i] : 0.0f);
+    }
+};
+
+constexpr int kColorsRoleThreads = 1024;
+constexpr int kColorsRows = 256;
+constexpr int kColorsSpan = 4 * kColorsRows;
+template <int DEG>
+constexpr size_t colors_role_lds() { return ColorsBatch<DEG, kColorsRoleThreads, kColorsRows>::kLdsBytes; }
+inline int colors_role_blocks(int first, int end) { return end > first ? (end - first + kColorsSpan - 1) / kColorsSpan : 0; }
+
+template <int DEG>
+__device__ __forceinline__ void colors_role(const ColorsArgs& a, int first, int end, int block, float* __restrict__ lds) {
+    using Batch = ColorsBatch<DEG, kColorsRoleThreads, kColorsRows>;
+    int g = first + block * kColorsSpan;
+    if (g >= end) return;
+    const int stop = min(end, g + kColorsSpan);
+    Batch b;
+    b.fetch(a, g, min(kColorsRows, stop - g));
+    for (; g < stop; g += kColorsRows) {
+        const int cnt = min(kColorsRows, stop - g);
+        if (Batch::RS > 0) {
+            b.stage(a, g, cnt, lds);
+            __syncthreads();
+            if (g + kColorsRows < stop) b.fetch(a, g + kColorsRows, min(kColorsRows, stop - g - kColorsRows));
+        }
+        Batch::evaluate(a, g, cnt, lds);
+        if (Batch::RS > 0) __syncthreads();
+    }
+}
+
+}
diff --git a/tinysplat_amd/csrc/frame.hip b/tinysplat_amd/csrc/frame.hip
--- a/tinysplat_amd/csrc/frame.hip
+++ b/tinysplat_amd/csrc/frame.hip
@@ -123,6 +123,18 @@
 int ts_frame_fwd_prepare(const ts_frame* f, void* stream) {
     TsRange range_("ts_frame_fwd_prepare");
     if (bad(f)) return TS_E_BADARG;
+    if ((f->flags & TS_FRAME_FUSED_COLORS) && ts_frame_fused_colors_ok(f)) {
+        if (f->fused_a < 0 || f->fused_c < f->fused_a || f->fused_c > f->n) return TS_E_BADARG;
+        int32_t* longest = nullptr;
+        if ((f->flags & TS_FRAME_LIST_STATS) && f->total_host) {
+            int32_t* dev = mapped_pointer(f->total_host);
+            if (dev) longest = dev + 1;
+        }
+        TS_TRY(TS_ENTRY("ts_bin_count", ts_frame_fused_colors(f, TS_FUSED_COUNT, 0, f->fused_a, nullptr, stream)));
+        TsEntry offsets_("ts_tile_offsets");
+        TS_TRY(ts_frame_fused_colors(f, TS_FUSED_COLUMN_SCAN, f->fused_a, f->fused_c, nullptr, stream));
+        return ts_frame_fused_colors(f, TS_FUSED_TILE_OFFSETS, f->fused_c, f->n, longest, stream);
+    }
     TS_TRY(TS_ENTRY("ts_colors_pack_fwd",
                     ts_colors_pack_fwd(f->n, f->sh_degree, f->num_bases, f->means, f->origin, f->colors_dc,
                                        f->num_bases > 1 ? f->colors_rest : nullptr, f->sh_mask,
diff --git a/tinysplat_amd/csrc/pack.h b/tinysplat_amd/csrc/pack.h
--- a/tinysplat_amd/csrc/pack.h
+++ b/tinysplat_amd/csrc/pack.h
@@ -30,8 +30,7 @@
     if (cnt <= 0) return;
     const int excl = a.cum_tiles_hit[i] - cnt;
     const int slot_base = excl - b.miny * w - b.minx;
-    float op = a.opacity[i];
-    if (a.flags & TS_RASTER_LOGIT_OPACITY) op = 1.0f / (1.0f + expf(-op));
+    const float op = record_opacity(a.opacity[i], (a.flags & TS_RASTER_LOGIT_OPACITY) != 0);
     a.splats[3 * (size_t)i] = make_float4(xy.x, xy.y, op, a.conics[3 * i]);
     a.splats[3 * (size_t)i + 1] = make_float4(a.conics[3 * i + 1], a.conics[3 * i + 2], c0, c1);
     a.splats[3 * (size_t)i + 2] =
diff --git a/tinysplat_amd/csrc/project.hip b/tinysplat_amd/csrc/project.hip
--- a/tinysplat_amd/csrc/project.hip
+++ b/tinysplat_amd/csrc/project.hip
@@ -1,6 +1,7 @@
 #include <hip/hip_runtime.h>
 
 #include "../../include/tinysplat_hip.h"
+#include "colors_stage.h"
 #include "pack.h"
 #include "splat_math.h"
 #include "adam_math.h"
@@ -20,10 +21,6 @@
     __builtin_nontemporal_store(v, reinterpret_cast<f4v*>(p));
 }
 constexpr int kShThreadsFwd = TS_SH_THREADS_FWD, kShThreadsBwd = TS_SH_THREADS_BWD;
-__device__ __forceinline__ float4 load4_stream(const float4* p) {
-    const f4v v = __builtin_nontemporal_load(reinterpret_cast<const f4v*>(p));
-    return make_float4(v.x, v.y, v.z, v.w);
-}
 
 #include "project_inputs.h"
 
@@ -238,69 +235,18 @@
 }
 
 template <int DEG>
-__global__ __launch_bounds__(kShThreadsFwd) void sh_colors_fwd_kernel(
-    int n, int num_bases, const float* __restrict__ means, const float* __restrict__ origin,
-    const float* __restrict__ dc, const float* __restrict__ rest, float* __restrict__ colors,
-    unsigned char* __restrict__ mask, const ts::PackArgs pk) {
-    constexpr int KA = (DEG + 1) * (DEG + 1);
-    constexpr int RS = 3 * (KA - 1);
-    constexpr int RSP = RS | 1;
+__global__ __launch_bounds__(kShThreadsFwd) void sh_colors_fwd_kernel(int n, const ts::ColorsArgs a) {
+    using Batch = ts::ColorsBatch<DEG, kShThreadsFwd, kShThreadsFwd>;
     extern __shared__ __align__(16) float lds[];
     const int g0 = blockIdx.x * kShThreadsFwd;
     const int cnt = min(kShThreadsFwd, n - g0);
-    const int tid = threadIdx.x;
-    if (RS > 0) {
-        const size_t row = 3 * (size_t)(num_bases - 1);
-        const float* src = rest + (size_t)g0 * row;
-        if (num_bases == KA && cnt == kShThreadsFwd && ((kShThreadsFwd * RS) & 3) == 0) {
-            const float4* src4 = reinterpret_cast<const float4*>(src);
-            constexpr int total4 = kShThreadsFwd * RS / 4;
-            constexpr int per = (total4 + kShThreadsFwd - 1) / kShThreadsFwd;
-            float4 v[per > 0 ? per : 1];
-#pragma unroll
-            for (int u = 0; u < per; ++u) {
-                const int f4 = tid + u * kShThreadsFwd;
-                v[u] = f4 < total4 ? load4_stream(src4 + f4) : make_float4(0.f, 0.f, 0.f, 0.f);
-            }
-#pragma unroll
-            for (int u = 0; u < per; ++u) {
-                const int f4 = tid + u * kShThreadsFwd;
-                if (f4 < total4) {
-                    const float e[4] = {v[u].x, v[u].y, v[u].z, v[u].w};
-#pragma unroll
-                    for (int c = 0; c < 4; ++c) {
-                        const int ff = 4 * f4 + c;
-                        lds[(ff / RS) * RSP + (ff % RS)] = e[c];
-                    }
-                }
-            }
-        } else {
-            const int total = cnt * RS;
-            for (int f = tid; f < total; f += kShThreadsFwd) {
-                const int g = f / RS, j = f % RS;
-                lds[g * RSP + j] = src[(size_t)g * row + j];
-            }
-        }
+    if (Batch::RS > 0) {
+        Batch b;
+        b.fetch(a, g0, cnt);
+        b.stage(a, g0, cnt, lds);
         __syncthreads();
     }
-    if (tid >= cnt) return;
-    const int i = g0 + tid;
-    float Y[KA];
-    ts::sh_basis(DEG, means[3 * i] - origin[0], means[3 * i + 1] - origin[1],
-                 means[3 * i + 2] - origin[2], Y);
-    float c0 = Y[0] * dc[3 * i], c1 = Y[0] * dc[3 * i + 1], c2 = Y[0] * dc[3 * i + 2];
-    const float* r = lds + tid * RSP;
-#pragma unroll
-    for (int k = 1; k < KA; ++k) {
-        c0 = c0 + Y[k] * r[3 * (k - 1)];
-        c1 = c1 + Y[k] * r[3 * (k - 1) + 1];
-        c2 = c2 + Y[k] * r[3 * (k - 1) + 2];
-    }
-    c0 = c0 + 0.5f; c1 = c1 + 0.5f; c2 = c2 + 0.5f;
-    if (mask) mask[i] = (unsigned char)((c0 >= 0.0f ? 1 : 0) | (c1 >= 0.0f ? 2 : 0) | (c2 >= 0.0f ? 4 : 0));
-    c0 = fmaxf(c0, 0.0f); c1 = fmaxf(c1, 0.0f); c2 = fmaxf(c2, 0.0f);
-    if (colors) { colors[3 * i] = c0; colors[3 * i + 1] = c1; colors[3 * i + 2] = c2; }
-    if (pk.splats) ts::pack_one(pk, i, c0, c1, c2, pk.channels == 4 ? pk.depths[i] : 0.0f);
+    Batch::evaluate(a, g0, cnt, lds);
 }
 
 template <int DEG>
@@ -614,6 +560,7 @@
 #undef TS_SHC_SPARSE
         return launch_status();
     }
+    const ts::ColorsArgs ca{num_bases, means3d, origin, colors_dc, colors_rest, colors, clamp_mask, pk};
     const int ka = (degrees_to_use + 1) * (degrees_to_use + 1);
     const size_t lds = (size_t)kShThreadsFwd * ((3 * (ka - 1)) | 1) * sizeof(float);
     const int grid_d = (n + kShThreadsFwd - 1) / kShThreadsFwd;
@@ -622,8 +569,7 @@
         if (lds > 48 * 1024)                                                                      \
             (void)hipFuncSetAttribute(reinterpret_cast<const void*>(&sh_colors_fwd_kernel<D>),    \
                                       hipFuncAttributeMaxDynamicSharedMemorySize, (int)lds);      \
-        hipLaunchKernelGGL(sh_colors_fwd_kernel<D>, dim3(grid_d), dim3(kShThreadsFwd), lds, s, n,  \
-                           num_bases, means3d, origin, colors_dc, colors_rest, colors, clamp_mask, pk); \
+        hipLaunchKernelGGL(sh_colors_fwd_kernel<D>, dim3(grid_d), dim3(kShThreadsFwd), lds, s, n, ca); \
     } while (0)
     switch (degrees_to_use) {
         case 0: TS_SHC_FWD(0); break;
diff --git a/tinysplat_amd/csrc/splat_math.h b/tinysplat_amd/csrc/splat_math.h
--- a/tinysplat_amd/csrc/splat_math.h
+++ b/tinysplat_amd/csrc/splat_math.h
@@ -363,6 +363,8 @@
     return log2f(x);
 #endif
 }
+
+TS_HD float record_opacity(float op, bool logit) { return logit ? 1.0f / (1.0f + expf(-op)) : op; }
 
 constexpr int kTilePix = 16;
 constexpr float kTightEps = 0.02f;
diff --git a/tinysplat_amd/frame.py b/tinysplat_amd/frame.py
--- a/tinysplat_amd/frame.py
+++ b/tinysplat_amd/frame.py
@@ -166,6 +166,22 @@
 DIRECT_GRADS = os.environ.get("TS_DIRECT_GRADS", "1") != "0"
 
 SURVIVORS = os.environ.get("TS_SURVIVORS", "1") != "0"
+
+FUSED_COLORS = os.environ.get("TS_FUSED_COLORS", "1") != "0"
+FUSED_COLORS_FROM = int(os.environ.get("TS_FUSED_COLORS_FROM", str(1 << 18)))
+FUSED_SPLIT = tuple(float(x) for x in os.environ.get("TS_FUSED_SPLIT", "0,0").split(","))
+FUSED_SPLIT_FORCE = None
+
+
+def _fused_split(n: int):
+    if FUSED_SPLIT_FORCE is not None:
+        a = max(0, min(n, int(FUSED_SPLIT_FORCE[0])))
+        return a, max(a, min(n, int(FUSED_SPLIT_FORCE[1])))
+    fa, fc = FUSED_SPLIT
+    a = min(n, int(n * min(max(fa, 0.0), 1.0)) // 1024 * 1024) if fa < 1.0 else n
+    c = min(n, int(n * min(max(fc, 0.0), 1.0)) // 1024 * 1024) if fc < 1.0 else n
+    return a, max(a, c)
+
 
 CAPACITY_ALLOC = os.environ.get("TS_CAPACITY_ALLOC", "0") != "0"
 CAPACITY_GROWTH = 1.25
@@ -298,6 +314,9 @@
             fr.flags |= 512
         if full:
             _stats_mode[dev.index] = mode
+        if FUSED_COLORS and full and mode == 0 and not stripe and n >= FUSED_COLORS_FROM:
+            fr.flags |= 1024
+            fr.fused_a, fr.fused_c = _fused_split(n)
         fr.cam = cam
         fr.means, fr.scales, fr.quats, fr.opacities = means.data_ptr(), scales.data_ptr(), quats.data_ptr(), opacities.data_ptr()
         fr.colors_dc, fr.colors_rest = colors_dc.data_ptr(), colors_rest.data_ptr()
```
